# LANL-Bioinformatics/PCRamp

Measured on AMD Instinct MI355X. Metric: primer-pair x target amplification evals/sec, higher is better.
Workload: dtype u32

## Files before the change

### pcramp_amd/csrc/pcr_device.hip

```cpp
#include <hip/hip_runtime.h>
#include <cstring>
#include <rocprim/device/device_radix_sort.hpp>

#include <stdint.h>
#include <string.h>
#include <math.h>
#include <stdlib.h>
#include <string>
#include <vector>
#include <chrono>
#include <algorithm>
#include <unordered_map>
#include <type_traits>
#include <thread>
#include <mutex>
#include <condition_variable>
#include <functional>
#include <memory>
#include <atomic>
#include <cassert>
#include <sched.h>
#include <pthread.h>

#include "../../include/pcramp_hip.h"
#include "pcr_host.hpp"
#include "pcr_launch_queue.hpp"

using pcrhost::Planes;

namespace { thread_local std::string g_err; }
#include "pcr_owned.hpp"

namespace {

using pcrown::DevBuf; using pcrown::MappedBuf; using pcrown::Event; using pcrown::Stream;

#define HIP_TRY(expr) do{ hipError_t e_ = (expr); if(e_ != hipSuccess){ \
	g_err = std::string(#expr) + ": " + hipGetErrorString(e_); return PCR_ERR_DEVICE; } }while(0)

constexpr int TILE_POS = 1024;
constexpr int SCAN_THREADS = 256;
constexpr int SCAN_NPOS = TILE_POS/SCAN_THREADS;

constexpr int KEY_SEQ_SHIFT = 40;
constexpr int KEY_LOC_SHIFT = 8;
constexpr int LOC_BIAS = 64;

struct Hit { uint64_t key; uint32_t cand; uint32_t cnt; };

struct PassMail { volatile uint32_t counters[4]; volatile uint32_t seq; uint32_t pad[11]; };

constexpr uint32_t N_TOUCHED_UNKNOWN_DEV = 0xFFFFFFFFu;

struct IrrDev { Planes w; int32_t loc; uint32_t seq; uint32_t meta;  uint32_t local_id; };

struct DevEntry { Planes w; int32_t loc; uint32_t seq; uint32_t strand; uint32_t pad; };

struct OligoDev {
	Planes m;
	uint32_t floor2;
	float norm;
	int32_t start, stop;
	uint32_t p1, p2;
};

__constant__ float c_taq_mama[256];

const float h_taq_mama[256] = {
	1.000f, 0.968f, 0.947f, 1.034f, 0.547f, 0.253f, 0.230f, 0.359f, 0.606f, 0.282f, 0.372f, 0.347f, 0.957f, 0.382f, 0.399f, 0.687f,
	0.989f, 1.000f, 1.023f, 1.000f, 0.420f, 0.662f, 0.445f, 0.367f, 0.870f, 0.512f, 0.492f, 0.508f, 0.372f, 1.000f, 0.492f, 0.714f,
	1.011f, 1.000f, 1.000f, 1.000f, 0.459f, 0.277f, 0.570f, 0.343f, 0.927f, 0.362f, 0.590f, 0.542f, 0.439f, 0.488f, 0.978f, 0.662f,
	1.000f, 0.907f, 1.000f, 1.000f, 0.382f, 0.234f, 0.228f, 0.542f, 0.763f, 0.309f, 0.410f, 0.473f, 0.426f, 0.347f, 0.423f, 0.947f,
	0.590f, 0.334f, 0.445f, 0.323f, 1.000f, 0.978f, 0.927f, 0.989f, 0.907f, 0.645f, 0.525f, 0.455f, 0.927f, 0.408f, 0.408f, 0.707f,
	0.327f, 0.595f, 0.319f, 0.396f, 0.947f, 1.000f, 0.978f, 0.989f, 0.405f, 0.861f, 0.681f, 0.512f, 0.410f, 0.968f, 0.452f, 0.714f,
	0.410f, 0.420f, 0.590f, 0.311f, 1.023f, 1.000f, 1.000f, 1.000f, 0.488f, 0.898f, 0.907f, 0.566f, 0.442f, 0.449f, 0.989f, 0.707f,
	0.423f, 0.343f, 0.305f, 0.585f, 1.034f, 0.879f, 0.927f, 1.000f, 0.473f, 0.720f, 0.547f, 0.957f, 0.459f, 0.374f, 0.459f, 1.023f,
	1.023f, 0.429f, 0.473f, 0.477f, 1.023f, 0.466f, 0.420f, 0.477f, 1.000f, 0.978f, 0.907f, 0.978f, 0.907f, 0.380f, 0.525f, 0.669f,
	0.442f, 1.046f, 0.455f, 0.470f, 0.432f, 1.058f, 0.481f, 0.485f, 0.917f, 1.000f, 1.023f, 1.023f, 0.336f, 0.968f, 0.534f, 0.639f,
	0.617f, 0.452f, 1.011f, 0.439f, 0.492f, 0.504f, 0.978f, 0.462f, 0.989f, 0.947f, 1.000f, 0.978f, 0.405f, 0.405f, 0.888f, 0.606f,
	0.601f, 0.377f, 0.377f, 1.046f, 0.500f, 0.399f, 0.408f, 1.034f, 0.978f, 0.720f, 0.870f, 1.000f, 0.402f, 0.313f, 0.651f, 0.927f,
	0.978f, 0.462f, 0.466f, 0.488f, 0.420f, 0.239f, 0.225f, 0.336f, 0.504f, 0.269f, 0.319f, 0.656f, 1.000f, 0.835f, 0.907f, 1.034f,
	0.429f, 1.011f, 0.473f, 0.477f, 0.340f, 0.413f, 0.357f, 0.354f, 0.352f, 0.538f, 0.413f, 0.794f, 0.927f, 1.000f, 1.058f, 1.000f,
	0.595f, 0.492f, 0.968f, 0.485f, 0.367f, 0.282f, 0.388f, 0.439f, 0.413f, 0.309f, 0.566f, 0.917f, 0.957f, 0.957f, 1.000f, 0.989f,
	0.590f, 0.380f, 0.410f, 0.968f, 0.364f, 0.223f, 0.230f, 0.416f, 0.321f, 0.239f, 0.301f, 0.645f, 0.978f, 0.714f, 0.947f, 1.000f
};

__device__ __forceinline__ uint32_t funnel(uint32_t lo, uint32_t hi, uint32_t sh)
{
	return __builtin_amdgcn_alignbit(hi, lo, sh);
}

__device__ __forceinline__ uint32_t match_count(uint32_t wa, uint32_t wc, uint32_t wg, uint32_t wt, const uint4 m)
{
	return __popc((wa & m.x) | (wc & m.y) | (wg & m.z) | (wt & m.w));
}

__global__ void k_transpose(const uint8_t *__restrict__ packed, const uint64_t *__restrict__ byte_off,
	const uint64_t *__restrict__ len, const uint64_t *__restrict__ blk_off, const uint32_t *__restrict__ blk_seq,
	uint4 *__restrict__ planes, uint32_t *__restrict__ nib, uint32_t *__restrict__ tb, uint64_t total_blocks)
{
	const uint64_t gb = (uint64_t)blockIdx.x*blockDim.x + threadIdx.x;
	if(gb >= total_blocks) return;
	const uint32_t s = blk_seq[gb];
	const uint64_t b = gb - blk_off[s];
	const uint64_t L = len[s];
	const uint8_t *src = packed + byte_off[s];
	uint32_t a = 0, c = 0, g = 0, t = 0;
	uint32_t nw[4] = {0, 0, 0, 0};
	uint32_t tw[2] = {0, 0};
	for(int j = 0;j < 32;++j){
		const uint64_t pos = b*32 + j;
		if(pos >= L) break;
		const uint8_t v = src[pos >> 1];
		const uint32_t code = (pos & 1) ? (v & 0xF) : (v >> 4);
		a |= (code & 1u) << j;
		c |= ((code >> 1) & 1u) << j;
		g |= ((code >> 2) & 1u) << j;
		t |= ((code >> 3) & 1u) << j;
		nw[j >> 3] |= code << ((j & 7)*4);
		const uint32_t c2 = (code == 2) ? 1u : (code == 4) ? 2u : (code == 8) ? 3u : 0u;
		tw[j >> 4] |= c2 << ((j & 15)*2);
	}
	planes[gb] = make_uint4(a, c, g, t);
	((uint4 *)nib)[gb] = make_uint4(nw[0], nw[1], nw[2], nw[3]);
	((uint2 *)tb)[gb] = make_uint2(tw[0], tw[1]);
}

__global__ void k_valid(const uint4 *__restrict__ planes, const uint64_t *__restrict__ blk_off,
	const uint32_t *__restrict__ blk_seq, const uint64_t *__restrict__ nblk_real, uint32_t *__restrict__ valid,
	uint64_t total_blocks, uint32_t max_degen, uint64_t gc_ok, uint64_t first_block, uint64_t n_blocks)
{
	const uint64_t i = (uint64_t)blockIdx.x*blockDim.x + threadIdx.x;
	if(i >= n_blocks) return;
	const uint64_t gb = first_block + i;
	if(gb >= total_blocks) return;
	const uint32_t s = blk_seq[gb];
	const uint64_t b = gb - blk_off[s];
	if(b >= nblk_real[s]){ valid[gb] = 0; return; }
	const uint4 lo = planes[gb];
	const uint4 hi = planes[gb + 1];
	uint32_t nzl, d2l, d3l, d4l, cgl, nzh, d2h, d3h, d4h, cgh;
	{
		const uint32_t x = lo.x ^ lo.y, y = lo.x & lo.y, u = lo.z ^ lo.w, v = lo.z & lo.w;
		const uint32_t ones = x ^ u, c1 = x & u;
		const uint32_t twos = y ^ v ^ c1;
		const uint32_t fours = (y & v) | (c1 & (y ^ v));
		nzl = lo.x | lo.y | lo.z | lo.w;
		d2l = ~ones & twos & ~fours; d3l = ones & twos; d4l = fours;
		cgl = lo.y | lo.z;
	}
	{
		const uint32_t x = hi.x ^ hi.y, y = hi.x & hi.y, u = hi.z ^ hi.w, v = hi.z & hi.w;
		const uint32_t ones = x ^ u, c1 = x & u;
		const uint32_t twos = y ^ v ^ c1;
		const uint32_t fours = (y & v) | (c1 & (y ^ v));
		nzh = hi.x | hi.y | hi.z | hi.w;
		d2h = ~ones & twos & ~fours; d3h = ones & twos; d4h = fours;
		cgh = hi.y | hi.z;
	}
	uint32_t out = 0;
	for(uint32_t j = 0;j < 32;++j){
		if(funnel(nzl, nzh, j) != 0xFFFFFFFFu) continue;
		const uint32_t ngc = __popc(funnel(cgl, cgh, j));
		if(!((gc_ok >> ngc) & 1ull)) continue;
		const uint32_t n2 = __popc(funnel(d2l, d2h, j));
		const uint32_t n3 = __popc(funnel(d3l, d3h, j));
		const uint32_t n4 = __popc(funnel(d4l, d4h, j));
		const uint32_t e = n2 + 2*n4;
		bool exceeds;
		if(e >= 33){ exceeds = true; }
		else{
			uint64_t p3 = 1;
			for(uint32_t k = 0;k < n3;++k) p3 *= 3;
			exceeds = p3 > ((uint64_t)max_degen >> e);
		}
		if(!exceeds) out |= (1u << j);
	}
	valid[gb] = out;
}

struct HitSink { uint32_t *best; Hit *hits; uint32_t *seq_count; uint32_t *counters; uint32_t cap; uint32_t ncand; uint32_t epoch; };

__device__ __forceinline__ void record_hit_inline(const HitSink &k, uint32_t seq, uint32_t cand, uint64_t key, uint32_t cnt)
{
	const uint32_t tagged = (k.epoch << 8) | cnt;
	const uint32_t old = atomicMax(&k.best[(size_t)seq*k.ncand + cand], tagged);
	if(tagged >= old){
		const uint32_t slot = atomicAdd(&k.seq_count[seq], 1u);
		if(slot < k.cap){
			Hit h; h.key = key; h.cand = cand; h.cnt = cnt;
			k.hits[(size_t)seq*k.cap + slot] = h;
		}
		else{ atomicOr(&k.counters[0], 1u); atomicMax(&k.counters[2], slot + 1); }
	}
}

__device__ __noinline__ void record_hit(const HitSink k, uint32_t seq, uint32_t cand, uint64_t key, uint32_t cnt)
{
	record_hit_inline(k, seq, cand, key, cnt);
}

__device__ __forceinline__ uint64_t make_key(uint32_t seq, int32_t loc, uint32_t strand , uint32_t kind, uint32_t ord)
{
	return ((uint64_t)seq << KEY_SEQ_SHIFT) | ((uint64_t)(uint32_t)(loc + LOC_BIAS) << KEY_LOC_SHIFT) |
		((uint64_t)(strand - 1) << 7) | ((uint64_t)kind << 6) | ord;
}

__global__ void k_touched(const uint32_t *__restrict__ seq_count, uint32_t n, uint32_t *__restrict__ counters, uint32_t *__restrict__ touched)
{
	const uint32_t s = blockIdx.x*blockDim.x + threadIdx.x;
	const uint32_t fill = (s < n) ? seq_count[s] : 0u;
	const bool has = fill > 0;
	const uint64_t mask = __ballot(has);
	if(!mask) return;
	const uint32_t lane = threadIdx.x & 63u, leader = (uint32_t)__builtin_ctzll(mask);
	{
		uint32_t mx = fill;
		for(int d = 32;d > 0;d >>= 1) mx = max(mx, (uint32_t)__shfl_xor((int)mx, d));
		if(lane == leader) atomicMax(&counters[2], mx);
	}
	uint32_t base = 0;
	if(lane == leader) base = atomicAdd(&counters[3], (uint32_t)__builtin_popcountll(mask));
	base = __shfl(base, leader);
	if(has) touched[base + (uint32_t)__builtin_popcountll(mask & ((1ull << lane) - 1ull))] = s;
}

__global__ void k_touched_seg(const uint32_t *__restrict__ seg_hi, uint32_t n, uint32_t *__restrict__ counters, uint32_t *__restrict__ touched)
{
	const uint32_t s = blockIdx.x*blockDim.x + threadIdx.x;
	const bool has = s < n && seg_hi[s] != 0;
	const uint64_t mask = __ballot(has);
	if(!mask) return;
	const uint32_t lane = threadIdx.x & 63u, leader = (uint32_t)__builtin_ctzll(mask);
	uint32_t base = 0;
	if(lane == leader) base = atomicAdd(&counters[3], (uint32_t)__builtin_popcountll(mask));
	base = __shfl(base, leader);
	if(has) touched[base + (uint32_t)__builtin_popcountll(mask & ((1ull << lane) - 1ull))] = s;
}

__global__ __launch_bounds__(SCAN_THREADS) void k_scan(
	const uint4 *__restrict__ planes, const uint32_t *__restrict__ valid,
	const uint64_t *__restrict__ blk_off, const uint64_t *__restrict__ len, const uint8_t *__restrict__ active,
	const uint32_t *__restrict__ tile_seq, const uint32_t *__restrict__ tile_pos0,
	const uint4 *__restrict__ cand_fwd, const uint4 *__restrict__ cand_rc, const uint32_t *__restrict__ cand_floor,
	uint32_t ncand, HitSink sink)
{
	const uint32_t tile = blockIdx.x;
	const uint32_t seq = tile_seq[tile];
	if(!active[seq]) return;
	const uint64_t L = len[seq];
	const uint64_t base = blk_off[seq];
	const uint32_t p0 = tile_pos0[tile];

	uint32_t wa[SCAN_NPOS], wc[SCAN_NPOS], wg[SCAN_NPOS], wt[SCAN_NPOS], ok[SCAN_NPOS];
#pragma unroll
	for(int i = 0;i < SCAN_NPOS;++i){
		const uint32_t p = p0 + threadIdx.x + SCAN_THREADS*i;
		wa[i] = wc[i] = wg[i] = wt[i] = 0; ok[i] = 0;
		if((uint64_t)p + 32 <= L){
			const uint32_t b = p >> 5, sh = p & 31;
			const uint4 lo = planes[base + b];
			const uint4 hi = planes[base + b + 1];
			wa[i] = funnel(lo.x, hi.x, sh); wc[i] = funnel(lo.y, hi.y, sh);
			wg[i] = funnel(lo.z, hi.z, sh); wt[i] = funnel(lo.w, hi.w, sh);
			ok[i] = (valid[base + b] >> sh) & 1u;
		}
	}

	for(uint32_t c = 0;c < ncand;++c){
		const uint4 mf = cand_fwd[c];
		const uint4 mr = cand_rc[c];
		const uint32_t fl = cand_floor[c];
#pragma unroll
		for(int i = 0;i < SCAN_NPOS;++i){
			const uint32_t cf = match_count(wa[i], wc[i], wg[i], wt[i], mf);
			const uint32_t cr = match_count(wa[i], wc[i], wg[i], wt[i], mr);
			if((cf >= fl || cr >= fl) && ok[i]){
				const int32_t p = (int32_t)(p0 + threadIdx.x + SCAN_THREADS*i);
				if(cf >= fl) record_hit(sink, seq, c, make_key(seq, p, 1, 0, 0), cf);
				if(cr >= fl) record_hit(sink, seq, c, make_key(seq, p + 31, 2, 0, 0), cr);
			}
		}
	}
}

constexpr int IRR_THREADS = 256, IRR_PER_LANE = 2;
struct IrrArgs { const IrrDev *irr; const uint32_t *perm; uint32_t n_live; uint32_t off_mask;  };

__device__ __forceinline__ void scan_irr_block(uint32_t block, const IrrDev *__restrict__ irr, const uint32_t *__restrict__ perm, uint32_t n_live,
	const uint8_t *__restrict__ active, const uint4 *__restrict__ cand_fwd, const uint32_t *__restrict__ cand_floor, uint32_t ncand,
	const HitSink &sink)
{
	uint32_t wa[IRR_PER_LANE], wc[IRR_PER_LANE], wg[IRR_PER_LANE], wt[IRR_PER_LANE];
	const uint32_t i0 = block*(IRR_THREADS*IRR_PER_LANE) + threadIdx.x;
#pragma unroll
	for(int k = 0;k < IRR_PER_LANE;++k){
		const uint32_t i = i0 + k*IRR_THREADS;
		wa[k] = wc[k] = wg[k] = wt[k] = 0;
		if(i < n_live){
			const IrrDev e = irr[perm[i]];
			if(active[e.seq]){ wa[k] = e.w.a; wc[k] = e.w.c; wg[k] = e.w.g; wt[k] = e.w.t; }
		}
	}
#pragma unroll 8
	for(uint32_t c = 0;c < ncand;++c){
		const uint4 m = cand_fwd[c];
		const uint32_t fl = max(cand_floor[c], 1u);
		const bool zero_floor = cand_floor[c] == 0;
#pragma unroll
		for(int k = 0;k < IRR_PER_LANE;++k){
			const uint32_t cnt = match_count(wa[k], wc[k], wg[k], wt[k], m);
			if(cnt >= fl || (zero_floor && (wa[k] | wc[k] | wg[k] | wt[k]))){
				const IrrDev e = irr[perm[i0 + k*IRR_THREADS]];
				record_hit(sink, e.seq, c, make_key(e.seq, e.loc, e.meta & 0xFF, 1, (e.meta >> 16) & 0xFF), cnt);
			}
		}
	}
}

__global__ __launch_bounds__(IRR_THREADS) void k_scan_irr(const IrrDev *__restrict__ irr, const uint32_t *__restrict__ perm, uint32_t n_live,
	const uint8_t *__restrict__ active, const uint4 *__restrict__ cand_fwd, const uint32_t *__restrict__ cand_floor, uint32_t ncand,
	HitSink sink)
{
	scan_irr_block(blockIdx.x, irr, perm, n_live, active, cand_fwd, cand_floor, ncand, sink);
}

__device__ __forceinline__ void wave_sync() { __builtin_amdgcn_fence(__ATOMIC_ACQ_REL, "wavefront"); __builtin_amdgcn_wave_barrier(); }

#include "pcr_scan_bitsliced.inc"
#include "pcr_scan_seed.inc"
#include "pcr_scan_seed2.inc"
#include "pcr_scan_seed3.inc"

constexpr int FIN_WAVES = 8;
constexpr uint32_t MAX_BUCKET_CAP = 8192;


__device__ __forceinline__ void materialise_entry_at(uint64_t k, const uint4 *__restrict__ planes, uint64_t seq_base,
	const IrrDev *__restrict__ irr, const uint32_t *__restrict__ irr_off, DevEntry &e)
{
	const uint32_t seq = (uint32_t)(k >> KEY_SEQ_SHIFT);
	const int32_t loc = (int32_t)(uint32_t)((k >> KEY_LOC_SHIFT) & 0xFFFFFFFFull) - LOC_BIAS;
	const uint32_t strand = (uint32_t)((k >> 7) & 1) + 1;
	const uint32_t kind = (uint32_t)((k >> 6) & 1), ord = (uint32_t)(k & 63);
	e.loc = loc; e.seq = seq; e.strand = strand; e.pad = 0;
	if(kind == 0){
		const uint32_t p = (strand == 1) ? (uint32_t)loc : (uint32_t)(loc - 31);
		const uint32_t b = p >> 5, sh = p & 31;
		const uint4 lo = planes[seq_base + b];
		const uint4 hi = planes[seq_base + b + 1];
		const uint32_t a = funnel(lo.x, hi.x, sh), c = funnel(lo.y, hi.y, sh);
		const uint32_t g = funnel(lo.z, hi.z, sh), t = funnel(lo.w, hi.w, sh);
		if(strand == 1){ e.w.a = a; e.w.c = c; e.w.g = g; e.w.t = t; }
		else{ e.w.a = __brev(t); e.w.t = __brev(a); e.w.c = __brev(g); e.w.g = __brev(c); }
	}
	else{
		e.w.a = e.w.c = e.w.g = e.w.t = 0;
		for(uint32_t j = irr_off[seq];j < irr_off[seq + 1];++j){
			const IrrDev r = irr[j];
			if(r.loc == loc && (r.meta & 0xFF) == strand && ((r.meta >> 16) & 0xFF) == ord){ e.w = r.w; break; }
		}
	}
}

__device__ void materialise_entry(uint64_t k, const uint4 *__restrict__ planes, const uint64_t *__restrict__ blk_off,
	const IrrDev *__restrict__ irr, const uint32_t *__restrict__ irr_off, DevEntry &e)
{
	const uint32_t seq = (uint32_t)(k >> KEY_SEQ_SHIFT);
	const int32_t loc = (int32_t)(uint32_t)((k >> KEY_LOC_SHIFT) & 0xFFFFFFFFull) - LOC_BIAS;
	const uint32_t strand = (uint32_t)((k >> 7) & 1) + 1;
	const uint32_t kind = (uint32_t)((k >> 6) & 1), ord = (uint32_t)(k & 63);
	e.loc = loc; e.seq = seq; e.strand = strand; e.pad = 0;
	if(kind == 0){
		const uint32_t p = (strand == 1) ? (uint32_t)loc : (uint32_t)(loc - 31);
		const uint32_t b = p >> 5, sh = p & 31;
		const uint4 lo = planes[blk_off[seq] + b];
		const uint4 hi = planes[blk_off[seq] + b + 1];
		const uint32_t a = funnel(lo.x, hi.x, sh), c = funnel(lo.y, hi.y, sh);
		const uint32_t g = funnel(lo.z, hi.z, sh), t = funnel(lo.w, hi.w, sh);
		if(strand == 1){ e.w.a = a; e.w.c = c; e.w.g = g; e.w.t = t; }
		else{ e.w.a = __brev(t); e.w.t = __brev(a); e.w.c = __brev(g); e.w.g = __brev(c); }
	}
	else{
		e.w.a = e.w.c = e.w.g = e.w.t = 0;
		for(uint32_t j = irr_off[seq];j < irr_off[seq + 1];++j){
			const IrrDev r = irr[j];
			if(r.loc == loc && (r.meta & 0xFF) == strand && ((r.meta >> 16) & 0xFF) == ord){ e.w = r.w; break; }
		}
	}
}

template<int WAVES, bool ALL = false>
__global__ __launch_bounds__(64*WAVES) void k_finalize(const Hit *__restrict__ hits, const uint32_t *__restrict__ seq_count,
	uint32_t cap, const uint32_t *__restrict__ best, uint32_t ncand, const uint4 *__restrict__ planes,
	const uint64_t *__restrict__ blk_off, const IrrDev *__restrict__ irr, const uint32_t *__restrict__ irr_off,
	DevEntry *__restrict__ db, uint32_t *__restrict__ seg_hi, uint32_t *__restrict__ counters, uint32_t epoch,
	const uint32_t *__restrict__ touched)
{
	extern __shared__ __attribute__((aligned(16))) uint64_t fin_lds[];
	__shared__ uint32_t part_all[64*WAVES];
	const uint32_t wave = threadIdx.x >> 6, lane = threadIdx.x & 63;
	uint32_t np2cap = 1; while(np2cap < cap) np2cap <<= 1;
	for(uint32_t t_idx = blockIdx.x*WAVES + wave;t_idx < counters[3];t_idx += gridDim.x*WAVES){
	const uint32_t seq = touched[t_idx];
	uint64_t *fin_keys = fin_lds + (size_t)wave*np2cap;
	uint32_t *part = part_all + wave*64;
	const uint32_t n = min(seq_count[seq], cap);
	uint32_t np2 = 1; while(np2 < n) np2 <<= 1;
	for(uint32_t i = lane;i < np2;i += 64){
		uint64_t k = ~0ull;
		if(i < n){
			const Hit h = hits[(size_t)seq*cap + i];
			if constexpr (ALL) k = h.key;
			else if(((epoch << 8) | h.cnt) == best[(size_t)seq*ncand + h.cand]) k = h.key;
		}
		fin_keys[i] = k;
	}
	wave_sync();
	for(uint32_t k = 2;k <= np2;k <<= 1){
		for(uint32_t j = k >> 1;j > 0;j >>= 1){
			for(uint32_t i = lane;i < np2;i += 64){
				const uint32_t l = i ^ j;
				if(l > i){
					const uint64_t a = fin_keys[i], b = fin_keys[l];
					const bool up = ((i & k) == 0);
					if((a > b) == up){ fin_keys[i] = b; fin_keys[l] = a; }
				}
			}
			wave_sync();
		}
	}
	const uint32_t chunk = (np2 + 63)/64;
	const uint32_t lo = lane*chunk, hi = min(np2, lo + chunk);
	uint32_t cnt = 0;
	for(uint32_t i = lo;i < hi;++i){
		const uint64_t k = fin_keys[i];
		if(k != ~0ull && (i == 0 || fin_keys[i - 1] != k)) ++cnt;
	}
	part[lane] = cnt;
	wave_sync();
	if(lane == 0){
		uint32_t run = 0;
		for(int t = 0;t < 64;++t){ const uint32_t c = part[t]; part[t] = run; run += c; }
		seg_hi[seq] = seq*cap + run;
	}
	wave_sync();
	uint32_t rank = part[lane];
	for(uint32_t i = lo;i < hi;++i){
		const uint64_t k = fin_keys[i];
		if(k != ~0ull && (i == 0 || fin_keys[i - 1] != k)){
			DevEntry e;
			materialise_entry(k, planes, blk_off, irr, irr_off, e);
			db[(size_t)seq*cap + rank] = e;
			++rank;
		}
	}
	wave_sync();
	}
}

constexpr int FINBIG_THREADS = 256;
constexpr uint32_t MAX_BUCKET_CAP_GLOBAL = 65536;
template<bool ALL = false>
__global__ __launch_bounds__(FINBIG_THREADS) void k_finalize_big(const Hit *__restrict__ hits, const uint32_t *__restrict__ seq_count,
	uint32_t cap, const uint32_t *__restrict__ best, uint32_t ncand, const uint4 *__restrict__ planes,
	const uint64_t *__restrict__ blk_off, const IrrDev *__restrict__ irr, const uint32_t *__restrict__ irr_off,
	DevEntry *__restrict__ db, uint32_t *__restrict__ seg_hi, uint32_t *__restrict__ counters, uint32_t epoch,
	const uint32_t *__restrict__ touched, uint64_t *__restrict__ scratch)
{
	__shared__ uint32_t part[FINBIG_THREADS];
	if(blockIdx.x >= counters[3]) return;
	const uint32_t seq = touched[blockIdx.x], tid = threadIdx.x;
	uint32_t np2cap = 1; while(np2cap < cap) np2cap <<= 1;
	uint64_t *fin_keys = scratch + (size_t)blockIdx.x*np2cap;
	const uint32_t n = min(seq_count[seq], cap);
	uint32_t np2 = 1; while(np2 < n) np2 <<= 1;
	for(uint32_t i = tid;i < np2;i += FINBIG_THREADS){
		uint64_t k = ~0ull;
		if(i < n){
			const Hit h = hits[(size_t)seq*cap + i];
			if constexpr (ALL) k = h.key;
			else if(((epoch << 8) | h.cnt) == best[(size_t)seq*ncand + h.cand]) k = h.key;
		}
		fin_keys[i] = k;
	}
	__syncthreads();
	for(uint32_t k = 2;k <= np2;k <<= 1){
		for(uint32_t j = k >> 1;j > 0;j >>= 1){
			for(uint32_t i = tid;i < np2;i += FINBIG_THREADS){
				const uint32_t l = i ^ j;
				if(l > i){
					const uint64_t a = fin_keys[i], b = fin_keys[l];
					const bool up = ((i & k) == 0);
					if((a > b) == up){ fin_keys[i] = b; fin_keys[l] = a; }
				}
			}
			__syncthreads();
		}
	}
	const uint32_t chunk = (np2 + FINBIG_THREADS - 1)/FINBIG_THREADS;
	const uint32_t lo = min(np2, tid*chunk), hi = min(np2, lo + chunk);
	uint32_t cnt = 0;
	for(uint32_t i = lo;i < hi;++i){
		const uint64_t k = fin_keys[i];
		if(k != ~0ull && (i == 0 || fin_keys[i - 1] != k)) ++cnt;
	}
	part[tid] = cnt;
	__syncthreads();
	if(tid == 0){
		uint32_t run = 0;
		for(int t = 0;t < FINBIG_THREADS;++t){ const uint32_t c = part[t]; part[t] = run; run += c; }
		seg_hi[seq] = seq*cap + run;
	}
	__syncthreads();
	uint32_t rank = part[tid];
	for(uint32_t i = lo;i < hi;++i){
		const uint64_t k = fin_keys[i];
		if(k != ~0ull && (i == 0 || fin_keys[i - 1] != k)){
			DevEntry e;
			materialise_entry(k, planes, blk_off, irr, irr_off, e);
			db[(size_t)seq*cap + rank] = e;
			++rank;
		}
	}
}

#include "pcr_screen.inc"

#include "pcr_sw.inc"
#include "pcr_thermo.inc"

constexpr uint32_t N_TOUCHED_UNKNOWN = 0xFFFFFFFFu;
constexpr uint32_t EPOCH_LIMIT = (1u << 24) - 1;

struct SeqSet {
	uint32_t n = 0;
	std::vector<std::vector<uint8_t> > packed;
	std::vector<uint64_t> len, blk_off, nblk_real;
	std::vector<float> weight; DevBuf<float> d_weight; bool weight_dirty = true;
	std::vector<uint8_t> active;
	std::vector<std::vector<pcrhost::IrrEntry> > irr_host;
	uint64_t total_blocks = 0;
	uint32_t n_tiles = 0, n_irr = 0;
	bool ctrl_clean = false;
	bool touched_from_seg = false;
	uint32_t bucket_cap = 64;
	DevBuf<uint32_t> irr_perm; uint32_t irr_size_count[256];
	DevBuf<uint4> planes;
	DevBuf<uint32_t> valid, nib, tb, blk_seq, tile_seq, tile_pos0, irr_off, degen_tiles;
	uint32_t *valid_d() const { return valid.p + S2_VALID_FRONT; }
	uint32_t *tb_d() const { return tb.p + S2_TB_FRONT; }
	DevBuf<uint8_t> tile_degen; uint32_t n_degen_tiles = 0;
	DevBuf<TileDesc> tile_desc;
	DevBuf<uint64_t> d_len, d_blk_off, d_nblk_real;
	DevBuf<uint8_t> d_active;
	std::vector<uint8_t> has_eos; DevBuf<uint8_t> d_has_eos;
	DevBuf<IrrDev> irr;
	DevBuf<IrrScan> irr_scan;
	DevBuf<uint32_t> irx_first, irx_last, irx_words, irx_sums; bool irx_valid = false, irx_usable = false;
	uint32_t irr_n_multi = 0;
	DevBuf<uint32_t> pix_first, pix_last, pix_sums, blk_info, blk_local, blk_tile0; DevBuf<uint4> pix_ent; std::vector<uint32_t> pix_start_h; uint64_t pix_generation = 0; bool pix_valid = false, pix_usable = false;
	DevBuf<uint8_t> codes; DevBuf<uint64_t> d_code_off; bool have_codes = false;
	bool have_db = false;
	uint32_t n_entries = 0;
	uint32_t db_cap = 0;
	uint64_t n_slots = 0;
	DevBuf<DevEntry> db;
	DevBuf<uint32_t> touched;
	DevBuf<uint32_t> ctrl;
	uint32_t n_touched = 0;
	bool touched_built = false;
	uint32_t *d_seg_hi = nullptr;
};

}

struct HostPool {
	std::vector<std::thread> th;
	std::mutex m; std::condition_variable cv_go, cv_done;
	std::function<void(unsigned)> fn; unsigned n_parts = 0, next = 0, pending = 0; uint64_t gen = 0; bool stop = false;
	explicit HostPool(unsigned n_workers){ for(unsigned i = 0;i < n_workers;++i) th.emplace_back([this]{ work(); }); }
	~HostPool(){ { std::lock_guard<std::mutex> lk(m); stop = true; } cv_go.notify_all(); for(std::thread &t : th) t.join(); }
	unsigned size() const { return (unsigned)th.size(); }
	void work()
	{
		uint64_t seen = 0;
		std::unique_lock<std::mutex> lk(m);
		while(true){
			cv_go.wait(lk, [&]{ return stop || gen != seen; });
			if(stop) return;
			seen = gen;
			while(next < n_parts){ const unsigned p = next++; lk.unlock(); fn(p); lk.lock(); }
			if(--pending == 0) cv_done.notify_one();
		}
	}
	void run(unsigned parts, std::function<void(unsigned)> f)
	{
		std::unique_lock<std::mutex> lk(m);
		fn = std::move(f); n_parts = parts; next = 0; pending = (unsigned)th.size(); ++gen;
		cv_go.notify_all();
		while(next < n_parts){ const unsigned p = next++; lk.unlock(); fn(p); lk.lock(); }
		cv_done.wait(lk, [&]{ return pending == 0; });
	}
};

namespace { struct PassJob; struct Launcher; }

struct pcr_ctx {
	int device = 0;
	std::unique_ptr<HostPool> pool_;
	HostPool &host_pool()
	{
		if(!pool_){ const unsigned hw = std::max(1u, std::thread::hardware_concurrency()); pool_.reset(new HostPool(std::min(hw, 16u) - 1u)); }
		return *pool_;
	}
	Stream stream;
	Stream aux_stream;
	std::string design_text;
	DevBuf<uint64_t> split_where;
	pcr_params params;
	pcrhost::PackFilter filt;
	SeqSet sets[PCR_N_SETS];
	DevBuf<uint32_t> best, counters, mask, status;
	int scan_version = 3;
	bool force_seed1 = false;
	struct S2Key { uint32_t a, c, g, t, floor_; bool operator==(const S2Key &o) const { return a == o.a && c == o.c && g == o.g && t == o.t && floor_ == o.floor_; } };
	struct S2KeyHash { size_t operator()(const S2Key &k) const { uint64_t h = 0x9E3779B97F4A7C15ull; for(uint32_t v : {k.a, k.c, k.g, k.t, k.floor_}){ h ^= v; h *= 0x100000001B3ull; h ^= h >> 29; } return (size_t)h; } };
	struct S2Entry { std::vector<uint32_t> seeds;  uint32_t off_mask; bool seedable; uint4 mask;  };
	std::unordered_map<S2Key, S2Entry, S2KeyHash> s2_cache;
	std::vector<pcrhost::Seed> s2_tmp;
	static constexpr int S3_CHUNK_SETS = 4;
	struct S3Chunks { uint64_t gen = 0; uint32_t total = 0; std::vector<uint32_t> run; };
	struct S3Entry : S2Entry { std::vector<uint8_t> spans;  S3Chunks chunks[S3_CHUNK_SETS]; uint32_t next_slot = 0; };
	std::unordered_map<S2Key, S3Entry, S2KeyHash> s3_cache;
	std::vector<pcrhost::FoldSeed> s3_tmp;
	struct S3Launch { Seed3Slices W; uint32_t n_chunks, per_wg, slice_cap, n_irr_wg; };
	bool no_seed3 = false, s3_attr_set = false;
	bool s3_next = true;
	bool s2_attr_set = false; uint32_t s2_dbg = 0; bool no_irr_index = false;
	std::unordered_map<S2Key, S2Entry, S2KeyHash> s1_cache;
	DevBuf<uint32_t> s1_image, s1_heads, s1_multi, s1_part;
	bool host_seed_tables = false;
	DevBuf<Hit> hits;
	DevBuf<uint64_t> bits_fr, bits_rf;
	DevBuf<OligoDev> oligos;
	DevBuf<SwJob> sw_jobs; DevBuf<SwOut> sw_out; DevBuf<uint8_t> sw_q, sw_qlen, sw_t, entry_codes, entry_lens;
	DevBuf<AmpRec> amp_recs, amp_recs2; DevBuf<BgPairDev> bg_pairs;
	DevBuf<uint64_t> amp_keys; DevBuf<uint32_t> amp_pkeys, amp_pair_start; DevBuf<uint8_t> sort_tmp;
	DevBuf<thermo::Job> th_jobs; DevBuf<thermo::JobOut> th_out; DevBuf<int> th_dg; DevBuf<uint2> th_map; DevBuf<uint32_t> th_bad;
	float th_dg_salt = -1.0f;
	DevBuf<unsigned long long> th_dbg; bool th_attr_set = false;
	std::vector<thermo::Job> th_host_jobs; std::vector<thermo::JobOut> th_host_res;
	MappedBuf<uint8_t> sw_pin; Event sw_done[2];
	DevBuf<pcr_amplicon> mx_amp;
	DevBuf<OligoDev> opt_oligos; DevBuf<uint2> opt_jobs; DevBuf<float> opt_cov; DevBuf<uint32_t> opt_loc, opt_tasks;
	DevBuf<Planes> mx_keys; uint32_t mx_n_keys = 0; DevBuf<uint32_t> mx_count;
	DevBuf<uint8_t> pool_in, pool_tmp; DevBuf<uint32_t> pool_cnt, pool_ord; DevBuf<uint64_t> pool_eoff, pool_ioff, pool_keys; DevBuf<uint2> pool_items; DevBuf<pcr_product> pool_rec;
	DevBuf<uint8_t> site_in, site_tmp; DevBuf<uint32_t> site_cnt, site_ord, site_flag; DevBuf<uint64_t> site_eoff, site_joff, site_keys; DevBuf<uint2> site_items; DevBuf<float4> site_res; DevBuf<pcr_site> site_rec;
	bool site_attr_set = false;
	pcr_comm *shard_comm = nullptr; uint64_t shard_first = 0, shard_n_total = 0; int shard_mode = 0;
	DevBuf<uint64_t> sh_rec, sh_full; DevBuf<uint8_t> sh_stage;
	std::vector<uint64_t> shard_bounds; DevBuf<uint64_t> d_shard_bounds;
	bool design_ready = false; DevBuf<uint64_t> sh_bits;
	std::vector<std::vector<uint8_t> > samp_packed; std::vector<uint64_t> samp_len;
	void drop_shard(){ shard_comm = nullptr; shard_mode = 0; shard_bounds.clear(); design_ready = false; samp_packed.clear(); samp_len.clear(); }
	pcr_comm *trial_comm = nullptr;
	size_t amp_cap = size_t(1) << 20;
	uint32_t n_cu = 256;
	DevBuf<uint64_t> fin_scratch;
	std::vector<uint16_t> seed_count; std::vector<uint8_t> seed_fill, seed_own;
	uint32_t epoch = 0;
	uint32_t debug_epoch = 0;
	bool opt_pm_global = false;
	uint32_t opt_dbg_wg_tasks = 0, opt_dbg_task_cap = 0;
	uint64_t best_seen = 0;
	static constexpr int STAGE_RING = 4;
	struct StageSlot { MappedBuf<uint8_t> buf; Event done; bool busy = false;
	                   uint32_t guard_seq = 0;  };
	StageSlot stage[STAGE_RING]; int stage_next = 0;
	struct DirectSlot { DevBuf<uint8_t> buf{true}; uint32_t guard_seq = 0; };
	DirectSlot dstage[STAGE_RING]; int dstage_next = 0;
	bool direct_ok = false;
	typedef PassMail Mail;
	static constexpr uint32_t MAIL_RING = 8;
	MappedBuf<Mail> mail;
	uint32_t mail_seq = 0;
	MappedBuf<uint8_t> ret;
	MappedBuf<uint8_t> in;
	MappedBuf<uint32_t> ret_flag; uint32_t ret_seq = 0;
	struct Pending {
		uint32_t seq; int which; std::vector<pcr_pair> pairs; int opt5, opt3; float thr; uint32_t min_len;
		pcr_amplify_args args; uint64_t *d_fr, *d_rf;
	};
	std::vector<Pending> pending;
	bool launch_thread = true;
	Launcher *launcher = nullptr; pcrq::Client lq_client; uint64_t n_pipelined = 0;
	std::mutex job_m; std::vector<PassJob *> job_free, job_all;
	DevBuf<uint8_t> arena;
	const uint4 *d_cand_fwd = nullptr, *d_cand_rc = nullptr; const uint32_t *d_cand_floor = nullptr;
	const OligoDev *d_oligos = nullptr;
	bool debug_log = false;
	bool timing = false; double t_host[8] = {0, 0, 0, 0, 0, 0, 0, 0}; uint64_t n_timed = 0;
	bool prof = false; uint32_t prof_stride = 1, prof_pass = 0;
	std::vector<std::pair<Event, Event> > prof_events;
	double prof_ms = 0.0; uint64_t prof_launches = 0;
	std::vector<std::pair<Event, Event> > prof_events_k[PCR_PROF_KERNELS];
	double prof_ms_k[PCR_PROF_KERNELS] = {0.0, 0.0, 0.0}; uint64_t prof_launches_k[PCR_PROF_KERNELS] = {0, 0, 0};
};

namespace {

int drain(pcr_ctx *ctx);
int flush_launcher(pcr_ctx *ctx);
void detach_launcher(pcr_ctx *ctx);
void free_jobs(pcr_ctx *ctx);

struct ProfScope {
	pcr_ctx *ctx; int k; Event e0, e1;
	ProfScope(pcr_ctx *c, int kernel, bool on = true) : ctx(c), k(kernel)
	{
		if(!on || !ctx->prof || k < 0 || k >= PCR_PROF_KERNELS) return;
		if(e0.create() != hipSuccess || e1.create() != hipSuccess){ e0.release(); return; }
		(void)hipEventRecord(e0, ctx->stream);
	}
	void finish()
	{
		if(!e0) return;
		(void)hipEventRecord(e1, ctx->stream);
		((k == PCR_PROF_SCAN) ? ctx->prof_events : ctx->prof_events_k[k]).emplace_back(std::move(e0), std::move(e1));
	}
	~ProfScope() { finish(); }
};
constexpr int PCR_SET_SCRATCH = 3;
inline bool set_ok(pcr_set which) { return (unsigned)which <= (unsigned)PCR_SET_MULTIPLEX; }
#define CHECK_SET(which) do{ if(!set_ok(which)){ g_err = "unknown sequence set (PCR_SET_TARGET, PCR_SET_BACKGROUND or PCR_SET_MULTIPLEX)"; return PCR_ERR_ARG; } }while(0)
#define FLUSH(ctx) do{ if((ctx)->launcher){ const int frc_ = flush_launcher(ctx); if(frc_ != PCR_OK) return frc_; } }while(0)
#define DRAIN(ctx) do{ FLUSH(ctx); if(!(ctx)->pending.empty()){ const int drc_ = drain(ctx); if(drc_ != PCR_OK) return drc_; } }while(0)

struct HostTimer {
	pcr_ctx *ctx; int slot; std::chrono::steady_clock::time_point t0;
	HostTimer(pcr_ctx *c, int s) : ctx(c), slot(s) { if(ctx->timing) t0 = std::chrono::steady_clock::now(); }
	void next(int s)
	{
		if(!ctx->timing) return;
		const auto t1 = std::chrono::steady_clock::now();
		ctx->t_host[slot] += std::chrono::duration<double, std::micro>(t1 - t0).count();
		slot = s; t0 = t1;
	}
	~HostTimer() { next(slot); }
};

__global__ void k_apply_splits(const uint64_t *__restrict__ where, uint32_t n, uint32_t *__restrict__ planes , uint32_t *__restrict__ nib)
{
	const uint32_t i = blockIdx.x*blockDim.x + threadIdx.x;
	if(i >= n) return;
	const uint64_t gb = where[2*(size_t)i];
	const uint32_t bit = (uint32_t)where[2*(size_t)i + 1];
	const uint32_t m = ~(1u << bit);
	for(int k = 0;k < 4;++k) atomicAnd(&planes[gb*4 + k], m);
	atomicAnd(&nib[gb*4 + (bit >> 3)], ~(0xFu << ((bit & 7u)*4u)));
}

int upload_irregular(pcr_ctx *ctx, SeqSet &S)
{
	const auto tu0 = std::chrono::steady_clock::now();
	auto ms_since = [&](){ return std::chrono::duration<double, std::milli>(std::chrono::steady_clock::now() - tu0).count(); };
	double t_flat = 0, t_sort = 0, t_scan = 0, t_copy1 = 0;
	size_t total = 0;
	for(uint32_t s = 0;s < S.n;++s) total += S.irr_host[s].size();
	std::vector<IrrDev> flat(total);
	std::vector<uint32_t> off(S.n + 1, 0);
	for(int k = 0;k < 256;++k) S.irr_size_count[k] = 0;
	{
		size_t at = 0;
		for(uint32_t s = 0;s < S.n;++s){
			off[s] = (uint32_t)at;
			const std::vector<pcrhost::IrrEntry> &v = S.irr_host[s];
			for(size_t k = 0;k < v.size();++k){
				const pcrhost::IrrEntry &e = v[k];
				IrrDev &d = flat[at++];
				d.w = e.w; d.loc = e.loc; d.seq = s;
				d.meta = (uint32_t)e.strand | ((uint32_t)e.cws << 8) | ((uint32_t)e.ord << 16);
				d.local_id = (uint32_t)k;
				++S.irr_size_count[e.cws & 0xFF];
			}
		}
	}
	off[S.n] = (uint32_t)flat.size();
	S.n_irr = (uint32_t)flat.size();
	t_flat = ms_since();
	std::vector<uint32_t> perm(flat.size());
	t_sort = ms_since();
	int rc;
	{
		auto spread = [](uint64_t v) -> uint64_t {
			v = (v | (v << 16)) & 0x0000FFFF0000FFFFull; v = (v | (v << 8)) & 0x00FF00FF00FF00FFull; v = (v | (v << 4)) & 0x0F0F0F0F0F0F0F0Full;
			v = (v | (v << 2)) & 0x3333333333333333ull; v = (v | (v << 1)) & 0x5555555555555555ull; return v;
		};
		uint32_t start[256];
		uint32_t run = 0;
		for(int k = 255;k >= 0;--k){ start[k] = run; run += S.irr_size_count[k]; }
		std::vector<IrrScan> scan(perm.size());
		uint32_t n_multi = 0;
		for(size_t i = 0;i < flat.size();++i){
			const IrrDev &d = flat[i];
			const uint32_t at = start[(d.meta >> 8) & 0xFF]++;
			perm[at] = (uint32_t)i;
			const uint32_t multi = (d.w.a & d.w.c) | (d.w.a & d.w.g) | (d.w.a & d.w.t) | (d.w.c & d.w.g) | (d.w.c & d.w.t) | (d.w.g & d.w.t);
			if(multi) ++n_multi;
			const uint32_t lo = d.w.c | d.w.t, hi = d.w.g | d.w.t;
			const uint64_t code = spread(lo) | (spread(hi) << 1);
			IrrScan r; r.w0 = (uint32_t)code; r.w1 = (uint32_t)(code >> 32); r.idx_flags = (uint32_t)i | (multi ? 0x80000000u : 0u); r.seq = d.seq;
			scan[at] = r;
		}
		S.irr_n_multi = n_multi; S.irx_valid = false;
		t_scan = ms_since();
		if((rc = S.irr_scan.ensure_slack(scan.size() + 1)) != PCR_OK) return rc;
		if(!scan.empty()) HIP_TRY(hipMemcpy(S.irr_scan.p, scan.data(), scan.size()*sizeof(IrrScan), hipMemcpyHostToDevice));
	}
	t_copy1 = ms_since();
	if((rc = S.irr_perm.ensure_slack(perm.size() + 1)) != PCR_OK) return rc;
	if(!perm.empty()) HIP_TRY(hipMemcpyAsync(S.irr_perm.p, perm.data(), perm.size()*sizeof(uint32_t), hipMemcpyHostToDevice, ctx->stream));
	if((rc = S.irr.ensure_slack(flat.size())) != PCR_OK) return rc;
	if((rc = S.irr_off.ensure(off.size())) != PCR_OK) return rc;
	if(!flat.empty()) HIP_TRY(hipMemcpyAsync(S.irr.p, flat.data(), flat.size()*sizeof(IrrDev), hipMemcpyHostToDevice, ctx->stream));
	HIP_TRY(hipMemcpyAsync(S.irr_off.p, off.data(), off.size()*sizeof(uint32_t), hipMemcpyHostToDevice, ctx->stream));
	HIP_TRY(hipStreamSynchronize(ctx->stream));
	if(ctx->timing && flat.size() > 100000) fprintf(stderr, "[pcramp] irregular list of %zu words: flat %.1f  order %.1f  scan records %.1f  first copy %.1f  other copies %.1f ms\n", flat.size(), t_flat, t_sort - t_flat, t_scan - t_sort, t_copy1 - t_scan, ms_since() - t_copy1);
	return PCR_OK;
}

void launch_exclusive_scan(pcr_ctx *ctx, uint32_t *counts, uint32_t *starts, uint32_t n, uint32_t *sums)
{
	const uint32_t n_blocks = (n + 4095u)/4096u;
	hipLaunchKernelGGL(k_scan_blocks, dim3(n_blocks), dim3(1024), 0, ctx->stream, counts, starts, n, sums);
	hipLaunchKernelGGL(k_scan_sums, dim3(1), dim3(1024), 0, ctx->stream, sums, n_blocks);
	hipLaunchKernelGGL(k_scan_add, dim3(n_blocks), dim3(1024), 0, ctx->stream, starts, counts, n, sums);
}

constexpr uint32_t IRX_MAX_RUN = 1024;
int ensure_irr_index(pcr_ctx *ctx, SeqSet &S)
{
	if(S.irx_valid) return PCR_OK;
	int rc;
	if((rc = S.irx_first.ensure(IRX_KEYS + 4)) != PCR_OK) return rc;
	if((rc = S.irx_last.ensure(IRX_KEYS + 4)) != PCR_OK) return rc;
	if((rc = S.irx_words.ensure_slack((size_t)24*S.n_irr + 4)) != PCR_OK) return rc;
	const uint32_t n_blocks = (IRX_KEYS + 4095u)/4096u;
	if((rc = S.irx_sums.ensure(n_blocks + 4)) != PCR_OK) return rc;
	HIP_TRY(hipMemsetAsync(S.irx_last.p, 0, (size_t)IRX_KEYS*sizeof(uint32_t), ctx->stream));
	if(S.n_irr){
		hipLaunchKernelGGL(k_irx_count, dim3((S.n_irr + 255)/256), dim3(256), 0, ctx->stream, S.irr.p, S.n_irr, S.irx_last.p);
		HIP_TRY(hipGetLastError());
	}
	{
		uint32_t longest = 0;
		HIP_TRY(hipMemsetAsync(S.irx_sums.p + n_blocks, 0, sizeof(uint32_t), ctx->stream));
		hipLaunchKernelGGL(k_irx_max, dim3(256), dim3(256), 0, ctx->stream, S.irx_last.p, IRX_KEYS, S.irx_sums.p + n_blocks);
		HIP_TRY(hipMemcpyAsync(&longest, S.irx_sums.p + n_blocks, sizeof(uint32_t), hipMemcpyDeviceToHost, ctx->stream));
		HIP_TRY(hipStreamSynchronize(ctx->stream));
		S.irx_usable = longest <= IRX_MAX_RUN;
		if(!S.irx_usable){ S.irx_valid = true; return PCR_OK; }
	}
	launch_exclusive_scan(ctx, S.irx_last.p, S.irx_first.p, IRX_KEYS, S.irx_sums.p);
	HIP_TRY(hipGetLastError());
	if(S.n_irr){
		hipLaunchKernelGGL(k_irx_scatter, dim3((S.n_irr + 255)/256), dim3(256), 0, ctx->stream, S.irr.p, S.n_irr, S.irx_last.p, S.irx_words.p);
		HIP_TRY(hipGetLastError());
	}
	S.irx_valid = true;
	return PCR_OK;
}

int ensure_pos_index(pcr_ctx *ctx, SeqSet &S)
{
	if(S.pix_valid) return PCR_OK;
	S.pix_valid = true; S.pix_usable = false;
	if(S.total_blocks == 0 || S.total_blocks*32 >= (uint64_t(1) << 32) - 64) return PCR_OK;
	int rc;
	if((rc = S.pix_first.ensure(PIX_KEYS + 4)) != PCR_OK) return rc;
	if((rc = S.pix_last.ensure(PIX_KEYS + 4)) != PCR_OK) return rc;
	const uint32_t n_blocks = (PIX_KEYS + 4095u)/4096u;
	if((rc = S.pix_sums.ensure(n_blocks + 4)) != PCR_OK) return rc;
	if((rc = S.pix_ent.ensure(S.total_blocks*32 + 64)) != PCR_OK) return rc;
	{
		if(S.n >= (1u << 30)){ return PCR_OK; }
		if((rc = S.blk_info.ensure(S.total_blocks + 1)) != PCR_OK) return rc;
		if((rc = S.blk_local.ensure(S.total_blocks + 1)) != PCR_OK) return rc;
		std::vector<uint32_t> tile0((size_t)S.n + 1);
		uint64_t t0 = 0;
		for(uint32_t q = 0;q < S.n;++q){ tile0[q] = (uint32_t)t0; t0 += (S.len[q] >= 32) ? (S.len[q] - 7 + TILE_POS - 1)/TILE_POS : 0; }
		tile0[S.n] = (uint32_t)t0;
		if(t0 >= (uint64_t(1) << 32)) return PCR_OK;
		if((rc = S.blk_tile0.ensure((size_t)S.n + 1)) != PCR_OK) return rc;
		HIP_TRY(hipMemcpyAsync(S.blk_tile0.p, tile0.data(), ((size_t)S.n + 1)*sizeof(uint32_t), hipMemcpyHostToDevice, ctx->stream));
		hipLaunchKernelGGL(k_blk_info, dim3((unsigned)((S.total_blocks + 255)/256)), dim3(256), 0, ctx->stream, S.blk_seq.p, S.d_blk_off.p, S.d_len.p,
			S.blk_tile0.p, S.tile_degen.p, S.d_active.p, S.total_blocks, S.blk_info.p, S.blk_local.p);
		HIP_TRY(hipGetLastError());
		HIP_TRY(hipStreamSynchronize(ctx->stream));
	}
	HIP_TRY(hipMemsetAsync(S.pix_last.p, 0, (size_t)PIX_KEYS*sizeof(uint32_t), ctx->stream));
	const unsigned grid = (unsigned)((S.total_blocks + 255)/256);
	hipLaunchKernelGGL(k_pix_build<false>, dim3(grid), dim3(256), 0, ctx->stream, S.tb_d(), S.blk_seq.p, S.d_blk_off.p, S.d_len.p, S.total_blocks, S.pix_last.p, (uint4 *)nullptr);
	launch_exclusive_scan(ctx, S.pix_last.p, S.pix_first.p, PIX_KEYS, S.pix_sums.p);
	hipLaunchKernelGGL(k_pix_build<true>, dim3(grid), dim3(256), 0, ctx->stream, S.tb_d(), S.blk_seq.p, S.d_blk_off.p, S.d_len.p, S.total_blocks, S.pix_last.p, S.pix_ent.p);
	HIP_TRY(hipGetLastError());
	{
		S.pix_start_h.resize((size_t)PIX_KEYS + 1);
		HIP_TRY(hipMemcpyAsync(S.pix_start_h.data(), S.pix_first.p, (size_t)PIX_KEYS*sizeof(uint32_t), hipMemcpyDeviceToHost, ctx->stream));
		HIP_TRY(hipMemcpyAsync(S.pix_start_h.data() + PIX_KEYS, S.pix_last.p + (PIX_KEYS - 1), sizeof(uint32_t), hipMemcpyDeviceToHost, ctx->stream));
		HIP_TRY(hipStreamSynchronize(ctx->stream));
		static uint64_t generations = 0;
		S.pix_generation = ++generations;
	}
	S.pix_usable = true;
	return PCR_OK;
}

int run_valid(pcr_ctx *ctx, SeqSet &S, uint64_t first_block, uint64_t n_blocks)
{
	if(n_blocks == 0) return PCR_OK;
	const unsigned threads = 256;
	const unsigned grid = (unsigned)((n_blocks + threads - 1)/threads);
	hipLaunchKernelGGL(k_valid, dim3(grid), dim3(threads), 0, ctx->stream, S.planes.p, S.d_blk_off.p, S.blk_seq.p,
		S.d_nblk_real.p, S.valid_d(), S.total_blocks, ctx->filt.max_degen, ctx->filt.gc_ok, first_block, n_blocks);
	HIP_TRY(hipGetLastError());
	return PCR_OK;
}

int build_tile_desc(pcr_ctx *ctx, SeqSet &S)
{
	if(S.n_tiles == 0) return PCR_OK;
	int rc = S.tile_desc.ensure(S.n_tiles);
	if(rc != PCR_OK) return rc;
	hipLaunchKernelGGL(k_tile_desc, dim3((S.n_tiles + 255)/256), dim3(256), 0, ctx->stream, S.d_blk_off.p, S.d_len.p, S.d_active.p, S.tile_seq.p,
		S.tile_pos0.p, S.tile_degen.p, S.n_tiles, S.tile_desc.p);
	HIP_TRY(hipGetLastError());
	return PCR_OK;
}

void fill_oligo_planes(OligoDev &o, const Planes &m, float thr2)
{
	o.m = m;
	const unsigned size = (unsigned)pcrhost::planes_size(o.m);
	o.floor2 = (unsigned)((float)size*thr2);
	o.norm = (size > 0) ? (float)(1.0/size) : 0.0f;
	o.start = pcrhost::planes_start(o.m);
	o.stop = pcrhost::planes_stop(o.m);
	o.p1 = (o.stop >= 1) ? pcrhost::planes_nibble(o.m, o.stop - 1) : 0;
	o.p2 = (o.stop >= 0) ? pcrhost::planes_nibble(o.m, o.stop) : 0;
}

void fill_oligo(OligoDev &o, const uint64_t w[2], float thr2) { fill_oligo_planes(o, pcrhost::planes_of_word(w), thr2); }

__global__ void k_stage(const uint4 *__restrict__ src, uint4 *__restrict__ dst, uint32_t n16,
	uint4 *__restrict__ z0, uint32_t n0, uint4 *__restrict__ z1, uint32_t n1, uint4 *__restrict__ z2, uint32_t n2)
{
	const uint32_t i = blockIdx.x*blockDim.x + threadIdx.x, stride = gridDim.x*blockDim.x;
	for(uint32_t k = i;k < n16;k += stride) dst[k] = src[k];
	const uint4 zero = make_uint4(0, 0, 0, 0);
	for(uint32_t k = i;k < n0;k += stride) z0[k] = zero;
	for(uint32_t k = i;k < n1;k += stride) z1[k] = zero;
	for(uint32_t k = i;k < n2;k += stride) z2[k] = zero;
}

enum SpinEnd { SPIN_SEEN, SPIN_IDLE, SPIN_ERROR };
template<class Seen> inline SpinEnd spin_until(hipStream_t stream, Seen seen, hipError_t &err)
{
	for(uint64_t spins = 1;!seen();++spins){
		__builtin_ia32_pause();
		if((spins & 0x3FFF) == 0){
			err = hipStreamQuery(stream);
			if(err == hipSuccess) return SPIN_IDLE;
			if(err != hipErrorNotReady) return SPIN_ERROR;
		}
	}
	return SPIN_SEEN;
}

int wait_published(pcr_ctx *ctx, uint32_t seq)
{
	const PassMail *const slot = ctx->mail.host + (seq % pcr_ctx::MAIL_RING);
	hipError_t e = hipSuccess;
	const SpinEnd end = spin_until(ctx->stream, [&]{
		const uint32_t v = __atomic_load_n((const uint32_t *)&slot->seq, __ATOMIC_ACQUIRE);
		return v >= seq && (v - seq) % pcr_ctx::MAIL_RING == 0; }, e);
	if(end == SPIN_ERROR){ g_err = std::string("device pass failed: ") + hipGetErrorString(e); return PCR_ERR_DEVICE; }
	return PCR_OK;
}

struct Stager {
	pcr_ctx *ctx; size_t used = 0; bool direct = false;
	explicit Stager(pcr_ctx *c) : ctx(c) {}
	pcr_ctx::StageSlot *slot = nullptr; pcr_ctx::DirectSlot *dslot = nullptr;
	uint8_t *host = nullptr, *dev = nullptr;
	int begin_direct(size_t bytes)
	{
		direct = true;
		dslot = &ctx->dstage[ctx->dstage_next];
		ctx->dstage_next = (ctx->dstage_next + 1) % pcr_ctx::STAGE_RING;
		if(dslot->guard_seq){ const int grc = wait_published(ctx, dslot->guard_seq); if(grc != PCR_OK) return grc; dslot->guard_seq = 0; }
		if(bytes + 256 > dslot->buf.cap){
			if(dslot->buf.p) HIP_TRY(hipStreamSynchronize(ctx->stream));
			const int rc = dslot->buf.ensure(std::max<size_t>((bytes + 256)*2, 1 << 17));
			if(rc != PCR_OK) return rc;
		}
		host = dev = dslot->buf.p;
		used = 0;
		return PCR_OK;
	}
	void seal(uint32_t pass_seq)
	{
		__builtin_ia32_sfence();
		dslot->guard_seq = pass_seq + 1;
	}
	int begin(size_t bytes)
	{
		slot = &ctx->stage[ctx->stage_next];
		ctx->stage_next = (ctx->stage_next + 1) % pcr_ctx::STAGE_RING;
		if(slot->busy){ HIP_TRY(hipEventSynchronize(slot->done)); slot->busy = false; }
		if(slot->guard_seq){ const int grc = wait_published(ctx, slot->guard_seq); if(grc != PCR_OK) return grc; slot->guard_seq = 0; }
		int rc = slot->buf.ensure(bytes, std::max<size_t>(bytes*2, 1 << 16));
		if(rc != PCR_OK) return rc;
		host = slot->buf.host; dev = slot->buf.dev;
		if(!slot->done) HIP_TRY(slot->done.create(hipEventDisableTiming));
		rc = ctx->arena.ensure(bytes + 256);
		used = 0;
		return rc;
	}
	template<class T> T *put(const T *src, size_t n)
	{
		used = (used + 15) & ~size_t(15);
		memcpy(host + used, src, n*sizeof(T));
		T *at = (T *)((direct ? dev : ctx->arena.p) + used);
		used += n*sizeof(T);
		return at;
	}
	int ship(void *z0 = nullptr, size_t bytes0 = 0, void *z1 = nullptr, size_t bytes1 = 0, void *z2 = nullptr, size_t bytes2 = 0, uint32_t guard_seq = 0)
	{
		const uint32_t n16 = (uint32_t)((used + 15)/16), n0 = (uint32_t)((bytes0 + 15)/16), n1 = (uint32_t)((bytes1 + 15)/16), n2 = (uint32_t)((bytes2 + 15)/16);
		const uint32_t most = std::max(std::max(n16, n2), std::max(n0, n1));
		if(most){
			const unsigned grid = std::min<unsigned>((most + 255)/256, 512u);
			hipLaunchKernelGGL(k_stage, dim3(grid), dim3(256), 0, ctx->stream, (const uint4 *)dev, (uint4 *)ctx->arena.p, n16,
				(uint4 *)z0, n0, (uint4 *)z1, n1, (uint4 *)z2, n2);
			HIP_TRY(hipGetLastError());
		}
		if(guard_seq) slot->guard_seq = guard_seq;
		else{
			HIP_TRY(hipEventRecord(slot->done, ctx->stream));
			slot->busy = true;
		}
		return PCR_OK;
	}
};

__global__ void k_publish(const uint32_t *__restrict__ counters, pcr_ctx::Mail *mail, uint32_t seq)
{
	if(threadIdx.x < 4) mail->counters[threadIdx.x] = counters[threadIdx.x];
	__threadfence_system();
	__syncthreads();
	if(threadIdx.x == 0) __hip_atomic_store((uint32_t *)&mail->seq, seq, __ATOMIC_RELEASE, __HIP_MEMORY_SCOPE_SYSTEM);
}

int mail_wait(pcr_ctx *ctx, uint32_t seq, uint32_t out[4])
{
	pcr_ctx::Mail *const slot = ctx->mail.host + (seq % pcr_ctx::MAIL_RING);
	auto seen = [&]{ return __atomic_load_n((const uint32_t *)&slot->seq, __ATOMIC_ACQUIRE) == seq; };
	hipError_t e = hipSuccess;
	const SpinEnd end = spin_until(ctx->stream, seen, e);
	if(end == SPIN_ERROR){ g_err = std::string("device pass failed: ") + hipGetErrorString(e); return PCR_ERR_DEVICE; }
	if(end == SPIN_IDLE && !seen()){ g_err = "device pass finished without publishing its counters"; return PCR_ERR_DEVICE; }
	for(int i = 0;i < 4;++i) out[i] = slot->counters[i];
	return PCR_OK;
}

__global__ void k_return(const uint4 *__restrict__ s0, uint32_t n0, const uint4 *__restrict__ s1, uint32_t n1,
	const uint4 *__restrict__ s2, uint32_t n2, uint4 *__restrict__ dst)
{
	const uint32_t stride = gridDim.x*blockDim.x, t = blockIdx.x*blockDim.x + threadIdx.x;
	for(uint32_t i = t;i < n0;i += stride) dst[i] = s0[i];
	for(uint32_t i = t;i < n1;i += stride) dst[n0 + i] = s1[i];
	for(uint32_t i = t;i < n2;i += stride) dst[n0 + n1 + i] = s2[i];
}

__global__ void k_return_flag(uint32_t *flag, uint32_t seq)
{
	__threadfence_system();
	__hip_atomic_store(flag, seq, __ATOMIC_RELEASE, __HIP_MEMORY_SCOPE_SYSTEM);
}

int return_to_host(pcr_ctx *ctx, const void *s0, size_t b0, const void *s1, size_t b1, const void *s2, size_t b2, const uint8_t *out[3])
{
	const uint32_t n0 = (uint32_t)((b0 + 15)/16), n1 = (uint32_t)((b1 + 15)/16), n2 = (uint32_t)((b2 + 15)/16);
	const size_t need = ((size_t)n0 + n1 + n2)*16;
	int rc;
	if(!ctx->ret_flag.host){
		if((rc = ctx->ret_flag.ensure(64)) != PCR_OK) return rc;
		*ctx->ret_flag.host = 0;
	}
	if(need > ctx->ret.cap){
		HIP_TRY(hipStreamSynchronize(ctx->stream));
		if((rc = ctx->ret.ensure(need, std::max<size_t>(need*2, 1 << 20))) != PCR_OK) return rc;
	}
	const uint32_t most = std::max(n0, std::max(n1, n2));
	if(most){
		const unsigned grid = std::min<unsigned>((most + 255)/256, 1024u);
		hipLaunchKernelGGL(k_return, dim3(grid), dim3(256), 0, ctx->stream, (const uint4 *)s0, n0, (const uint4 *)s1, n1, (const uint4 *)s2, n2, (uint4 *)ctx->ret.dev);
		HIP_TRY(hipGetLastError());
	}
	const uint32_t seq = ++ctx->ret_seq;
	hipLaunchKernelGGL(k_return_flag, dim3(1), dim3(1), 0, ctx->stream, ctx->ret_flag.dev, seq);
	HIP_TRY(hipGetLastError());
	auto seen = [&]{ return __atomic_load_n((const uint32_t *)ctx->ret_flag.host, __ATOMIC_ACQUIRE) == seq; };
	hipError_t e = hipSuccess;
	const SpinEnd end = spin_until(ctx->stream, seen, e);
	if(end == SPIN_ERROR){ g_err = std::string("device work failed: ") + hipGetErrorString(e); return PCR_ERR_DEVICE; }
	if(end == SPIN_IDLE && !seen()){ g_err = "device work finished without raising the return flag"; return PCR_ERR_DEVICE; }
	out[0] = ctx->ret.host; out[1] = ctx->ret.host + (size_t)n0*16; out[2] = ctx->ret.host + ((size_t)n0 + n1)*16;
	return PCR_OK;
}

int mapped_input(pcr_ctx *ctx, const void *src, size_t bytes, const void **dev_out)
{
	if(bytes > ctx->in.cap){
		HIP_TRY(hipStreamSynchronize(ctx->stream));
		const int rc = ctx->in.ensure(bytes, std::max<size_t>(bytes*2, 1 << 18));
		if(rc != PCR_OK) return rc;
	}
	memcpy(ctx->in.host, src, bytes);
	*dev_out = ctx->in.dev;
	return PCR_OK;
}

struct FusedAmp {
	const pcr_pair *pairs; uint32_t n_pairs; const pcr_amplify_args *a; uint64_t *d_fr, *d_rf;
	bool staged = false; const OligoDev *d_oligos = nullptr; uint32_t pub_seq = 0; const uint32_t *pub_counters = nullptr;
	bool posted = false;
};

void build_oligos(const pcr_pair *pairs, uint32_t n_pairs, const pcr_amplify_args *a, std::vector<OligoDev> &ol)
{
	const float thr2 = a->collect_threshold*a->collect_threshold;
	ol.resize(2*(size_t)n_pairs);
	for(uint32_t i = 0;i < n_pairs;++i){
		fill_oligo(ol[2*i], pairs[i].f.w, thr2);
		fill_oligo(ol[2*i + 1], pairs[i].r.w, thr2);
	}
}

int ensure_touched(pcr_ctx *ctx, SeqSet &S)
{
	if(S.touched_built || !S.have_db || !S.ctrl.p) return PCR_OK;
	if(S.touched_from_seg) hipLaunchKernelGGL(k_touched_seg, dim3((S.n + 255)/256), dim3(256), 0, ctx->stream, S.d_seg_hi, S.n, S.ctrl.p, S.touched.p);
	else hipLaunchKernelGGL(k_touched, dim3((S.n + 255)/256), dim3(256), 0, ctx->stream, S.ctrl.p + 8, S.n, S.ctrl.p, S.touched.p);
	HIP_TRY(hipGetLastError());
	uint32_t n = 0;
	HIP_TRY(hipMemcpyAsync(&n, S.ctrl.p + 3, sizeof(uint32_t), hipMemcpyDeviceToHost, ctx->stream));
	HIP_TRY(hipStreamSynchronize(ctx->stream));
	S.n_touched = n; S.n_entries = n ? 1 : 0; S.touched_built = true;
	return PCR_OK;
}

int amplify_launch(pcr_ctx *ctx, SeqSet &S, const pcr_pair *pairs, uint32_t n_pairs, const pcr_amplify_args *a,
	uint64_t *d_fr, uint64_t *d_rf, const FusedAmp *fa = nullptr)
{
	{ const int erc = ensure_touched(ctx, S); if(erc != PCR_OK) return erc; }
	if(!S.have_db){ g_err = "pcr_amplify: no word DB (call pcr_select_words first)"; return PCR_ERR_STATE; }
	const uint64_t words = (S.n + 63)/64;
	const size_t bits_bytes = (size_t)n_pairs*words*sizeof(uint64_t);
	if(S.n_entries == 0 || n_pairs == 0){
		if(bits_bytes){
			HIP_TRY(hipMemsetAsync(d_fr, 0, bits_bytes, ctx->stream));
			HIP_TRY(hipMemsetAsync(d_rf, 0, bits_bytes, ctx->stream));
		}
		return PCR_OK;
	}
	HostTimer timer(ctx, 4);
	int rc;
	const bool prestaged = fa && fa->staged;
	if(prestaged) ctx->d_oligos = fa->d_oligos;
	else{
		std::vector<OligoDev> ol;
		build_oligos(pairs, n_pairs, a, ol);
		Stager st(ctx);
		if((rc = st.begin(ol.size()*sizeof(OligoDev) + 64)) != PCR_OK) return rc;
		ctx->d_oligos = st.put(ol.data(), ol.size());
		const bool vec_ok = ((uintptr_t)d_fr % 16 == 0) && ((uintptr_t)d_rf % 16 == 0) && (bits_bytes % 16 == 0);
		if(!vec_ok){
			HIP_TRY(hipMemsetAsync(d_fr, 0, bits_bytes, ctx->stream));
			HIP_TRY(hipMemsetAsync(d_rf, 0, bits_bytes, ctx->stream));
		}
		if((rc = vec_ok ? st.ship(d_fr, bits_bytes, d_rf, bits_bytes) : st.ship()) != PCR_OK) return rc;
	}
	timer.next(5);
	const uint32_t mask_words = (2*n_pairs + 31)/32;
	if((rc = ctx->mask.ensure((size_t)S.n_slots*mask_words)) != PCR_OK) return rc;
	if((rc = ctx->status.ensure(1)) != PCR_OK) return rc;
	const bool dev_n = S.n_touched == N_TOUCHED_UNKNOWN;
	const uint32_t *n_dev = dev_n ? S.ctrl.p + 3 : nullptr;
	const uint32_t n_t = dev_n ? 0u : S.n_touched, n_db = n_t*S.db_cap;
	const unsigned threads = dev_n ? 256 : 128;
	const unsigned grid = dev_n ? (unsigned)std::min<uint64_t>(((uint64_t)S.n*S.db_cap + threads - 1)/threads, 1024) : (n_db + threads - 1)/threads;
	const unsigned mgrid = dev_n ? std::min<unsigned>((S.n + MATCH_WAVES - 1)/MATCH_WAVES, 1024u) : (n_t + MATCH_WAVES - 1)/MATCH_WAVES;
	hipLaunchKernelGGL(k_match, dim3(std::max(mgrid, 1u)), dim3(64*MATCH_WAVES), 0, ctx->stream, S.db.p, n_t, n_dev, S.db_cap,
		S.touched.p, S.d_seg_hi, ctx->d_oligos, 2*n_pairs, mask_words, ctx->mask.p, ctx->status.p,
		prestaged ? fa->pub_counters : (const uint32_t *)nullptr, prestaged ? ctx->mail.dev + (fa->pub_seq % pcr_ctx::MAIL_RING) : (pcr_ctx::Mail *)nullptr,
		prestaged ? fa->pub_seq : 0u);
	HIP_TRY(hipGetLastError());
	hipLaunchKernelGGL(k_pair, dim3(grid), dim3(threads), 0, ctx->stream, S.db.p, n_db, n_dev, S.db_cap, S.touched.p, S.d_seg_hi, ctx->mask.p,
		mask_words, ctx->d_oligos, n_pairs, S.planes.p, S.d_blk_off.p, S.d_len.p, S.d_active.p, a->amp_min, a->amp_max,
		a->ident_threshold, a->use_taq_mama, d_fr, d_rf, words, ctx->status.p);
	HIP_TRY(hipGetLastError());
	return PCR_OK;
}

template<int NSLOT, int KLO>
int launch_scan2_nw(pcr_ctx *ctx, SeqSet &S, uint32_t nw, uint32_t group0, uint32_t n_groups, uint32_t gw, uint32_t ncand, const HitSink &sink,
	const uint32_t *d_tab, const uint32_t *d_bias, const uint32_t *tile_ids, uint32_t n_tiles, const uint32_t *orient_ids)
{
#define SCAN2_ARGS S.nib.p, S.planes.p, S.valid_d(), S.d_blk_off.p, S.d_len.p, S.d_active.p, S.tile_seq.p, S.tile_pos0.p, \
	d_tab, d_bias, group0, gw, tile_ids, orient_ids, ctx->d_cand_fwd, ctx->d_cand_rc, ctx->d_cand_floor, ncand, sink
	const dim3 grid(n_tiles, n_groups), block(SCAN2_THREADS);
	switch(nw){
		case 1: hipLaunchKernelGGL((k_scan2<1, NSLOT, KLO>), grid, block, 0, ctx->stream, SCAN2_ARGS); break;
		case 2: hipLaunchKernelGGL((k_scan2<2, NSLOT, KLO>), grid, block, 0, ctx->stream, SCAN2_ARGS); break;
		case 3: hipLaunchKernelGGL((k_scan2<3, NSLOT, KLO>), grid, block, 0, ctx->stream, SCAN2_ARGS); break;
		case 4: hipLaunchKernelGGL((k_scan2<4, NSLOT, KLO>), grid, block, 0, ctx->stream, SCAN2_ARGS); break;
		case 5: hipLaunchKernelGGL((k_scan2<5, NSLOT, KLO>), grid, block, 0, ctx->stream, SCAN2_ARGS); break;
		case 6: hipLaunchKernelGGL((k_scan2<6, NSLOT, KLO>), grid, block, 0, ctx->stream, SCAN2_ARGS); break;
		case 7: hipLaunchKernelGGL((k_scan2<7, NSLOT, KLO>), grid, block, 0, ctx->stream, SCAN2_ARGS); break;
		default: hipLaunchKernelGGL((k_scan2<8, NSLOT, KLO>), grid, block, 0, ctx->stream, SCAN2_ARGS); break;
	}
#undef SCAN2_ARGS
	HIP_TRY(hipGetLastError());
	return PCR_OK;
}

int launch_scan2(pcr_ctx *ctx, SeqSet &S, const Scan2Tables &T, uint32_t ncand, const HitSink &sink,
	const uint32_t *d_tab, const uint32_t *d_bias, const uint32_t *tile_ids, uint32_t n_tiles, const uint32_t *orient_ids)
{
	if(n_tiles == 0 || T.n_groups == 0) return PCR_OK;
	const uint32_t full = (T.last_words == T.gw) ? T.n_groups : T.n_groups - 1;
	int rc = PCR_OK;
	if(full){
		rc = (T.nslot == 26) ? launch_scan2_nw<26, 3>(ctx, S, T.gw, 0, full, T.gw, ncand, sink, d_tab, d_bias, tile_ids, n_tiles, orient_ids)
			: launch_scan2_nw<32, 0>(ctx, S, T.gw, 0, full, T.gw, ncand, sink, d_tab, d_bias, tile_ids, n_tiles, orient_ids);
		if(rc != PCR_OK) return rc;
	}
	if(full < T.n_groups){
		rc = (T.nslot == 26) ? launch_scan2_nw<26, 3>(ctx, S, T.last_words, full, 1, T.gw, ncand, sink, d_tab, d_bias, tile_ids, n_tiles, orient_ids)
			: launch_scan2_nw<32, 0>(ctx, S, T.last_words, full, 1, T.gw, ncand, sink, d_tab, d_bias, tile_ids, n_tiles, orient_ids);
	}
	return rc;
}

int count_entries(pcr_ctx *ctx, SeqSet &S)
{
	uint64_t total = 0;
	if(S.n_touched){
		std::vector<uint32_t> hi(S.n);
		HIP_TRY(hipMemcpyAsync(hi.data(), S.d_seg_hi, S.n*sizeof(uint32_t), hipMemcpyDeviceToHost, ctx->stream));
		HIP_TRY(hipStreamSynchronize(ctx->stream));
		for(uint32_t q = 0;q < S.n;++q){ if(hi[q]) total += hi[q] - (uint64_t)q*S.db_cap; }
	}
	S.n_entries = (uint32_t)total;
	return PCR_OK;
}

}

extern "C" {

const char *pcr_last_error(void) { return g_err.c_str(); }

pcr_ctx *pcr_create(int device, void *hip_stream, const pcr_params *params)
{
	int count = 0;
	if(hipGetDeviceCount(&count) != hipSuccess || count <= 0){
		g_err = "pcr_create: no HIP device available (this library has no CPU fallback)";
		return nullptr;
	}
	if(device < 0 || device >= count){ g_err = "pcr_create: bad device index"; return nullptr; }
	if(hipSetDevice(device) != hipSuccess){ g_err = "pcr_create: hipSetDevice failed"; return nullptr; }
	hipDeviceProp_t prop;
	if(hipGetDeviceProperties(&prop, device) != hipSuccess){ g_err = "pcr_create: hipGetDeviceProperties failed"; return nullptr; }
	if(std::string(prop.gcnArchName).find("gfx950") == std::string::npos){
		g_err = std::string("pcr_create: device is ") + prop.gcnArchName + ", this build targets gfx950 only";
		return nullptr;
	}
	pcr_ctx *ctx = new pcr_ctx();
	ctx->device = device;
	if(hip_stream) ctx->stream.borrow((hipStream_t)hip_stream);
	else if(ctx->stream.create() != hipSuccess){ g_err = "pcr_create: hipStreamCreate failed"; delete ctx; return nullptr; }
	if(params){ ctx->params = *params; }
	else{ ctx->params.pack_max_degen = 256; ctx->params.pack_min_gc = 0.0f; ctx->params.pack_max_gc = 1.0f; }
	{ hipDeviceProp_t prop; if(hipGetDeviceProperties(&prop, device) == hipSuccess && prop.multiProcessorCount > 0) ctx->n_cu = (uint32_t)prop.multiProcessorCount; }
	if(const char *v = getenv("PCRAMP_TIMING")) ctx->timing = v[0] == '1';
	ctx->debug_log = getenv("PCRAMP_DEBUG") != nullptr;
	if(const char *v = getenv("PCRAMP_DEBUG_EPOCH")) ctx->debug_epoch = (uint32_t)strtoul(v, nullptr, 0);
	if(const char *v = getenv("PCRAMP_OPT_PM")) ctx->opt_pm_global = v[0] == 'g';
	if(const char *v = getenv("PCRAMP_DEBUG_OPT_TASKS")){ unsigned a = 0, b = 0; if(sscanf(v, "%u,%u", &a, &b) >= 1){ ctx->opt_dbg_wg_tasks = a; ctx->opt_dbg_task_cap = b; } }
	if(const char *v = getenv("PCRAMP_SEED")) ctx->force_seed1 = v[0] == '1';
	if(const char *v = getenv("PCRAMP_SEED_TABLES")) ctx->host_seed_tables = v[0] == 'h';
	if(const char *v = getenv("PCRAMP_S2DBG")) ctx->s2_dbg = (uint32_t)atoi(v);
	if(const char *v = getenv("PCRAMP_IRR_INDEX")) ctx->no_irr_index = v[0] == '0';
	if(const char *v = getenv("PCRAMP_SEED3")) ctx->no_seed3 = v[0] == '0';
	if(const char *v = getenv("PCRAMP_S3_NEXT")) ctx->s3_next = v[0] != '0';
	if(const char *v = getenv("PCRAMP_LAUNCH_THREAD")) ctx->launch_thread = v[0] != '0';
	if(const char *v = getenv("PCRAMP_SCAN")){ if(v[0] == '1') ctx->scan_version = 1; else if(v[0] == '2') ctx->scan_version = 2; }
	{
		const char *v = getenv("PCRAMP_STAGE");
		if(!(v && v[0] == 'k') && prop.isLargeBar){
			DevBuf<uint32_t> probe(true); MappedBuf<uint32_t> back; const std::string err_before = g_err;
			constexpr uint32_t PROBE_WORDS = 1024;
			if(probe.ensure(PROBE_WORDS) == PCR_OK && back.ensure(PROBE_WORDS*sizeof(uint32_t)) == PCR_OK){
				hipPointerAttribute_t at;
				bool ok = hipPointerGetAttributes(&at, probe.p) == hipSuccess;
				for(int round = 0;ok && round < 2;++round){
					volatile uint32_t *w = (volatile uint32_t *)probe.p;
					for(uint32_t i = 0;i < PROBE_WORDS;++i){ w[i] = 0x9E3779B9u*(i + 1) + (uint32_t)round; back.host[i] = 0; }
					__builtin_ia32_sfence();
					hipLaunchKernelGGL(k_stage, dim3(1), dim3(256), 0, ctx->stream, (const uint4 *)probe.p, (uint4 *)back.dev, PROBE_WORDS/4,
						(uint4 *)nullptr, 0u, (uint4 *)nullptr, 0u, (uint4 *)nullptr, 0u);
					ok = hipGetLastError() == hipSuccess && hipStreamSynchronize(ctx->stream) == hipSuccess;
					for(uint32_t i = 0;ok && i < PROBE_WORDS;++i) ok = back.host[i] == 0x9E3779B9u*(i + 1) + (uint32_t)round;
				}
				ctx->direct_ok = ok;
			}
			else{ (void)hipGetLastError(); g_err = err_before; }
		}
	}
	ctx->filt.max_degen = ctx->params.pack_max_degen;
	ctx->filt.set_gc(ctx->params.pack_min_gc, ctx->params.pack_max_gc);
	if(hipMemcpyToSymbol(HIP_SYMBOL(c_taq_mama), h_taq_mama, sizeof(h_taq_mama)) != hipSuccess ||
	   hipMemcpyToSymbol(HIP_SYMBOL(thermo::c_H), PCR_NN_H, sizeof(PCR_NN_H)) != hipSuccess ||
	   hipMemcpyToSymbol(HIP_SYMBOL(thermo::c_S), PCR_NN_S, sizeof(PCR_NN_S)) != hipSuccess ||
	   hipMemcpyToSymbol(HIP_SYMBOL(thermo::c_loop_S), PCR_LOOP_S, sizeof(PCR_LOOP_S)) != hipSuccess ||
	   hipMemcpyToSymbol(HIP_SYMBOL(thermo::c_bulge_S), PCR_BULGE_S, sizeof(PCR_BULGE_S)) != hipSuccess ||
	   hipMemcpyToSymbol(HIP_SYMBOL(thermo::c_hairpin_S), PCR_HAIRPIN_S, sizeof(PCR_HAIRPIN_S)) != hipSuccess ||
	   hipMemcpyToSymbol(HIP_SYMBOL(thermo::c_special_H), PCR_SPECIAL_H, sizeof(PCR_SPECIAL_H)) != hipSuccess ||
	   hipMemcpyToSymbol(HIP_SYMBOL(thermo::c_special_S), PCR_SPECIAL_S, sizeof(PCR_SPECIAL_S)) != hipSuccess ||
	   hipMemcpyToSymbol(HIP_SYMBOL(thermo::c_special_key), PCR_SPECIAL_KEY, sizeof(PCR_SPECIAL_KEY)) != hipSuccess ||
	   hipMemcpyToSymbol(HIP_SYMBOL(thermo::c_wc), PCR_WC, sizeof(PCR_WC)) != hipSuccess){
		g_err = "pcr_create: hipMemcpyToSymbol failed"; delete ctx; return nullptr;
	}
	if(ctx->mail.ensure(sizeof(pcr_ctx::Mail)*pcr_ctx::MAIL_RING) != PCR_OK){ g_err = "pcr_create: mapped host allocation failed"; delete ctx; return nullptr; }
	memset((void *)ctx->mail.host, 0, sizeof(pcr_ctx::Mail)*pcr_ctx::MAIL_RING);
	return ctx;
}

void pcr_destroy(pcr_ctx *ctx)
{
	if(!ctx) return;
	(void)hipSetDevice(ctx->device);
	(void)flush_launcher(ctx);
	detach_launcher(ctx);
	(void)hipStreamSynchronize(ctx->stream);
	if(ctx->aux_stream) (void)hipStreamSynchronize(ctx->aux_stream);
	ctx->pending.clear();
	free_jobs(ctx);
	if(ctx->timing && ctx->n_timed){
		const double n = (double)ctx->n_timed;
		fprintf(stderr, "[pcramp] host us/pass by stage: A (plan, caller's thread) %.1f  B (stage + launch, %s) %.1f  (%llu of %llu passes pipelined, queue depth <= %u)\n",
			ctx->t_host[0]/n, ctx->n_pipelined ? "launcher thread" : "caller's thread", (ctx->t_host[1] + ctx->t_host[2])/n,
			(unsigned long long)ctx->n_pipelined, (unsigned long long)ctx->n_timed, ctx->lq_client.max_depth);
		fprintf(stderr, "[pcramp] host us/pass: plan %.1f  stage %.1f  launch %.1f  wait %.1f | amplify prep %.1f  launch %.1f  (%llu passes)\n",
			ctx->t_host[0]/n, ctx->t_host[1]/n, ctx->t_host[2]/n, ctx->t_host[3]/n, ctx->t_host[4]/n, ctx->t_host[5]/n, (unsigned long long)ctx->n_timed);
	}
	delete ctx;
}

uint32_t pcr_num_sequences(pcr_ctx *ctx, pcr_set which) { return (ctx && set_ok(which)) ? ctx->sets[which].n : 0; }
uint64_t pcr_bitset_words(pcr_ctx *ctx, pcr_set which) { return (ctx && set_ok(which)) ? (ctx->sets[which].n + 63)/64 : 0; }

int pcr_staging_mode(pcr_ctx *ctx) { return (ctx && ctx->direct_ok) ? 1 : 0; }

int pcr_launcher_stats(pcr_ctx *ctx, uint64_t *passes_pipelined, uint32_t *max_queue_depth)
{
	if(!ctx){ g_err = "null ctx"; return PCR_ERR_ARG; }
	if(passes_pipelined) *passes_pipelined = ctx->n_pipelined;
	if(max_queue_depth) *max_queue_depth = ctx->lq_client.max_depth;
	return PCR_OK;
}

int pcr_live_resources(uint64_t out[4])
{
	if(!out){ g_err = "pcr_live_resources: bad argument"; return PCR_ERR_ARG; }
	for(int k = 0;k < 4;++k) out[k] = pcrown::g_live[k].load();
	return PCR_OK;
}

int pcr_synchronize(pcr_ctx *ctx)
{
	if(!ctx){ g_err = "null ctx"; return PCR_ERR_ARG; }
	HIP_TRY(hipSetDevice(ctx->device));
	DRAIN(ctx);
	HIP_TRY(hipStreamSynchronize(ctx->stream));
	return PCR_OK;
}

static int load_sequences_impl(pcr_ctx *ctx, int which, const uint8_t *packed4, const uint64_t *byte_offsets,
	const uint64_t *lengths, const float *weights, uint32_t n);

int pcr_load_sequences(pcr_ctx *ctx, pcr_set which, const uint8_t *packed4, const uint64_t *byte_offsets,
	const uint64_t *lengths, const float *weights, uint32_t n)
{
	if(!set_ok(which)){ g_err = "pcr_load_sequences: unknown sequence set"; return PCR_ERR_ARG; }
	return load_sequences_impl(ctx, (int)which, packed4, byte_offsets, lengths, weights, n);
}

static int load_sequences_impl(pcr_ctx *ctx, int which, const uint8_t *packed4, const uint64_t *byte_offsets,
	const uint64_t *lengths, const float *weights, uint32_t n)
{
	if(!ctx || which < 0 || which >= PCR_N_SETS || (n && (!packed4 || !byte_offsets || !lengths))){
		g_err = "pcr_load_sequences: bad argument"; return PCR_ERR_ARG;
	}
	DRAIN(ctx);
	if(n >= (1u << 24)){ g_err = "pcr_load_sequences: at most 2^24-1 sequences per GPU shard"; return PCR_ERR_CAPACITY; }
	HIP_TRY(hipSetDevice(ctx->device));
	HIP_TRY(hipStreamSynchronize(ctx->stream));
	SeqSet &S = ctx->sets[which];
	S.have_db = false; S.n_entries = 0; S.have_codes = false;
	S.n = n;
	S.packed.assign(n, std::vector<uint8_t>());
	S.len.assign(lengths, lengths + n);
	if(which == PCR_SET_TARGET) ctx->drop_shard();
	if(which == PCR_SET_TARGET || which == PCR_SET_BACKGROUND) ctx->trial_comm = nullptr;
	S.weight.assign(n, 1.0f);
	if(weights) S.weight.assign(weights, weights + n);
	S.weight_dirty = true;
	S.ctrl_clean = false; S.touched_from_seg = false;
	S.active.assign(n, 1);
	S.has_eos.assign(n, 0);
	S.blk_off.assign(n + 1, 0);
	S.nblk_real.assign(n, 0);
	S.irr_host.assign(n, std::vector<pcrhost::IrrEntry>());
	uint64_t total_bytes = 0, total_blocks = 0, n_tiles = 0;
	std::vector<uint64_t> dev_byte_off(n);
	for(uint32_t s = 0;s < n;++s){
		if(lengths[s] >= (uint64_t(1) << 31)){ g_err = "pcr_load_sequences: sequence longer than 2^31-1 bases"; return PCR_ERR_CAPACITY; }
		const uint64_t nb = (lengths[s] + 1)/2;
		S.packed[s].assign(packed4 + byte_offsets[s], packed4 + byte_offsets[s] + nb);
		if((lengths[s] & 1) && nb) S.packed[s][nb - 1] &= 0xF0;
		{
			const std::vector<uint8_t> &b = S.packed[s];
			bool eos = false;
			const uint64_t full = lengths[s]/2;
			for(uint64_t k = 0;k < full && !eos;++k) eos = ((b[k] & 0xF0) == 0) || ((b[k] & 0x0F) == 0);
			if(!eos && (lengths[s] & 1)) eos = ((b[full] & 0xF0) == 0);
			S.has_eos[s] = eos ? 1 : 0;
		}
		dev_byte_off[s] = total_bytes;
		total_bytes += nb;
		S.blk_off[s] = total_blocks;
		S.nblk_real[s] = (lengths[s] + 31)/32;
		total_blocks += S.nblk_real[s] + 2;
		if(lengths[s] >= 32) n_tiles += (lengths[s] - 7 + TILE_POS - 1)/TILE_POS;
	}
	S.blk_off[n] = total_blocks;
	S.total_blocks = total_blocks;
	if(n_tiles >= (uint64_t(1) << 31)){ g_err = "pcr_load_sequences: too many tiles"; return PCR_ERR_CAPACITY; }
	S.n_tiles = (uint32_t)n_tiles;

	std::vector<uint32_t> blk_seq(total_blocks), tile_seq(n_tiles), tile_pos0(n_tiles);
	uint64_t t = 0;
	S.pix_valid = false; S.pix_usable = false;
	for(uint32_t s = 0;s < n;++s){
		for(uint64_t b = S.blk_off[s];b < S.blk_off[s + 1];++b) blk_seq[b] = s;
		if(lengths[s] >= 32){
			const uint64_t nt = (lengths[s] - 7 + TILE_POS - 1)/TILE_POS;
			for(uint64_t k = 0;k < nt;++k, ++t){ tile_seq[t] = s; tile_pos0[t] = (uint32_t)(k*TILE_POS); }
		}
		pcrhost::PackedSeq q; q.buf = S.packed[s].data(); q.len = lengths[s];
		if(!pcrhost::irregular_words(q, ctx->filt, S.irr_host[s])){
			g_err = "pcr_load_sequences: more than 64 irregular words share one (loc, strand)"; return PCR_ERR_CAPACITY;
		}
	}

	int rc;
	DevBuf<uint8_t> d_packed; DevBuf<uint64_t> d_byte_off;
	if((rc = d_packed.ensure(total_bytes)) != PCR_OK) return rc;
	if((rc = d_byte_off.ensure(n)) != PCR_OK) return rc;
	if((rc = S.planes.ensure(total_blocks)) != PCR_OK) return rc;
	if((rc = S.valid.ensure(S2_VALID_FRONT + total_blocks + S2_TAIL_BLOCKS)) != PCR_OK) return rc;
	if((rc = S.nib.ensure(total_blocks*4 + 8)) != PCR_OK) return rc;
	if((rc = S.tb.ensure(S2_TB_FRONT + (total_blocks + S2_TAIL_BLOCKS)*2 + 8)) != PCR_OK) return rc;
	if((rc = S.tile_degen.ensure(n_tiles + 1)) != PCR_OK) return rc;
	if((rc = S.degen_tiles.ensure(n_tiles + 1)) != PCR_OK) return rc;
	if((rc = S.blk_seq.ensure(total_blocks)) != PCR_OK) return rc;
	if((rc = S.tile_seq.ensure(n_tiles)) != PCR_OK) return rc;
	if((rc = S.tile_pos0.ensure(n_tiles)) != PCR_OK) return rc;
	if((rc = S.d_len.ensure(n)) != PCR_OK) return rc;
	if((rc = S.d_blk_off.ensure(n + 1)) != PCR_OK) return rc;
	if((rc = S.d_nblk_real.ensure(n)) != PCR_OK) return rc;
	if((rc = S.d_active.ensure(n)) != PCR_OK) return rc;
	if((rc = S.d_has_eos.ensure(n)) != PCR_OK) return rc;
#define H2D(dst, src, bytes) do{ if((bytes) > 0){ hipError_t e_ = hipMemcpy(dst, src, bytes, hipMemcpyHostToDevice); \
	if(e_ != hipSuccess){ g_err = std::string("hipMemcpy: ") + hipGetErrorString(e_); return PCR_ERR_DEVICE; } } }while(0)
	{
		std::vector<uint8_t> flat(total_bytes);
		for(uint32_t s = 0;s < n;++s){ if(!S.packed[s].empty()) memcpy(flat.data() + dev_byte_off[s], S.packed[s].data(), S.packed[s].size()); }
		H2D(d_packed.p, flat.data(), flat.size());
	}
	H2D(d_byte_off.p, dev_byte_off.data(), n*sizeof(uint64_t));
	H2D(S.blk_seq.p, blk_seq.data(), total_blocks*sizeof(uint32_t));
	H2D(S.tile_seq.p, tile_seq.data(), n_tiles*sizeof(uint32_t));
	H2D(S.tile_pos0.p, tile_pos0.data(), n_tiles*sizeof(uint32_t));
	H2D(S.d_len.p, S.len.data(), n*sizeof(uint64_t));
	H2D(S.d_blk_off.p, S.blk_off.data(), (n + 1)*sizeof(uint64_t));
	H2D(S.d_nblk_real.p, S.nblk_real.data(), n*sizeof(uint64_t));
	H2D(S.d_active.p, S.active.data(), n);
	H2D(S.d_has_eos.p, S.has_eos.data(), n);
#undef H2D
	{
		hipError_t e_ = hipMemsetAsync(S.valid.p, 0, S2_VALID_FRONT*sizeof(uint32_t), ctx->stream);
		if(e_ == hipSuccess) e_ = hipMemsetAsync(S.valid_d() + total_blocks, 0, S2_TAIL_BLOCKS*sizeof(uint32_t), ctx->stream);
		if(e_ == hipSuccess) e_ = hipMemsetAsync(S.tb.p, 0, S2_TB_FRONT*sizeof(uint32_t), ctx->stream);
		if(e_ == hipSuccess) e_ = hipMemsetAsync(S.tb_d() + total_blocks*2, 0, (S2_TAIL_BLOCKS*2 + 8)*sizeof(uint32_t), ctx->stream);
		if(e_ != hipSuccess){ g_err = std::string("load: padding memset: ") + hipGetErrorString(e_); return PCR_ERR_DEVICE; }
	}
	if(total_blocks){
		const unsigned threads = 256;
		const unsigned grid = (unsigned)((total_blocks + threads - 1)/threads);
		hipLaunchKernelGGL(k_transpose, dim3(grid), dim3(threads), 0, ctx->stream, d_packed.p, d_byte_off.p, S.d_len.p,
			S.d_blk_off.p, S.blk_seq.p, S.planes.p, S.nib.p, S.tb_d(), total_blocks);
		if(hipGetLastError() != hipSuccess){ g_err = "k_transpose launch failed"; return PCR_ERR_DEVICE; }
		if((rc = run_valid(ctx, S, 0, total_blocks)) != PCR_OK) return rc;
	}
	S.bucket_cap = 64;
	S.n_degen_tiles = 0;
	if(n_tiles){
		hipLaunchKernelGGL(k_tile_degen, dim3((unsigned)((n_tiles + 255)/256)), dim3(256), 0, ctx->stream, S.planes.p, S.d_blk_off.p,
			S.d_nblk_real.p, S.tile_seq.p, S.tile_pos0.p, (uint32_t)n_tiles, S.tile_degen.p);
		if(hipGetLastError() != hipSuccess){ g_err = "k_tile_degen launch failed"; return PCR_ERR_DEVICE; }
	}
	if(total_blocks >= (uint64_t(1) << 40)){ g_err = "pcr_load_sequences: more than 2^40 blocks"; return PCR_ERR_CAPACITY; }
	if((rc = build_tile_desc(ctx, S)) != PCR_OK) return rc;
	if(hipStreamSynchronize(ctx->stream) != hipSuccess){ g_err = "load: stream sync failed"; return PCR_ERR_DEVICE; }
	if(n_tiles){
		std::vector<uint8_t> flags(n_tiles);
		std::vector<uint32_t> list;
		if(hipMemcpy(flags.data(), S.tile_degen.p, n_tiles, hipMemcpyDeviceToHost) != hipSuccess){ g_err = "load: flag download failed"; return PCR_ERR_DEVICE; }
		for(uint64_t t2 = 0;t2 < n_tiles;++t2){ if(flags[t2]) list.push_back((uint32_t)t2); }
		S.n_degen_tiles = (uint32_t)list.size();
		if(!list.empty() && hipMemcpy(S.degen_tiles.p, list.data(), list.size()*sizeof(uint32_t), hipMemcpyHostToDevice) != hipSuccess){
			g_err = "load: tile list upload failed"; return PCR_ERR_DEVICE;
		}
	}
	d_packed.release(); d_byte_off.release();
	return upload_irregular(ctx, S);
}

int pcr_set_active(pcr_ctx *ctx, pcr_set which, const uint8_t *active)
{
	if(!set_ok(which)){ g_err = "pcr_set_active: unknown sequence set"; return PCR_ERR_ARG; }
	if(!ctx || !active){ g_err = "pcr_set_active: bad argument"; return PCR_ERR_ARG; }
	DRAIN(ctx);
	HIP_TRY(hipSetDevice(ctx->device));
	SeqSet &S = ctx->sets[which];
	for(uint32_t i = 0;i < S.n;++i) S.active[i] = active[i] ? 1 : 0;
	if(S.n){
		HIP_TRY(hipMemcpyAsync(S.d_active.p, S.active.data(), S.n, hipMemcpyHostToDevice, ctx->stream));
		{ const int rc = build_tile_desc(ctx, S); if(rc != PCR_OK) return rc; }
		if(S.pix_valid && S.pix_usable && S.total_blocks){
			hipLaunchKernelGGL(k_blk_active, dim3((unsigned)((S.total_blocks + 255)/256)), dim3(256), 0, ctx->stream, S.blk_info.p, S.blk_seq.p, S.d_active.p, S.total_blocks);
			HIP_TRY(hipGetLastError());
		}
		HIP_TRY(hipStreamSynchronize(ctx->stream));
	}
	return PCR_OK;
}

int pcr_split_many(pcr_ctx *ctx, pcr_set which, const uint32_t *seq, const uint64_t *pos, uint32_t n)
{
	if(!set_ok(which)){ g_err = "pcr_split: unknown sequence set"; return PCR_ERR_ARG; }
	if(!ctx || (n && (!seq || !pos))){ g_err = "pcr_split: bad argument"; return PCR_ERR_ARG; }
	if(n == 0) return PCR_OK;
	DRAIN(ctx);
	HIP_TRY(hipSetDevice(ctx->device));
	SeqSet &S = ctx->sets[which];
	for(uint32_t i = 0;i < n;++i){ if(seq[i] >= S.n || pos[i] >= S.len[seq[i]]){ g_err = "pcr_split: out of range"; return PCR_ERR_ARG; } }
	std::vector<uint64_t> where(2*(size_t)n);
	std::vector<uint32_t> touched_seq;
	bool eos_changed = false;
	for(uint32_t i = 0;i < n;++i){
		uint8_t &v = S.packed[seq[i]][pos[i] >> 1];
		v = (pos[i] & 1) ? (v & 0xF0) : (v & 0x0F);
		if(!S.has_eos[seq[i]]){ S.has_eos[seq[i]] = 1; eos_changed = true; }
		where[2*(size_t)i] = S.blk_off[seq[i]] + (pos[i] >> 5); where[2*(size_t)i + 1] = pos[i] & 31u;
		touched_seq.push_back(seq[i]);
	}
	std::sort(touched_seq.begin(), touched_seq.end());
	touched_seq.erase(std::unique(touched_seq.begin(), touched_seq.end()), touched_seq.end());
	int rc;
	if(eos_changed) HIP_TRY(hipMemcpyAsync(S.d_has_eos.p, S.has_eos.data(), S.n, hipMemcpyHostToDevice, ctx->stream));
	if((rc = ctx->split_where.ensure(where.size())) != PCR_OK) return rc;
	HIP_TRY(hipMemcpyAsync(ctx->split_where.p, where.data(), where.size()*sizeof(uint64_t), hipMemcpyHostToDevice, ctx->stream));
	hipLaunchKernelGGL(k_apply_splits, dim3((n + 255)/256), dim3(256), 0, ctx->stream, ctx->split_where.p, n, (uint32_t *)S.planes.p, S.nib.p);
	HIP_TRY(hipGetLastError());
	HIP_TRY(hipStreamSynchronize(ctx->stream));
	for(uint32_t i = 0;i < n;++i){
		const uint64_t gb = where[2*(size_t)i];
		const uint64_t first = (gb > S.blk_off[seq[i]]) ? gb - 1 : gb;
		if((rc = run_valid(ctx, S, first, gb - first + 1)) != PCR_OK) return rc;
	}
	const auto t0 = std::chrono::steady_clock::now();
	for(uint32_t sq : touched_seq){
		S.irr_host[sq].clear();
		pcrhost::PackedSeq q; q.buf = S.packed[sq].data(); q.len = S.len[sq];
		if(!pcrhost::irregular_words(q, ctx->filt, S.irr_host[sq])){ g_err = "pcr_split: irregular word overflow"; return PCR_ERR_CAPACITY; }
	}
	S.have_db = false; S.have_codes = false;
	const auto t1 = std::chrono::steady_clock::now();
	rc = upload_irregular(ctx, S);
	if(ctx->timing) fprintf(stderr, "[pcramp] split_many: %u splits in %zu sequences; irregular words %.1f ms, list upload %.1f ms\n", n, touched_seq.size(),
		std::chrono::duration<double, std::milli>(t1 - t0).count(), std::chrono::duration<double, std::milli>(std::chrono::steady_clock::now() - t1).count());
	return rc;
}

int pcr_split(pcr_ctx *ctx, pcr_set which, uint32_t seq, uint64_t pos)
{
	return pcr_split_many(ctx, which, &seq, &pos, 1);
}

}

#include "pcr_select.inc"
#include "pcr_select_sites.inc"

extern "C" {

int pcr_select_words(pcr_ctx *ctx, pcr_set which, const pcr_pair *pairs, uint32_t n_pairs, int optimize_5, int optimize_3,
	float threshold, uint32_t min_oligo_length, uint64_t *n_entries_out)
{
	if(!set_ok(which)){ g_err = "pcr_select_words: unknown sequence set"; return PCR_ERR_ARG; }
	if(!ctx || (n_pairs && !pairs)){ g_err = "pcr_select_words: bad argument"; return PCR_ERR_ARG; }
	DRAIN(ctx);
	return select_impl(ctx, which, pairs, n_pairs, optimize_5, optimize_3, threshold, min_oligo_length, n_entries_out, false);
}

int pcr_screen_device(pcr_ctx *ctx, pcr_set which, const pcr_pair *pairs, uint32_t n_pairs, int optimize_5, int optimize_3,
	float select_threshold, uint32_t min_oligo_length, const pcr_amplify_args *args, uint64_t *d_bits_fr, uint64_t *d_bits_rf)
{
	if(!set_ok(which)){ g_err = "pcr_screen_device: unknown sequence set"; return PCR_ERR_ARG; }
	if(!ctx || !args || (n_pairs && (!pairs || !d_bits_fr || !d_bits_rf))){ g_err = "pcr_screen_device: bad argument"; return PCR_ERR_ARG; }
	if(ctx->pending.size() + 2 >= pcr_ctx::MAIL_RING) DRAIN(ctx);
	return screen_pass(ctx, which, pairs, n_pairs, optimize_5, optimize_3, select_threshold, min_oligo_length, args, d_bits_fr, d_bits_rf);
}

int64_t pcr_get_entries(pcr_ctx *ctx, pcr_set which, pcr_entry *out, uint64_t cap)
{
	if(!set_ok(which)){ g_err = "pcr_get_entries: unknown sequence set"; return PCR_ERR_ARG; }
	if(!ctx){ g_err = "null ctx"; return PCR_ERR_ARG; }
	DRAIN(ctx);
	SeqSet &S = ctx->sets[which];
	if(!S.have_db){ g_err = "pcr_get_entries: no word DB"; return PCR_ERR_STATE; }
	{ const int rc = count_entries(ctx, S); if(rc != PCR_OK) return rc; }
	if(cap && out && S.n_entries){
		std::vector<DevEntry> h(S.n_slots);
		std::vector<uint32_t> hi(S.n);
		hipError_t e = hipStreamSynchronize(ctx->stream);
		if(e == hipSuccess) e = hipMemcpy(h.data(), S.db.p, S.n_slots*sizeof(DevEntry), hipMemcpyDeviceToHost);
		if(e == hipSuccess) e = hipMemcpy(hi.data(), S.d_seg_hi, S.n*sizeof(uint32_t), hipMemcpyDeviceToHost);
		if(e != hipSuccess){ g_err = std::string("pcr_get_entries: ") + hipGetErrorString(e); return PCR_ERR_DEVICE; }
		uint64_t k = 0;
		for(uint32_t q = 0;q < S.n && k < cap;++q){
			for(uint32_t i = q*S.db_cap;i < hi[q] && k < cap;++i, ++k){
				pcrhost::word_of_planes(h[i].w, out[k].word.w);
				out[k].loc = h[i].loc; out[k].index = h[i].seq; out[k].strand = h[i].strand; out[k].pad = 0;
			}
// ... 284 lines not shown
```

### pcramp_amd/csrc/pcr_select.inc

```
namespace {

struct PlanLists {
	std::vector<uint32_t> s2_seeds; std::vector<uint4> s2_masks; std::vector<uint8_t> s2_floors;
	std::vector<uint32_t> s2_group_end, s2_group_offmask, s2_group_or, s2_group_nor;
	std::vector<pcr_ctx::S3Launch> s3_launch;
	std::vector<uint32_t> s3_prefix;
	std::vector<uint8_t> s3_spans;
	std::vector<uint32_t> s1_seeds;
	void clear()
	{
		s2_seeds.clear(); s2_masks.clear(); s2_floors.clear(); s2_group_end.clear(); s2_group_offmask.clear(); s2_group_or.clear(); s2_group_nor.clear();
		s3_launch.clear(); s3_prefix.clear(); s3_spans.clear(); s1_seeds.clear();
	}
};

inline uint32_t spread16(uint32_t v)
{
	v &= 0xFFFFu;
	v = (v | (v << 8)) & 0x00FF00FFu; v = (v | (v << 4)) & 0x0F0F0F0Fu;
	v = (v | (v << 2)) & 0x33333333u; return (v | (v << 1)) & 0x55555555u;
}

constexpr uint32_t S2_MAX_GROUPS = 4096;
bool plan_seed2(pcr_ctx *ctx, PlanLists &L, const std::vector<pcrhost::Candidate> &cand, std::vector<uint32_t> &or_seed, std::vector<uint32_t> &or_plain, uint32_t &irr_off_mask,
	const SeqSet *S3 = nullptr)
{
	std::vector<uint32_t> &pf = L.s3_prefix;
	pf.clear();
	uint32_t pf_run = 0;
	const uint32_t n_or = 2*(uint32_t)cand.size();
	std::vector<uint32_t> &out = L.s2_seeds;
	out.clear(); L.s2_group_end.clear(); L.s2_group_offmask.clear(); L.s2_group_or.clear(); L.s2_group_nor.clear();
	irr_off_mask = 0;
	L.s2_masks.resize(n_or);
	if(ctx->s2_cache.size() > 16384) ctx->s2_cache.clear();
	size_t group_begin = 0; uint32_t group_mask = 0, group_or0 = 0, group_last = 0;
	auto fits = [&](size_t n, uint32_t g_or){
		if(S3) return g_or <= S3_MAX_OR && n <= S3_MAX_SEEDS;
		return g_or <= S2_MAX_OR && n <= S2_MAX_SEEDS && sizeof(S2Shared) + 17*(size_t)g_or + 8*n + 1024 <= 160*1024;
	};
	auto mask_of = [](const Planes &m){
		return make_uint4(spread16(m.a) | (spread16(m.a >> 16) << 1), spread16(m.c) | (spread16(m.c >> 16) << 1),
		                  spread16(m.g) | (spread16(m.g >> 16) << 1), spread16(m.t) | (spread16(m.t >> 16) << 1));
	};
	std::vector<uint8_t> &spans = L.s3_spans;
	spans.clear();
	if(ctx->s3_cache.size() > 16384) ctx->s3_cache.clear();
	for(uint32_t o = 0;o < n_or;++o){
		const pcrhost::Candidate &c = cand[o >> 1];
		const Planes &m = (o & 1u) ? c.rc : c.fwd;
		const pcr_ctx::S2Key key = {m.a, m.c, m.g, m.t, c.floor_};
		pcr_ctx::S3Entry *e3 = nullptr; const pcr_ctx::S2Entry *e2 = nullptr;
		if(S3){
			auto it = ctx->s3_cache.find(key);
			if(it == ctx->s3_cache.end()){
				pcr_ctx::S3Entry e; e.off_mask = 0;
				ctx->s3_tmp.clear(); ctx->s2_tmp.clear();
				e.seedable = pcrhost::orientation_index_seeds(m, c.floor_, ctx->s3_next, ctx->s3_tmp, ctx->s2_tmp);
				e.mask = mask_of(m);
				e.seeds.reserve(ctx->s3_tmp.size()); e.spans.reserve(ctx->s3_tmp.size());
				for(const pcrhost::FoldSeed &sd : ctx->s3_tmp){
					e.seeds.push_back((sd.code << 14) | ((uint32_t)sd.off << 9)); e.spans.push_back((uint8_t)(sd.lo | (sd.hi << 2))); e.off_mask |= 1u << sd.off;
				}
				it = ctx->s3_cache.emplace(key, std::move(e)).first;
			}
			e3 = &it->second; e2 = e3;
		}
		else{
			auto it = ctx->s2_cache.find(key);
			if(it == ctx->s2_cache.end()){
				pcr_ctx::S2Entry e; e.off_mask = 0;
				ctx->s2_tmp.clear();
				e.seedable = pcrhost::orientation_seeds(m, c.floor_, 0, ctx->s2_tmp, nullptr, S2_Q);
				e.mask = mask_of(m);
				e.seeds.reserve(ctx->s2_tmp.size());
				for(const pcrhost::Seed &sd : ctx->s2_tmp){ e.seeds.push_back((sd.code << 14) | ((uint32_t)sd.off << 9)); e.off_mask |= 1u << sd.off; }
				it = ctx->s2_cache.emplace(key, std::move(e)).first;
			}
			e2 = &it->second;
		}
		const pcr_ctx::S2Entry &e = *e2;
		L.s2_masks[o] = e.mask;
		if(!e.seedable){ or_plain.push_back(o); continue; }
		or_seed.push_back(o);
		if(!fits(out.size() - group_begin + e.seeds.size(), o - group_or0 + 1)){
			if(!fits(e.seeds.size(), 1) || L.s2_group_end.size() + 1 >= S2_MAX_GROUPS) return false;
			L.s2_group_end.push_back((uint32_t)out.size()); L.s2_group_offmask.push_back(group_mask); L.s2_group_or.push_back(group_or0); L.s2_group_nor.push_back(group_last - group_or0 + 1);
			group_begin = out.size(); group_mask = 0; group_or0 = o;
			if(S3){ pf.push_back(pf_run); pf_run = 0; }
		}
		group_last = o;
		const size_t at = out.size();
		out.resize(at + e.seeds.size());
		for(size_t k = 0;k < e.seeds.size();++k) out[at + k] = e.seeds[k] | (o - group_or0);
		if(S3){
			spans.insert(spans.end(), e3->spans.begin(), e3->spans.end());
			pcr_ctx::S3Chunks *ch = nullptr;
			for(pcr_ctx::S3Chunks &x : e3->chunks){ if(x.gen == S3->pix_generation){ ch = &x; break; } }
			if(!ch){
				ch = &e3->chunks[e3->next_slot]; e3->next_slot = (e3->next_slot + 1u) % pcr_ctx::S3_CHUNK_SETS;
				ch->run.resize(e.seeds.size());
				const uint32_t *const start = S3->pix_start_h.data();
				uint32_t run = 0;
				for(size_t k = 0;k < e.seeds.size();++k){
					const uint32_t key4 = (e.seeds[k] >> 14) << 2, sp = e3->spans[k];
					ch->run[k] = run; run += (start[key4 + (sp >> 2) + 1u] - start[key4 + (sp & 3u)] + 63u) >> 6;
				}
				ch->total = run; ch->gen = S3->pix_generation;
			}
			const size_t pa = pf.size();
			pf.resize(pa + ch->run.size());
			for(size_t k = 0;k < ch->run.size();++k) pf[pa + k] = pf_run + ch->run[k];
			pf_run += ch->total;
		}
		if(!(o & 1u)){ irr_off_mask |= e.off_mask; group_mask |= e.off_mask; }
	}
	L.s2_group_end.push_back((uint32_t)out.size()); L.s2_group_offmask.push_back(group_mask); L.s2_group_or.push_back(group_or0);
	L.s2_group_nor.push_back(or_seed.empty() ? 0u : group_last - group_or0 + 1);
	if(S3) pf.push_back(pf_run);
	return true;
}

constexpr size_t S3_LDS_BUDGET = 120*1024;
constexpr uint32_t S3_WG_THREADS = 1024;
uint32_t seed3_grid(const pcr_ctx *ctx) { return std::min<uint32_t>(2*ctx->n_cu, S3_MAX_WG); }
bool plan_seed3_slices(pcr_ctx *ctx, PlanLists &PL, bool with_irr)
{
	const uint32_t G_all = seed3_grid(ctx), seeds_per_turn = 16u*(S3_WG_THREADS/64);
	PL.s3_launch.resize(PL.s2_group_end.size());
	size_t g_begin = 0, g_prefix = 0;
	for(size_t g = 0;g < PL.s2_group_end.size();++g){
		const uint32_t ns = PL.s2_group_end[g] - (uint32_t)g_begin;
		g_begin = PL.s2_group_end[g];
		const uint32_t *P = PL.s3_prefix.data() + g_prefix;
		g_prefix += (size_t)ns + 1;
		pcr_ctx::S3Launch &L = PL.s3_launch[g];
		L.n_irr_wg = with_irr ? std::min<uint32_t>((ns + seeds_per_turn - 1u)/seeds_per_turn, G_all/4u) : 0u;
		const uint32_t G = G_all - L.n_irr_wg;
		L.n_chunks = P[ns]; L.per_wg = std::max<uint32_t>(1u, (L.n_chunks + G - 1u)/G); L.slice_cap = 2;
		if(ns == 0) continue;
		uint32_t at = 0;
		for(uint32_t w = 0;w <= G;++w){
			const uint64_t target = (uint64_t)w*L.per_wg;
			while(at + 1u < ns && P[at + 1u] <= target) ++at;
			L.W.start[w] = at;
		}
		for(uint32_t w = G + 1;w <= S3_MAX_WG;++w) L.W.start[w] = at;
		for(uint32_t w = 0;w < G;++w) L.slice_cap = std::max(L.slice_cap, std::min(L.W.start[w + 1] + 2u, ns + 1u) - L.W.start[w]);
		if(17*(size_t)PL.s2_group_nor[g] + 9*(size_t)L.slice_cap + 64 > S3_LDS_BUDGET) return false;
	}
	return true;
}

void plan_seed1(pcr_ctx *ctx, PlanLists &L, const std::vector<pcrhost::Candidate> &cand, std::vector<uint32_t> &or_seed, std::vector<uint32_t> &or_plain, uint32_t &irr_off_mask)
{
	const uint32_t n_or = 2*(uint32_t)cand.size();
	std::vector<uint32_t> &out = L.s1_seeds;
	out.clear();
	irr_off_mask = 0;
	if(ctx->s1_cache.size() > 16384) ctx->s1_cache.clear();
	std::vector<const pcr_ctx::S2Entry *> ent(n_or);
	size_t total = 0;
	for(uint32_t o = 0;o < n_or;++o){
		const pcrhost::Candidate &c = cand[o >> 1];
		const Planes &m = (o & 1u) ? c.rc : c.fwd;
		const pcr_ctx::S2Key key = {m.a, m.c, m.g, m.t, c.floor_};
		auto it = ctx->s1_cache.find(key);
		if(it == ctx->s1_cache.end()){
			pcr_ctx::S2Entry e; e.off_mask = 0;
			ctx->s2_tmp.clear();
			e.seedable = pcrhost::orientation_seeds(m, c.floor_, 0, ctx->s2_tmp);
			e.seeds.reserve(ctx->s2_tmp.size());
			for(const pcrhost::Seed &sd : ctx->s2_tmp){ e.seeds.push_back(sd.code | ((uint32_t)sd.off << 16)); e.off_mask |= 1u << sd.off; }
			it = ctx->s1_cache.emplace(key, std::move(e)).first;
		}
		ent[o] = &it->second;
		if(ent[o]->seedable) total += ent[o]->seeds.size();
	}
	std::vector<uint8_t> drop(n_or, 0);
	if(total > S1_MAX_SEEDS){
		std::vector<uint32_t> by_len;
		for(uint32_t o = 0;o < n_or;++o){ if(ent[o]->seedable) by_len.push_back(o); }
		std::stable_sort(by_len.begin(), by_len.end(), [&](uint32_t x, uint32_t y){ return ent[x]->seeds.size() > ent[y]->seeds.size(); });
		for(size_t i = 0;i < by_len.size() && total > S1_MAX_SEEDS;++i){ drop[by_len[i]] = 1; total -= ent[by_len[i]]->seeds.size(); }
	}
	out.resize(total);
	size_t at = 0;
	for(uint32_t o = 0;o < n_or;++o){
		const pcr_ctx::S2Entry &e = *ent[o];
		if(!e.seedable || drop[o]){ or_plain.push_back(o); continue; }
		or_seed.push_back(o);
		const uint32_t tag = o << 21;
		for(size_t k = 0;k < e.seeds.size();++k) out[at + k] = e.seeds[k] | tag;
		at += e.seeds.size();
		if(!(o & 1u)) irr_off_mask |= e.off_mask;
	}
}

struct HostSeedPlan {
	std::vector<pcrhost::Seed> seeds;
	std::vector<std::vector<std::pair<uint16_t, int8_t> > > inheritors;
	size_t n_inherited = 0;
	std::vector<uint32_t> image, heads, multi;
};

int plan_seed_host(pcr_ctx *ctx, const std::vector<pcrhost::Candidate> &cand, HostSeedPlan &H, std::vector<uint32_t> &or_seed, std::vector<uint32_t> &or_plain,
	uint32_t &irr_off_mask)
{
	const uint32_t n_or = 2*(uint32_t)cand.size();
	struct OrientInfo { uint32_t begin, end; int max_exact_pos; bool seeded; };
	std::vector<OrientInfo> info;
	std::vector<pcrhost::Seed> &seeds = H.seeds;
	std::vector<std::vector<std::pair<uint16_t, int8_t> > > &inheritors = H.inheritors;
	size_t &n_inherited = H.n_inherited;
	std::vector<uint32_t> &image = H.image, &heads = H.heads, &multi = H.multi;
	info.assign(n_or, OrientInfo());
	inheritors.assign(n_or, std::vector<std::pair<uint16_t, int8_t> >());
	seeds.reserve((size_t)n_or*32);
	for(uint32_t o = 0;o < n_or;++o){
		const pcrhost::Candidate &c = cand[o >> 1];
		OrientInfo &me = info[o];
		me.begin = (uint32_t)seeds.size(); me.max_exact_pos = -1;
		const uint32_t bo = 2*c.base + (o & 1u);
		const int32_t sh = (o & 1u) ? -c.shift : c.shift;
		if(c.base != (o >> 1) && info[bo].seeded && info[bo].max_exact_pos <= 24 && info[bo].max_exact_pos + sh <= 24){
			inheritors[bo].push_back(std::make_pair((uint16_t)o, (int8_t)sh));
			n_inherited += info[bo].end - info[bo].begin;
			me.seeded = true; me.max_exact_pos = (info[bo].max_exact_pos < 0) ? -1 : info[bo].max_exact_pos + sh;
		}
		else me.seeded = pcrhost::orientation_seeds((o & 1) ? c.rc : c.fwd, c.floor_, o, seeds, &me.max_exact_pos);
		me.end = (uint32_t)seeds.size();
		if(me.seeded) or_seed.push_back(o); else or_plain.push_back(o);
	}
	if(or_seed.empty()) return PCR_OK;
	if(ctx->seed_count.size() != 65536){ ctx->seed_count.assign(65536, 0); ctx->seed_own.assign(65536, 0); }
	std::vector<uint16_t> &count = ctx->seed_count;
	bool overflow = false;
	uint32_t distinct = 0;
	std::vector<uint8_t> &own = ctx->seed_own;
	for(;;){
		image.assign(SEED_IMAGE_WORDS, 0u);
		overflow = false; distinct = 0;
		for(const pcrhost::Seed &sd : seeds){
			uint16_t &c = count[sd.code];
			if(c == 0){ image[sd.code >> 5] |= 1u << (sd.code & 31); ++distinct; }
			c = (uint16_t)(c + 1 + (inheritors.empty() ? 0 : inheritors[sd.orient].size()));
			if(c > 255){ overflow = true; break; }
			++own[sd.code];
		}
		if(distinct > SEED_MAX_DISTINCT) overflow = true;
		if(!overflow || n_inherited || or_seed.size() < 2) break;
		for(const pcrhost::Seed &sd : seeds){ count[sd.code] = 0; own[sd.code] = 0; }
		std::vector<uint32_t> by_len(or_seed);
		std::stable_sort(by_len.begin(), by_len.end(), [&](uint32_t x, uint32_t y){ return info[x].end - info[x].begin > info[y].end - info[y].begin; });
		const size_t n_drop = (by_len.size() + 3)/4;
		std::vector<uint8_t> drop(n_or, 0);
		for(size_t i = 0;i < n_drop;++i) drop[by_len[i]] = 1;
		std::vector<pcrhost::Seed> kept; kept.reserve(seeds.size());
		for(uint32_t o = 0;o < n_or;++o){
			const uint32_t b = info[o].begin, e = info[o].end;
			info[o].begin = (uint32_t)kept.size();
			if(!drop[o]) kept.insert(kept.end(), seeds.begin() + b, seeds.begin() + e);
			info[o].end = (uint32_t)kept.size();
			if(drop[o]) info[o].seeded = false;
		}
		seeds.swap(kept);
		or_seed.clear(); or_plain.clear();
		for(uint32_t o = 0;o < n_or;++o){ if(info[o].seeded) or_seed.push_back(o); else or_plain.push_back(o); }
	}
	for(const pcrhost::Seed &sd : seeds){
		if(sd.orient & 1u) continue;
		irr_off_mask |= 1u << sd.off;
		if(!inheritors.empty()){ for(const std::pair<uint16_t, int8_t> &in : inheritors[sd.orient]) irr_off_mask |= 1u << (sd.off + in.second); }
	}
	if(overflow){
		or_plain.clear(); or_seed.clear(); image.clear();
		for(uint32_t o = 0;o < n_or;++o) or_plain.push_back(o);
	}
	else{
		uint16_t *rank16 = (uint16_t *)(image.data() + SEED_BITMAP_WORDS);
		uint32_t run = 0;
		for(uint32_t w = 0;w < SEED_BITMAP_WORDS;++w){ rank16[w] = (uint16_t)run; run += (uint32_t)__builtin_popcount(image[w]); }
		heads.assign(distinct, 0u);
		uint32_t n_multi = 0;
		for(const pcrhost::Seed &sd : seeds){
			const uint32_t h = rank16[sd.code >> 5] + (uint32_t)__builtin_popcount(image[sd.code >> 5] & ((1u << (sd.code & 31)) - 1u));
			if(count[sd.code] == 1){ heads[h] = SEED_SINGLE | ((uint32_t)sd.orient << 8) | sd.off; continue; }
			if(heads[h] == 0){ heads[h] = 0x40000000u | n_multi; n_multi += own[sd.code]; }
		}
		std::vector<uint32_t> raw(n_multi, 0u);
		std::vector<uint8_t> &fill = ctx->seed_fill; fill.assign(distinct, 0);
		for(const pcrhost::Seed &sd : seeds){
			if(count[sd.code] == 1) continue;
			const uint32_t h = rank16[sd.code >> 5] + (uint32_t)__builtin_popcount(image[sd.code >> 5] & ((1u << (sd.code & 31)) - 1u));
			const uint32_t start = heads[h] & 0x3FFFFFFFu;
			raw[start + fill[h]++] = (uint32_t)sd.orient | ((uint32_t)sd.off << 24);
		}
		multi.clear(); multi.reserve(n_multi + n_multi/2 + 16);
		for(uint32_t h = 0;h < distinct;++h){
			if(heads[h] & SEED_SINGLE) continue;
			const uint32_t start = heads[h] & 0x3FFFFFFFu, n = fill[h];
			const uint32_t out0 = (uint32_t)multi.size();
			uint32_t header_at = 0, members = 0, cur_base = 0xFFFFFFFFu; int32_t cur_boff = -1;
			for(uint32_t e = 0;e < n;++e){
				const uint32_t sd = raw[start + e], orient = sd & 0xFFFFu, off = sd >> 24;
				const pcrhost::Candidate &c = cand[orient >> 1];
				const int32_t sh = (orient & 1u) ? -c.shift : c.shift;
				int32_t boff = (int32_t)off - sh;
				uint32_t base_orient = 2*c.base + (orient & 1u);
				if(boff < 0 || boff > 24){ boff = (int32_t)off; base_orient = orient; }
				if(members && base_orient == cur_base && boff == cur_boff && members < 256){
					multi.push_back(sd); ++members;
					multi[header_at] = SEED_GROUP | cur_base | ((uint32_t)cur_boff << 16) | ((members - 1) << 21);
				}
				else{
					header_at = (uint32_t)multi.size(); members = 1; cur_base = base_orient; cur_boff = boff;
					multi.push_back(SEED_GROUP | cur_base | ((uint32_t)cur_boff << 16));
					multi.push_back(sd);
				}
				if(!inheritors.empty()){
					for(const std::pair<uint16_t, int8_t> &in : inheritors[orient]){
						if(members == 256){
							header_at = (uint32_t)multi.size(); members = 0;
							multi.push_back(SEED_GROUP | cur_base | ((uint32_t)cur_boff << 16));
						}
						multi.push_back((uint32_t)in.first | ((uint32_t)((int32_t)off + in.second) << 24)); ++members;
						multi[header_at] = SEED_GROUP | cur_base | ((uint32_t)cur_boff << 16) | ((members - 1) << 21);
					}
				}
			}
			heads[h] = (out0 << 9) | ((uint32_t)multi.size() - out0);
		}
		n_multi = (uint32_t)multi.size();
		if(n_multi >= (1u << 22)){ ctx->seed_count.clear(); g_err = "pcr_select_words: seed table too large"; return PCR_ERR_CAPACITY; }
	}
	return PCR_OK;
}


enum class ScanForm { Popcount, BitSliced, Seed1Host, Seed1Dev, Seed2, Seed3 };
inline const char *form_name(ScanForm f)
{
	static const char *const names[] = { "popcount", "bitsliced", "seed1-host", "seed1-dev", "seed2", "seed3" };
	return names[(int)f];
}
inline bool is_seed1(ScanForm f) { return f == ScanForm::Seed1Host || f == ScanForm::Seed1Dev; }
inline bool is_seed2(ScanForm f) { return f == ScanForm::Seed2 || f == ScanForm::Seed3; }

struct ScanPlan {
	ScanForm form = ScanForm::BitSliced;
	std::vector<uint32_t> or_seed, or_plain;
	uint32_t irr_off_mask = 0;
	HostSeedPlan H;
	bool s3_with_irr = false;
	bool need_plain = false, need_seedset = false;
	size_t n_seeds = 0;
	uint32_t n_live = 0, min_len = 0;
	void reset()
	{
		form = ScanForm::BitSliced; or_seed.clear(); or_plain.clear(); irr_off_mask = 0;
		H.seeds.clear(); H.inheritors.clear(); H.n_inherited = 0; H.image.clear(); H.heads.clear(); H.multi.clear();
		s3_with_irr = need_plain = need_seedset = false; n_seeds = 0; n_live = min_len = 0;
	}
};

inline uint32_t live_irregular(const SeqSet &S, uint32_t min_oligo_length)
{
	uint32_t n_live = 0;
	for(uint32_t k = std::min<uint32_t>(min_oligo_length, 256);k < 256;++k) n_live += S.irr_size_count[k];
	return n_live;
}

int irr_index_usable(pcr_ctx *ctx, SeqSet &S, bool &usable)
{
	usable = false;
	if(S.irr_n_multi != 0 || (uint64_t)24*S.n_irr >= (uint64_t(1) << 32)) return PCR_OK;
	const int rc = ensure_irr_index(ctx, S);
	usable = rc == PCR_OK && S.irx_usable;
	return rc;
}

int choose_scan_form(pcr_ctx *ctx, SeqSet &S, const std::vector<pcrhost::Candidate> &cand, int optimize_5, int optimize_3, uint32_t min_oligo_length, ScanPlan &P, PlanLists &L)
{
	const uint32_t n_or = 2*(uint32_t)cand.size();
	std::vector<uint32_t> &or_seed = P.or_seed, &or_plain = P.or_plain;
	P.min_len = min_oligo_length; P.n_live = live_irregular(S, min_oligo_length);
	int rc;
	const bool no_shifts = ctx->scan_version == 3 && !optimize_5 && !optimize_3;
	const bool seed2_ok = no_shifts && !ctx->force_seed1 && n_or <= 65535;
	bool want_seed3 = false;
	if(seed2_ok && !ctx->no_seed3 && !ctx->no_irr_index && ctx->s2_dbg == 0){
		bool worth = true;
		if(!S.pix_valid){
			std::vector<uint32_t> os, op; uint32_t om = 0;
			worth = plan_seed2(ctx, L, cand, os, op, om, nullptr) && op.empty() && !os.empty();
		}
		if(worth){
			if((rc = ensure_pos_index(ctx, S)) != PCR_OK) return rc;
			bool irr_ok = P.n_live == 0;
			if(S.pix_usable && !irr_ok && (rc = irr_index_usable(ctx, S, irr_ok)) != PCR_OK) return rc;
			want_seed3 = S.pix_usable && irr_ok; P.s3_with_irr = P.n_live > 0;
		}
	}
	bool use_seed2 = false;
	if(seed2_ok){
		use_seed2 = plan_seed2(ctx, L, cand, or_seed, or_plain, P.irr_off_mask, want_seed3 ? &S : nullptr);
		if(want_seed3 && !(use_seed2 && or_plain.empty() && !or_seed.empty() && plan_seed3_slices(ctx, L, P.s3_with_irr))){
			or_seed.clear(); or_plain.clear();
			use_seed2 = plan_seed2(ctx, L, cand, or_seed, or_plain, P.irr_off_mask, nullptr);
		}
		if(use_seed2 && !or_plain.empty() && (n_or <= S1_MAX_OR || or_seed.empty())) use_seed2 = false;
		if(!use_seed2){ or_seed.clear(); or_plain.clear(); P.irr_off_mask = 0; }
	}
	const bool use_seed3 = use_seed2 && want_seed3 && or_plain.empty() && !or_seed.empty()
		&& L.s3_prefix.size() == L.s2_seeds.size() + L.s2_group_end.size() && L.s3_spans.size() == L.s2_seeds.size();
	if(use_seed2){ P.form = use_seed3 ? ScanForm::Seed3 : ScanForm::Seed2; P.n_seeds = L.s2_seeds.size(); }
	else if(no_shifts && !ctx->host_seed_tables && n_or <= S1_MAX_OR){
		plan_seed1(ctx, L, cand, or_seed, or_plain, P.irr_off_mask);
		P.form = ScanForm::Seed1Dev; P.n_seeds = L.s1_seeds.size();
	}
	else if(ctx->scan_version == 3 && n_or <= 65535){
		const int prc = plan_seed_host(ctx, cand, P.H, or_seed, or_plain, P.irr_off_mask);
		if(ctx->seed_count.size() == 65536){ for(const pcrhost::Seed &sd : P.H.seeds){ ctx->seed_count[sd.code] = 0; ctx->seed_own[sd.code] = 0; } }
		if(prc != PCR_OK) return prc;
		P.form = ScanForm::Seed1Host; P.n_seeds = P.H.seeds.size() + P.H.n_inherited;
	}
	else{
		for(uint32_t o = 0;o < n_or;++o) or_plain.push_back(o);
		P.form = (ctx->scan_version == 1) ? ScanForm::Popcount : ScanForm::BitSliced;
	}
	if(or_seed.empty() && P.form != ScanForm::Popcount) P.form = ScanForm::BitSliced;
	P.need_plain = (ctx->scan_version != 1) && !or_plain.empty();
	P.need_seedset = !or_seed.empty() && S.n_degen_tiles > 0;
	return PCR_OK;
}

struct PassJob {
	pcr_ctx *ctx = nullptr; int which = 0, opt5 = 0, opt3 = 0; float thr = 0.0f; uint32_t min_len = 0; bool async = false;
	pcr_amplify_args args = {}; FusedAmp fa = {}; bool has_fa = false;
	uint32_t seq = 0;
	bool begun = false, ctrl_was_clean = false;
	std::vector<pcrhost::Candidate> cand; ScanPlan P; PlanLists L;
	std::vector<uint4> hf, hr; std::vector<uint32_t> hfl;
	std::vector<OligoDev> ol;
	bool fuse = false; size_t bits_bytes = 0;
	void reset()
	{
		seq = 0; begun = ctrl_was_clean = false; has_fa = false; fa = FusedAmp(); async = false;
		cand.clear(); P.reset(); L.clear(); hf.clear(); hr.clear(); hfl.clear(); ol.clear(); fuse = false; bits_bytes = 0;
	}
};

struct Scan2Staged { Scan2Tables T; const uint32_t *d_tab = nullptr, *d_bias = nullptr, *d_map = nullptr; };
struct StagedTables {
	SeedTables ST = {};
	Seed2Tables ST2 = {};
	const uint32_t *d_s3_prefix = nullptr; const uint8_t *d_s3_spans = nullptr;
	Scan2Staged plain, seedset;
	bool lean = false, fuse = false;
	size_t bits_bytes = 0;
};

void stage_scan2(Stager &st, const std::vector<uint32_t> &orients, Scan2Staged &B)
{
	B.d_tab = st.put(B.T.tab.data(), B.T.tab.size());
	B.d_bias = st.put(B.T.bias.data(), B.T.bias.size());
	std::vector<uint32_t> m(orients);
	m.resize((m.size() + 255) & ~size_t(255), 0xFFFFFFFFu);
	B.d_map = st.put(m.data(), m.size());
}

void prepare_tables(const SeqSet &S, PassJob &J, FusedAmp *fa)
{
	const std::vector<pcrhost::Candidate> &cand = J.cand;
	const uint32_t ncand = (uint32_t)cand.size(), n_or = 2*ncand;
	J.hf.resize(ncand); J.hr.resize(ncand); J.hfl.resize(ncand);
	for(uint32_t c = 0;c < ncand;++c){
		J.hf[c] = make_uint4(cand[c].fwd.a, cand[c].fwd.c, cand[c].fwd.g, cand[c].fwd.t);
		J.hr[c] = make_uint4(cand[c].rc.a, cand[c].rc.c, cand[c].rc.g, cand[c].rc.t);
		J.hfl[c] = cand[c].floor_;
	}
	if(is_seed2(J.P.form)){
		std::vector<uint8_t> &floors2 = J.L.s2_floors;
		floors2.assign(((size_t)n_or + 15) & ~size_t(15), 0);
		for(uint32_t o = 0;o < n_or;++o) floors2[o] = (uint8_t)std::min<uint32_t>(cand[o >> 1].floor_, 255u);
	}
	J.fuse = false; J.bits_bytes = 0; J.ol.clear();
	if(fa && fa->n_pairs){
		J.bits_bytes = (size_t)fa->n_pairs*((S.n + 63)/64)*sizeof(uint64_t);
		J.fuse = ((uintptr_t)fa->d_fr % 16 == 0) && ((uintptr_t)fa->d_rf % 16 == 0) && (J.bits_bytes % 16 == 0);
		if(J.fuse) build_oligos(fa->pairs, fa->n_pairs, fa->a, J.ol);
	}
}

int stage_tables(pcr_ctx *ctx, SeqSet &S, const PassJob &J, FusedAmp *fa, bool async, bool ctrl_was_clean, StagedTables &T)
{
	const std::vector<pcrhost::Candidate> &cand = J.cand;
	const ScanPlan &P = J.P; const PlanLists &L = J.L;
	const uint32_t ncand = (uint32_t)cand.size(), n_or = 2*ncand;
	const bool seed2 = is_seed2(P.form), seed3 = P.form == ScanForm::Seed3;
	const bool build_tables = P.form == ScanForm::Seed1Dev;
	const HostSeedPlan &H = P.H;
	int rc;
	if(P.need_plain) build_scan2_tables(cand, P.or_plain, T.plain.T);
	if(P.need_seedset) build_scan2_tables(cand, P.or_seed, T.seedset.T);
	size_t bytes = ncand*(2*sizeof(uint4) + sizeof(uint32_t)) + 1024;
	bytes += (T.plain.T.tab.size() + T.plain.T.bias.size() + P.or_plain.size() + 256)*sizeof(uint32_t);
	bytes += (T.seedset.T.tab.size() + T.seedset.T.bias.size() + P.or_seed.size() + 256)*sizeof(uint32_t);
	bytes += (H.image.size() + H.heads.size() + H.multi.size() + 64)*sizeof(uint32_t);
	if(seed2){
		bytes += L.s2_masks.size()*sizeof(uint4) + L.s2_floors.size() + L.s2_seeds.size()*sizeof(uint32_t) + 512;
		if(seed3) bytes += L.s3_prefix.size()*sizeof(uint32_t) + L.s3_spans.size() + 128;
	}
	if(build_tables) bytes += L.s1_seeds.size()*sizeof(uint32_t) + 256;
	T.bits_bytes = J.bits_bytes; T.fuse = J.fuse;
	if(T.fuse) bytes += J.ol.size()*sizeof(OligoDev) + 64;
	const uint32_t guard_seq = J.seq ? J.seq : ctx->mail_seq + 1;
	const uint64_t gen = S.ctrl.generation;
	if((rc = S.ctrl.ensure(8 + 2*(size_t)S.n + 4)) != PCR_OK) return rc;
	T.lean = ctx->direct_ok && async && T.fuse && seed2 && !P.or_seed.empty() && ctrl_was_clean && gen == S.ctrl.generation
		&& S.bucket_cap == POST_CAP && 2*fa->n_pairs <= 32*POST_MASK_WORDS;
	if(ctx->debug_log) fprintf(stderr, "[pcramp] staging: %s\n", T.lean ? "lean (tables written into device memory, no staging launch)" : "k_stage");
	Stager st(ctx);
	if((rc = T.lean ? st.begin_direct(bytes) : st.begin(bytes)) != PCR_OK) return rc;
	ctx->d_cand_fwd = st.put(J.hf.data(), ncand);
	ctx->d_cand_rc = st.put(J.hr.data(), ncand);
	ctx->d_cand_floor = st.put(J.hfl.data(), ncand);
	if(P.need_plain) stage_scan2(st, P.or_plain, T.plain);
	if(P.need_seedset) stage_scan2(st, P.or_seed, T.seedset);
	if(!H.image.empty()){
		T.ST.image = st.put(H.image.data(), H.image.size());
		T.ST.heads = st.put(H.heads.data(), H.heads.size());
		T.ST.multi = H.multi.empty() ? T.ST.heads : st.put(H.multi.data(), H.multi.size());
	}
	const uint32_t *d_s1_seeds = nullptr;
	if(build_tables){
		d_s1_seeds = st.put(L.s1_seeds.data(), L.s1_seeds.size());
		if((rc = ctx->s1_image.ensure(SEED_IMAGE_WORDS)) != PCR_OK) return rc;
		if((rc = ctx->s1_heads.ensure(2*(size_t)S1_MAX_SEEDS)) != PCR_OK) return rc;
		if((rc = ctx->s1_multi.ensure(S1_MAX_SEEDS)) != PCR_OK) return rc;
		T.ST.image = ctx->s1_image.p; T.ST.heads = ctx->s1_heads.p; T.ST.multi = ctx->s1_multi.p; T.ST.flat = 1;
	}
	if(seed2){
		T.ST2.seeds = st.put(L.s2_seeds.data(), L.s2_seeds.size());
		T.ST2.masks = st.put(L.s2_masks.data(), L.s2_masks.size());
		T.ST2.floors = st.put(L.s2_floors.data(), L.s2_floors.size());
		T.ST2.n_seeds = (uint32_t)L.s2_seeds.size(); T.ST2.n_or = n_or;
		if(seed3){ T.d_s3_prefix = st.put(L.s3_prefix.data(), L.s3_prefix.size()); T.d_s3_spans = st.put(L.s3_spans.data(), L.s3_spans.size()); }
	}
	const size_t ctrl_bytes = (8 + 2*(size_t)S.n)*sizeof(uint32_t);
	if(T.fuse){
		fa->d_oligos = st.put(J.ol.data(), J.ol.size());
		fa->staged = true;
		if(T.lean) st.seal(guard_seq);
		else if((rc = st.ship(S.ctrl.p, ctrl_bytes, fa->d_fr, T.bits_bytes, fa->d_rf, T.bits_bytes, guard_seq)) != PCR_OK) return rc;
	}
	else if((rc = st.ship(S.ctrl.p, ctrl_bytes, nullptr, 0, nullptr, 0, guard_seq)) != PCR_OK) return rc;
	if(build_tables){
		if((rc = ctx->s1_part.ensure(2*S1_GROUPS)) != PCR_OK) return rc;
		hipLaunchKernelGGL(k_seed_tables<false>, dim3(S1_GROUPS), dim3(S1_BUILD_THREADS), 0, ctx->stream, d_s1_seeds, (uint32_t)L.s1_seeds.size(),
			ctx->s1_part.p, ctx->s1_image.p, ctx->s1_heads.p, ctx->s1_multi.p);
		hipLaunchKernelGGL(k_seed_tables<true>, dim3(S1_GROUPS), dim3(S1_BUILD_THREADS), 0, ctx->stream, d_s1_seeds, (uint32_t)L.s1_seeds.size(),
			ctx->s1_part.p, ctx->s1_image.p, ctx->s1_heads.p, ctx->s1_multi.p);
		HIP_TRY(hipGetLastError());
	}
	return PCR_OK;
}


int launch_popcount(pcr_ctx *ctx, SeqSet &S, const HitSink &sink)
{
	hipLaunchKernelGGL(k_scan, dim3(S.n_tiles), dim3(SCAN_THREADS), 0, ctx->stream, S.planes.p, S.valid_d(),
		S.d_blk_off.p, S.d_len.p, S.d_active.p, S.tile_seq.p, S.tile_pos0.p, ctx->d_cand_fwd, ctx->d_cand_rc,
		ctx->d_cand_floor, sink.ncand, sink);
	HIP_TRY(hipGetLastError());
	return PCR_OK;
}

int launch_seed1(pcr_ctx *ctx, SeqSet &S, const ScanPlan &P, const StagedTables &T, const HitSink &sink)
{
	const uint32_t ncand = sink.ncand;
	const bool cand_lds = ncand <= SEED_CAND_LDS;
	const auto kernel = cand_lds ? k_seed<true> : k_seed<false>;
	const size_t dyn = cand_lds ? (size_t)ncand*(2*sizeof(uint4) + sizeof(uint32_t)) : 0;
	int per_cu = 0;
	const hipError_t oe = hipOccupancyMaxActiveBlocksPerMultiprocessor(&per_cu, kernel, SEED_THREADS, dyn);
	const size_t lds_wg = ((sizeof(SeedShared) + dyn + 4095)/4096)*4096;
	per_cu = std::max(1, std::min<int>(per_cu, (int)((160*1024)/lds_wg)));
	const uint32_t resident = (oe == hipSuccess) ? (uint32_t)per_cu*ctx->n_cu : SEED_MAX_GRID;
	const uint32_t tiles_per_wg = SEED_WAVES*SEED_TILES_PER_WAVE;
	const dim3 sgrid(std::min<uint32_t>((S.n_tiles + tiles_per_wg - 1)/tiles_per_wg, resident)), sblock(SEED_THREADS);
	IrrArgs IA; IA.irr = S.irr.p; IA.perm = S.irr_perm.p; IA.n_live = P.n_live; IA.off_mask = P.or_plain.empty() ? P.irr_off_mask : 0u;
	const uint32_t irr_wgs = (P.n_live + IRR_THREADS*IRR_PER_LANE - 1)/(IRR_THREADS*IRR_PER_LANE);
	const dim3 fgrid(sgrid.x + irr_wgs);
	if(ctx->debug_log) fprintf(stderr, "[pcramp] k_seed: %d workgroups per CU x %u CUs\n", per_cu, ctx->n_cu);
	hipLaunchKernelGGL(kernel, fgrid, sblock, dyn, ctx->stream, S.tb_d(), S.planes.p, S.valid_d(), S.d_blk_off.p, S.d_nblk_real.p, S.d_len.p, S.d_active.p,
		S.tile_seq.p, S.tile_pos0.p, S.tile_degen.p, S.n_tiles, T.ST, ctx->d_cand_fwd, ctx->d_cand_rc, ctx->d_cand_floor, ncand, IA, sgrid.x, sink);
	HIP_TRY(hipGetLastError());
	return PCR_OK;
}

int launch_seed3_group(pcr_ctx *ctx, SeqSet &S, const Seed2Tables &Tg, const uint32_t *d_chunk_prefix, const uint8_t *d_spans, const pcr_ctx::S3Launch &L3, const IrrArgs2 &IA,
	const HitSink &sink, const S2Clear &Z)
{
	Seed3Tables T3; T3.seeds = Tg.seeds; T3.spans = d_spans; T3.chunk_prefix = d_chunk_prefix; T3.masks = Tg.masks; T3.floors = Tg.floors;
	T3.n_seeds = Tg.n_seeds; T3.n_or = Tg.n_or; T3.or_base = Tg.or_base;
	T3.pix_first = S.pix_first.p; T3.pix_last = S.pix_last.p; T3.pix_ent = S.pix_ent.p;
	Seed3Set Q3 = { S.valid_d(), S.blk_info.p, S.blk_local.p, S.d_active.p };
	T3.n_chunks = L3.n_chunks; T3.per_wg = L3.per_wg; T3.slice_cap = L3.slice_cap;
	T3.n_irr_wg = IA.ix_first ? L3.n_irr_wg : 0u;
	const size_t dyn3 = (size_t)Tg.n_or*sizeof(uint4) + 2*(size_t)T3.slice_cap*sizeof(uint32_t) + (((size_t)Tg.n_or + 15) & ~size_t(15)) + (((size_t)T3.slice_cap + 15) & ~size_t(15)) + 16;
	if(!ctx->s3_attr_set){
		HIP_TRY(hipFuncSetAttribute((const void *)k_seed3<S3_WG_THREADS>, hipFuncAttributeMaxDynamicSharedMemorySize, 128*1024));
		ctx->s3_attr_set = true;
	}
	hipLaunchKernelGGL(k_seed3<S3_WG_THREADS>, dim3(seed3_grid(ctx)), dim3(S3_WG_THREADS), dyn3, ctx->stream, T3, Q3, IA, ctx->d_cand_fwd, ctx->d_cand_floor, sink, Z, L3.W);
	return PCR_OK;
}

int launch_seed_groups(pcr_ctx *ctx, SeqSet &S, const ScanPlan &P, const PlanLists &L, const StagedTables &T, const FusedAmp *fa, const HitSink &sink)
{
	const bool seed3 = P.form == ScanForm::Seed3;
	const uint32_t tiles_per_wg = S2_WAVES*2;
	const dim3 sgrid(std::max<uint32_t>(1u, std::min<uint32_t>((S.n_tiles + tiles_per_wg - 1)/tiles_per_wg, ctx->n_cu))), sblock(S2_THREADS);
	int rc;
	if(!ctx->s2_attr_set){
		HIP_TRY(hipFuncSetAttribute((const void *)k_seed2<false>, hipFuncAttributeMaxDynamicSharedMemorySize, (int)(160*1024 - sizeof(S2Shared))));
		HIP_TRY(hipFuncSetAttribute((const void *)k_seed2<true>, hipFuncAttributeMaxDynamicSharedMemorySize, (int)(160*1024 - sizeof(S2Shared))));
		ctx->s2_attr_set = true;
	}
	const auto k_seed2_of_ctx = ctx->s2_dbg ? k_seed2<true> : k_seed2<false>;
	bool irr_by_index = P.s3_with_irr;
	if(!seed3){
		irr_by_index = P.or_plain.empty() && P.n_live > 0 && !ctx->no_irr_index;
		for(size_t g = 0, b = 0;g < L.s2_group_end.size();++g){ if((size_t)L.s2_group_end[g] - b > (size_t)sgrid.x*S2_THREADS) irr_by_index = false; b = L.s2_group_end[g]; }
		if(irr_by_index && (rc = irr_index_usable(ctx, S, irr_by_index)) != PCR_OK) return rc;
	}
	uint32_t g_begin = 0, g_prefix = 0;
	bool first_launch = true;
	for(size_t g = 0;g < L.s2_group_end.size();++g){
		Seed2Tables Tg = T.ST2;
		const uint32_t or0 = L.s2_group_or[g], g_or = L.s2_group_nor[g];
		const uint8_t *const d_spans = seed3 ? T.d_s3_spans + g_begin : nullptr;
		Tg.seeds = T.ST2.seeds + g_begin; Tg.n_seeds = L.s2_group_end[g] - g_begin;
		Tg.masks = T.ST2.masks + (size_t)or0; Tg.floors = T.ST2.floors + or0; Tg.n_or = g_or; Tg.or_base = or0;
		g_begin = L.s2_group_end[g];
		if(Tg.n_seeds == 0){ g_prefix += 1u; continue; }
		const size_t dyn = (size_t)g_or*sizeof(uint4) + (((size_t)g_or + 15) & ~size_t(15)) + 8*((size_t)Tg.n_seeds + 64) + 16;
		IrrArgs2 IA; IA.scan = S.irr_scan.p; IA.irr = S.irr.p; IA.n_live = P.n_live;
		IA.off_mask = L.s2_group_offmask[g];
		IA.exhaustive = first_launch ? 1u : 0u;
		IA.ix_first = IA.ix_last = IA.ix_words = nullptr; IA.min_cws = std::min<uint32_t>(P.min_len, 255u);
		if(!P.or_plain.empty()){
			IA.off_mask = 0;
			if(!first_launch) IA.n_live = 0;
		}
		else if(irr_by_index){
			IA.ix_first = S.irx_first.p; IA.ix_last = S.irx_last.p; IA.ix_words = S.irx_words.p; IA.n_live = 0;
		}
		if(ctx->debug_log) fprintf(stderr, "[pcramp] k_seed2: %u workgroups, %u seeds of orientations %u..%u (group %zu of %zu), %zu + %zu B of LDS\n", sgrid.x, Tg.n_seeds,
			or0, or0 + g_or - 1, g + 1, L.s2_group_end.size(), sizeof(S2Shared), dyn);
		S2Clear Z = { nullptr, 0u, nullptr, 0u, nullptr };
		if(T.lean && first_launch){
			Z.z0 = (uint4 *)fa->d_fr; Z.z1 = (uint4 *)fa->d_rf; Z.n0 = Z.n1 = (uint32_t)(T.bits_bytes/16); Z.ctrl = sink.counters;
		}
		if(seed3){
			if((rc = launch_seed3_group(ctx, S, Tg, T.d_s3_prefix + g_prefix, d_spans, L.s3_launch[g], IA, sink, Z)) != PCR_OK) return rc;
			g_prefix += Tg.n_seeds + 1u;
		}
		else hipLaunchKernelGGL(k_seed2_of_ctx, sgrid, sblock, dyn, ctx->stream, S.tb_d(), S.valid_d(), S.tile_desc.p, S.n_tiles, Tg, S.d_active.p, ctx->d_cand_fwd, ctx->d_cand_floor,
			sink.ncand, IA, sink, ctx->s2_dbg, Z);
		HIP_TRY(hipGetLastError());
		first_launch = false;
	}
	return PCR_OK;
}

int launch_irregular(pcr_ctx *ctx, SeqSet &S, const ScanPlan &P, const HitSink &sink)
{
	const unsigned irr_grid = (P.n_live + IRR_THREADS*IRR_PER_LANE - 1)/(IRR_THREADS*IRR_PER_LANE);
	hipLaunchKernelGGL(k_scan_irr, dim3(irr_grid), dim3(IRR_THREADS), 0, ctx->stream, S.irr.p, S.irr_perm.p, P.n_live,
		S.d_active.p, ctx->d_cand_fwd, ctx->d_cand_floor, sink.ncand, sink);
	HIP_TRY(hipGetLastError());
	return PCR_OK;
}

int launch_scans(pcr_ctx *ctx, SeqSet &S, const ScanPlan &P, const PlanLists &L, const StagedTables &T, const FusedAmp *fa, const HitSink &sink)
{
	int rc = PCR_OK;
	const uint32_t ncand = sink.ncand;
	if(S.n_tiles){
		ProfScope scan_prof(ctx, PCR_PROF_SCAN, ctx->prof && (ctx->prof_pass++ % ctx->prof_stride) == 0);
		if(P.need_plain && (rc = launch_scan2(ctx, S, T.plain.T, ncand, sink, T.plain.d_tab, T.plain.d_bias, nullptr, S.n_tiles, T.plain.d_map)) != PCR_OK) return rc;
		if(P.form == ScanForm::Popcount) rc = launch_popcount(ctx, S, sink);
		else if(is_seed1(P.form)) rc = launch_seed1(ctx, S, P, T, sink);
		else if(is_seed2(P.form)) rc = launch_seed_groups(ctx, S, P, L, T, fa, sink);
		if(rc != PCR_OK) return rc;
		if(P.need_seedset && (rc = launch_scan2(ctx, S, T.seedset.T, ncand, sink, T.seedset.d_tab, T.seedset.d_bias, S.degen_tiles.p, S.n_degen_tiles,
			T.seedset.d_map)) != PCR_OK) return rc;
		scan_prof.finish();
	}
	const bool irr_taken = S.n_tiles && (is_seed1(P.form) || is_seed2(P.form));
	if(P.n_live && !irr_taken) rc = launch_irregular(ctx, S, P, sink);
	return rc;
}


template<class K>
void launch_post(K kernel, uint32_t waves, pcr_ctx *ctx, SeqSet &S, const HitSink &sink, const FusedAmp *fa, uint32_t seq)
{
	hipLaunchKernelGGL(kernel, dim3((S.n + waves - 1)/waves), dim3(64*waves), 0, ctx->stream, sink.hits, sink.seq_count, sink.best, sink.ncand, S.planes.p,
		S.d_blk_off.p, S.irr.p, S.irr_off.p, S.db.p, S.d_seg_hi, sink.counters, sink.epoch, S.n,
		fa->d_oligos, fa->n_pairs, (2*fa->n_pairs + 31)/32, S.d_len.p, S.d_active.p, fa->a->amp_min, fa->a->amp_max,
		fa->a->ident_threshold, fa->a->use_taq_mama, fa->d_fr, fa->d_rf, (uint64_t)((S.n + 63)/64), ctx->mail.dev + (seq % pcr_ctx::MAIL_RING), seq);
}
int fused_tail(pcr_ctx *ctx, SeqSet &S, const HitSink &sink, FusedAmp *fa, uint32_t reserved_seq)
{
	const uint32_t seq = reserved_seq ? reserved_seq : ++ctx->mail_seq;
	if(sink.cap == POST_CAP){
		launch_post(k_post<8>, 8, ctx, S, sink, fa, seq);
		S.ctrl_clean = true; S.touched_from_seg = true;
	}
	else if(sink.cap == 128) launch_post(k_post_big<128, 4>, 4, ctx, S, sink, fa, seq);
	else launch_post(k_post_big<256, 4>, 4, ctx, S, sink, fa, seq);
	HIP_TRY(hipGetLastError());
	fa->posted = true;
	S.touched_built = false;
	return PCR_OK;
}

template<class K, class... Extra>
void launch_finalize(K kernel, dim3 grid, dim3 block, size_t lds, pcr_ctx *ctx, SeqSet &S, const HitSink &sink, Extra... extra)
{
	hipLaunchKernelGGL(kernel, grid, block, lds, ctx->stream, sink.hits, sink.seq_count, sink.cap, sink.best, sink.ncand, S.planes.p, S.d_blk_off.p, S.irr.p,
		S.irr_off.p, S.db.p, S.d_seg_hi, sink.counters, sink.epoch, S.touched.p, extra...);
}
template<bool ALL = false>
int plain_tail(pcr_ctx *ctx, SeqSet &S, const HitSink &sink, bool async, FusedAmp *fa)
{
	int rc;
	hipLaunchKernelGGL(k_touched, dim3((S.n + 255)/256), dim3(256), 0, ctx->stream, sink.seq_count, S.n, sink.counters, S.touched.p);
	HIP_TRY(hipGetLastError());
	S.touched_built = true;
	uint32_t np2 = 1; while(np2 < sink.cap) np2 <<= 1;
	if(np2 <= 1024) launch_finalize(k_finalize<FIN_WAVES, ALL>, dim3((S.n + FIN_WAVES - 1)/FIN_WAVES), dim3(64*FIN_WAVES), (size_t)FIN_WAVES*np2*sizeof(uint64_t), ctx, S, sink);
	else if(np2 <= MAX_BUCKET_CAP) launch_finalize(k_finalize<1, ALL>, dim3(S.n), dim3(64), (size_t)np2*sizeof(uint64_t), ctx, S, sink);
	else{
		if((rc = ctx->fin_scratch.ensure((size_t)S.n*np2)) != PCR_OK) return rc;
		launch_finalize(k_finalize_big<ALL>, dim3(S.n), dim3(FINBIG_THREADS), 0, ctx, S, sink, ctx->fin_scratch.p);
	}
	HIP_TRY(hipGetLastError());
	++ctx->mail_seq;
	if(async && fa && fa->staged){ fa->pub_seq = ctx->mail_seq; fa->pub_counters = sink.counters; }
	else{
		hipLaunchKernelGGL(k_publish, dim3(1), dim3(64), 0, ctx->stream, sink.counters, ctx->mail.dev + (ctx->mail_seq % pcr_ctx::MAIL_RING), ctx->mail_seq);
		HIP_TRY(hipGetLastError());
	}
	return PCR_OK;
}

uint32_t resized_buckets(bool overflowed, uint32_t cap, uint32_t largest_fill, int attempt)
{
	if(overflowed){
		uint32_t want = cap*2;
		while(want < largest_fill && want < MAX_BUCKET_CAP_GLOBAL) want *= 2;
		return want;
	}
	if(cap <= 64 || attempt >= 12) return 0;
	uint32_t want = 64;
	while(want < largest_fill + largest_fill/16) want *= 2;
	return (want*4 <= cap) ? want : 0;
}

inline bool fused_tail_fits(uint32_t cap, uint32_t n_pairs) { return (cap == POST_CAP || cap == 128 || cap == 256) && 2*n_pairs <= 32*POST_MASK_WORDS; }
inline bool buckets_fit(uint64_t n_slots) { return n_slots < (uint64_t(1) << 32) && n_slots*(sizeof(Hit) + sizeof(DevEntry)) <= (uint64_t(96) << 30); }

inline bool begin_pass(SeqSet &S)
{
	S.have_db = false; S.n_entries = 0;
	const bool ctrl_was_clean = S.ctrl_clean;
	S.ctrl_clean = false; S.touched_from_seg = false;
	return ctrl_was_clean;
}

int plan_pass(pcr_ctx *ctx, PassJob &J, const pcr_pair *pairs, uint32_t n_pairs)
{
	SeqSet &S = ctx->sets[J.which];
	HostTimer timer(ctx, 0);
	if(ctx->timing) ++ctx->n_timed;
	pcrhost::build_candidates((const uint64_t *)pairs, n_pairs, J.opt5 != 0, J.opt3 != 0, J.thr, J.cand);
	const uint32_t ncand = (uint32_t)J.cand.size();
	if(S.n == 0 || ncand == 0) return PCR_OK;
	int rc;
	if((rc = choose_scan_form(ctx, S, J.cand, J.opt5, J.opt3, J.min_len, J.P, J.L)) != PCR_OK) return rc;
	if(ctx->debug_log) fprintf(stderr, "[pcramp] scan plan: form=%s, %u candidates, %zu seeded orientations (%zu seeds), %zu plain, %u/%u IUPAC tiles, %u-slot buckets\n",
		form_name(J.P.form), ncand, J.P.or_seed.size(), J.P.n_seeds, J.P.or_plain.size(), S.n_degen_tiles, S.n_tiles, S.bucket_cap);
	prepare_tables(S, J, J.has_fa ? &J.fa : nullptr);
	return PCR_OK;
}

bool plans_without_device_work(const pcr_ctx *ctx, const SeqSet &S, int opt5, int opt3, uint32_t min_len)
{
	if(ctx->scan_version != 3 || opt5 || opt3 || ctx->force_seed1) return false;
	const bool may_want_seed3 = !ctx->no_seed3 && !ctx->no_irr_index && ctx->s2_dbg == 0;
	if(may_want_seed3 && !S.pix_valid) return false;
	if(live_irregular(S, min_len) == 0 || ctx->no_irr_index) return true;
	return S.irr_n_multi != 0 || (uint64_t)24*S.n_irr >= (uint64_t(1) << 32) || S.irx_valid;
}

bool pass_is_pipelinable(const pcr_ctx *ctx, const PassJob &J)
{
	const SeqSet &S = ctx->sets[J.which];
	return J.async && J.has_fa && J.fuse && S.n != 0 && !J.cand.empty() && is_seed2(J.P.form)
		&& fused_tail_fits(S.bucket_cap, J.fa.n_pairs) && buckets_fit((uint64_t)S.n*S.bucket_cap);
}

int run_pass(pcr_ctx *ctx, PassJob &J, uint64_t *n_entries_out)
{
	SeqSet &S = ctx->sets[J.which];
	FusedAmp *const fa = J.has_fa ? &J.fa : nullptr;
	const bool async = J.async;
	const bool ctrl_was_clean = J.begun ? J.ctrl_was_clean : begin_pass(S);
	const ScanPlan &P = J.P;
	const uint32_t ncand = (uint32_t)J.cand.size();
	if(S.n == 0 || ncand == 0){ S.have_db = true; S.n_touched = 0; return PCR_OK; }
	HostTimer timer(ctx, 1);
	int rc;
	if((rc = ctx->best.ensure((size_t)S.n*ncand)) != PCR_OK) return rc;
	if(ctx->best.generation != ctx->best_seen){
		HIP_TRY(hipMemsetAsync(ctx->best.p, 0, ctx->best.cap*sizeof(uint32_t), ctx->stream));
		ctx->best_seen = ctx->best.generation; ctx->epoch = std::min(ctx->debug_epoch, EPOCH_LIMIT);
	}
	StagedTables T;
	if((rc = stage_tables(ctx, S, J, fa, async, ctrl_was_clean, T)) != PCR_OK) return rc;

	timer.next(2);
	uint32_t h_counters[4];
	if((rc = S.touched.ensure(S.n)) != PCR_OK) return rc;
	S.d_seg_hi = S.ctrl.p + 8 + S.n;
	for(int attempt = 0;;++attempt){
		const uint32_t cap = S.bucket_cap;
		const uint64_t n_slots = (uint64_t)S.n*cap;
		if(!buckets_fit(n_slots)){
			assert(J.seq == 0);
			S.bucket_cap = 64;
			g_err = "pcr_select_words: the per-sequence hit buckets would not fit (too many tied sites per sequence)"; return PCR_ERR_CAPACITY;
		}
		if((rc = ctx->hits.ensure(n_slots)) != PCR_OK) return rc;
		if((rc = S.db.ensure(n_slots)) != PCR_OK) return rc;
		if(attempt > 0) HIP_TRY(hipMemsetAsync(S.ctrl.p, 0, (8 + 2*(size_t)S.n)*sizeof(uint32_t), ctx->stream));
		if(ctx->epoch >= EPOCH_LIMIT){
			HIP_TRY(hipMemsetAsync(ctx->best.p, 0, ctx->best.cap*sizeof(uint32_t), ctx->stream));
			ctx->epoch = 0;
		}
		++ctx->epoch;
		HitSink sink; sink.best = ctx->best.p; sink.hits = ctx->hits.p; sink.seq_count = S.ctrl.p + 8;
		sink.counters = S.ctrl.p; sink.cap = cap; sink.ncand = ncand; sink.epoch = ctx->epoch;
		const bool fused = async && fa && fa->staged && fused_tail_fits(cap, fa->n_pairs);
		if(J.seq && !fused){ g_err = "pcr_screen_device: a pipelined pass lost its fused tail"; return PCR_ERR_STATE; }
		if((rc = launch_scans(ctx, S, P, J.L, T, fa, sink)) != PCR_OK) return rc;
		if((rc = fused ? fused_tail(ctx, S, sink, fa, J.seq) : plain_tail(ctx, S, sink, async, fa)) != PCR_OK) return rc;
		if(async){
			S.db_cap = cap; S.n_slots = n_slots;
			S.n_touched = N_TOUCHED_UNKNOWN; S.n_entries = 1; S.have_db = true;
			return PCR_OK;
		}
		timer.next(3);
		if((rc = mail_wait(ctx, ctx->mail_seq, h_counters)) != PCR_OK) return rc;
		timer.next(2);
		S.db_cap = cap; S.n_slots = n_slots;
		const bool overflowed = (h_counters[0] & 1u) != 0;
		if(overflowed && (attempt >= 12 || cap >= MAX_BUCKET_CAP_GLOBAL)){ g_err = "pcr_select_words: more than 65536 candidate sites in one sequence (per-sequence bucket limit)"; return PCR_ERR_CAPACITY; }
		const uint32_t want = resized_buckets(overflowed, cap, h_counters[2], attempt);
		if(!want) break;
		S.bucket_cap = want;
	}
	if(ctx->debug_log) fprintf(stderr, "[pcramp] pass done: %u-slot buckets, largest fill %u, %u sequences with entries\n", S.db_cap, h_counters[2], h_counters[3]);
	S.n_touched = h_counters[3];
	S.n_entries = S.n_touched ? 1 : 0;
	S.have_db = true;
	if(n_entries_out){
		if((rc = count_entries(ctx, S)) != PCR_OK) return rc;
		*n_entries_out = S.n_entries;
	}
	return PCR_OK;
}

void fill_job(pcr_ctx *ctx, PassJob &J, pcr_set which, int optimize_5, int optimize_3, float threshold, uint32_t min_oligo_length, bool async, const FusedAmp *fa)
{
	J.ctx = ctx; J.which = (int)which; J.opt5 = optimize_5; J.opt3 = optimize_3; J.thr = threshold; J.min_len = min_oligo_length; J.async = async;
	J.has_fa = fa != nullptr;
	if(fa){ J.fa = *fa; J.args = *fa->a; J.fa.a = &J.args; }
}

int select_impl(pcr_ctx *ctx, pcr_set which, const pcr_pair *pairs, uint32_t n_pairs, int optimize_5, int optimize_3,
	float threshold, uint32_t min_oligo_length, uint64_t *n_entries_out, bool async, FusedAmp *fa = nullptr)
{
	if(!ctx || (n_pairs && !pairs)){ g_err = "pcr_select_words: bad argument"; return PCR_ERR_ARG; }
	if(min_oligo_length < 1 || min_oligo_length > 32){ g_err = "pcr_select_words: min_oligo_length must be in [1,32]"; return PCR_ERR_ARG; }
	HIP_TRY(hipSetDevice(ctx->device));
	if(n_entries_out) *n_entries_out = 0;
	assert(ctx->lq_client.queued.load() == 0);
	PassJob J;
	fill_job(ctx, J, which, optimize_5, optimize_3, threshold, min_oligo_length, async, fa);
	J.ctrl_was_clean = begin_pass(ctx->sets[which]); J.begun = true;
	int rc = plan_pass(ctx, J, pairs, n_pairs);
	if(rc == PCR_OK) rc = run_pass(ctx, J, n_entries_out);
	if(fa){ const pcr_amplify_args *a = fa->a; *fa = J.fa; fa->a = a; }
	return rc;
}


struct Launcher {
	int device; hipStream_t stream; unsigned refs = 0;
	cpu_set_t near; bool have_near = false;
	pcrq::LaunchQueue q;
	Launcher(int dev, hipStream_t st, unsigned spin_us);
};
std::mutex g_launchers_m;
std::vector<Launcher *> g_launchers;

PassJob *acquire_job(pcr_ctx *ctx)
{
	PassJob *J = nullptr;
	{
		std::lock_guard<std::mutex> lk(ctx->job_m);
		if(!ctx->job_free.empty()){ J = ctx->job_free.back(); ctx->job_free.pop_back(); }
	}
	if(!J){ J = new PassJob(); ctx->job_all.push_back(J); }
	return J;
}
void release_job(pcr_ctx *ctx, PassJob *J)
{
	J->reset();
	std::lock_guard<std::mutex> lk(ctx->job_m);
	ctx->job_free.push_back(J);
}
void free_jobs(pcr_ctx *ctx)
{
	for(PassJob *J : ctx->job_all) delete J;
	ctx->job_all.clear(); ctx->job_free.clear();
}

constexpr unsigned LAUNCH_SPIN_US = 200;

bool read_cpu_list(const std::string &path, cpu_set_t &set)
{
	CPU_ZERO(&set);
	FILE *f = fopen(path.c_str(), "r");
	if(!f) return false;
	char buf[4096]; const bool got = fgets(buf, sizeof(buf), f) != nullptr;
	fclose(f);
	if(!got) return false;
	for(const char *p = buf;*p && *p != '\n';){
		char *e; const long a = strtol(p, &e, 10);
		if(e == p) return false;
		long b = a;
		if(*e == '-'){ p = e + 1; b = strtol(p, &e, 10); if(e == p) return false; }
		for(long c = a;c <= b && c < CPU_SETSIZE;++c) CPU_SET((int)c, &set);
		p = (*e == ',') ? e + 1 : e;
	}
	return true;
}
bool near_cpus(cpu_set_t &out)
{
	const int cpu = sched_getcpu();
	if(cpu < 0) return false;
	const std::string base = "/sys/devices/system/cpu/cpu" + std::to_string(cpu);
	cpu_set_t llc, core, allowed;
	if(!read_cpu_list(base + "/cache/index3/shared_cpu_list", llc)) return false;
	if(!read_cpu_list(base + "/topology/thread_siblings_list", core)) CPU_ZERO(&core);
	CPU_SET(cpu, &core);
	if(sched_getaffinity(0, sizeof(allowed), &allowed) != 0) return false;
	CPU_ZERO(&out);
	for(int c = 0;c < CPU_SETSIZE;++c){ if(CPU_ISSET(c, &llc) && CPU_ISSET(c, &allowed) && !CPU_ISSET(c, &core)) CPU_SET(c, &out); }
	return CPU_COUNT(&out) > 0;
}

Launcher::Launcher(int dev, hipStream_t st, unsigned spin_us) : device(dev), stream(st),
	q([](void *job, std::string &err) -> int {
		PassJob &J = *(PassJob *)job;
		assert(J.seq != 0 && J.ctx->launcher);
		const int rc = run_pass(J.ctx, J, nullptr);
		if(rc != PCR_OK) err = g_err;
		return rc;
	},
	[](void *job){ PassJob *J = (PassJob *)job; release_job(J->ctx, J); },
	[this]{
		if(have_near) (void)pthread_setaffinity_np(pthread_self(), sizeof(near), &near);
		(void)hipSetDevice(device);
	},
	spin_us)
{
	const char *v = getenv("PCRAMP_LAUNCH_PIN");
	have_near = !(v && v[0] == '0') && near_cpus(near);
}

Launcher *attach_launcher(pcr_ctx *ctx)
{
	if(ctx->launcher) return ctx->launcher;
	std::lock_guard<std::mutex> lk(g_launchers_m);
	for(Launcher *L : g_launchers){ if(L->device == ctx->device && L->stream == ctx->stream){ ++L->refs; return ctx->launcher = L; } }
	unsigned spin = LAUNCH_SPIN_US;
	if(const char *v = getenv("PCRAMP_LAUNCH_SPIN_US")) spin = (unsigned)std::min<unsigned long>(strtoul(v, nullptr, 0), 10000ul);
	Launcher *L = new Launcher(ctx->device, ctx->stream, spin);
	if(ctx->debug_log || ctx->timing) fprintf(stderr, "[pcramp] launcher thread for stream %p: caller on cpu %d, launcher %s (%d cpus), spin %u us\n", (void *)ctx->stream,
		sched_getcpu(), L->have_near ? "pinned beside it" : "not pinned", L->have_near ? CPU_COUNT(&L->near) : 0, spin);
	L->refs = 1;
	g_launchers.push_back(L);
	return ctx->launcher = L;
}
void detach_launcher(pcr_ctx *ctx)
{
	Launcher *L = ctx->launcher;
	if(!L) return;
	ctx->launcher = nullptr;
	{
		std::lock_guard<std::mutex> lk(g_launchers_m);
		if(--L->refs) return;
		g_launchers.erase(std::find(g_launchers.begin(), g_launchers.end(), L));
	}
	L->q.stop();
	delete L;
}

int flush_launcher(pcr_ctx *ctx)
{
	if(!ctx->launcher) return PCR_OK;
	ctx->launcher->q.flush(&ctx->lq_client);
	int code; std::string msg; uint32_t seq;
	if(!ctx->lq_client.take_error(code, msg, seq)) return PCR_OK;
	std::vector<pcr_ctx::Pending> &pd = ctx->pending;
	pd.erase(std::remove_if(pd.begin(), pd.end(), [&](const pcr_ctx::Pending &q){ return (int32_t)(q.seq - seq) >= 0; }), pd.end());
	g_err = msg;
	return code;
}

int screen_pass(pcr_ctx *ctx, pcr_set which, const pcr_pair *pairs, uint32_t n_pairs, int optimize_5, int optimize_3,
	float select_threshold, uint32_t min_oligo_length, const pcr_amplify_args *args, uint64_t *d_bits_fr, uint64_t *d_bits_rf)
{
	if(min_oligo_length < 1 || min_oligo_length > 32){ g_err = "pcr_select_words: min_oligo_length must be in [1,32]"; return PCR_ERR_ARG; }
	int rc;
	if(ctx->lq_client.poisoned.load(std::memory_order_acquire) && (rc = flush_launcher(ctx)) != PCR_OK) return rc;
	HIP_TRY(hipSetDevice(ctx->device));
	SeqSet &S = ctx->sets[which];
	FusedAmp fa; fa.pairs = pairs; fa.n_pairs = n_pairs; fa.a = args; fa.d_fr = d_bits_fr; fa.d_rf = d_bits_rf;
	PassJob *J = acquire_job(ctx);
	fill_job(ctx, *J, which, optimize_5, optimize_3, select_threshold, min_oligo_length, true, &fa);
	bool inline_pass = !ctx->launch_thread || !plans_without_device_work(ctx, S, optimize_5, optimize_3, min_oligo_length);
	if(inline_pass){
		if((rc = flush_launcher(ctx)) != PCR_OK){ release_job(ctx, J); return rc; }
		J->ctrl_was_clean = begin_pass(S); J->begun = true;
	}
	rc = plan_pass(ctx, *J, pairs, n_pairs);
	if(rc == PCR_OK && !inline_pass && !pass_is_pipelinable(ctx, *J)){
		inline_pass = true;
		rc = flush_launcher(ctx);
	}
	if(rc != PCR_OK){
		if(!J->begun){ (void)flush_launcher(ctx); (void)begin_pass(S); }
		release_job(ctx, J);
		return rc;
	}
	pcr_ctx::Pending p;
	p.which = (int)which; p.pairs.assign(pairs, pairs + n_pairs); p.opt5 = optimize_5; p.opt3 = optimize_3;
	p.thr = select_threshold; p.min_len = min_oligo_length; p.args = *args; p.d_fr = d_bits_fr; p.d_rf = d_bits_rf;
	if(!inline_pass){
		Launcher *L = attach_launcher(ctx);
		p.seq = J->seq = ++ctx->mail_seq;
		J->fa.pairs = nullptr;
		ctx->pending.push_back(std::move(p));
		++ctx->n_pipelined;
		L->q.push(&ctx->lq_client, J, J->seq);
		return PCR_OK;
	}
	assert(ctx->lq_client.queued.load() == 0);
	const uint32_t seq0 = ctx->mail_seq;
	rc = run_pass(ctx, *J, nullptr);
	if(rc == PCR_OK && !J->fa.posted) rc = amplify_launch(ctx, S, pairs, n_pairs, args, d_bits_fr, d_bits_rf, &J->fa);
	release_job(ctx, J);
	if(rc != PCR_OK) return rc;
	if(ctx->mail_seq != seq0){
		p.seq = ctx->mail_seq;
		ctx->pending.push_back(std::move(p));
	}
	return PCR_OK;
}

int drain(pcr_ctx *ctx)
{
	{ const int frc = flush_launcher(ctx); if(frc != PCR_OK) return frc; }
	if(ctx->pending.empty()) return PCR_OK;
	std::vector<pcr_ctx::Pending> pend;
	pend.swap(ctx->pending);
	int rc;
	for(size_t i = 0;i < pend.size();++i){
		uint32_t c[4];
		if((rc = mail_wait(ctx, pend[i].seq, c)) != PCR_OK) return rc;
		SeqSet &S = ctx->sets[pend[i].which];
		if(!(c[0] & 1u)){
			if(c[3] == N_TOUCHED_UNKNOWN_DEV){ S.n_touched = N_TOUCHED_UNKNOWN; S.n_entries = 1; }
			else{ S.n_touched = c[3]; S.n_entries = c[3] ? 1 : 0; }
			continue;
		}
		uint32_t want = S.bucket_cap*2;
		while(want < c[2] && want < MAX_BUCKET_CAP_GLOBAL) want *= 2;
		S.bucket_cap = std::min(want, MAX_BUCKET_CAP_GLOBAL);
		for(size_t j = i;j < pend.size();++j){
			const pcr_ctx::Pending &q = pend[j];
			if((rc = select_impl(ctx, (pcr_set)q.which, q.pairs.data(), (uint32_t)q.pairs.size(), q.opt5, q.opt3, q.thr, q.min_len, nullptr, false)) != PCR_OK) return rc;
			if((rc = amplify_launch(ctx, ctx->sets[q.which], q.pairs.data(), (uint32_t)q.pairs.size(), &q.args, q.d_fr, q.d_rf)) != PCR_OK) return rc;
		}
		break;
	}
	return PCR_OK;
}

}
```

Baseline: 23.91 billion.

## Restructure seed3 host planning around cached per-orientation blocks and deferred expansion

Replaces the per-pass seed3 list building with a BlockCache that keeps each orientation's seeds, spans and per-generation chunk prefix runs in one aligned block. The pass plan now holds lightweight records, and the seed, span and prefix arrays are expanded straight into the staging buffer instead of being built in intermediate vectors and then copied. The aim is to cut host planning time and memcpy traffic on the pipelined pass path. It also adds per-stage plan timers and env switches, and it carries the risk of subtle mismatches in slice or group bookkeeping.

Measured after the change: 23.09 billion. -3.4%, worse.

```diff
diff --git a/pcramp_amd/csrc/pcr_device.hip b/pcramp_amd/csrc/pcr_device.hip
--- a/pcramp_amd/csrc/pcr_device.hip
+++ b/pcramp_amd/csrc/pcr_device.hip
@@ -25,6 +25,7 @@
 #include "../../include/pcramp_hip.h"
 #include "pcr_host.hpp"
 #include "pcr_launch_queue.hpp"
+#include "pcr_plan.hpp"
 
 using pcrhost::Planes;
 
@@ -629,14 +630,10 @@
 	struct S2Entry { std::vector<uint32_t> seeds;  uint32_t off_mask; bool seedable; uint4 mask;  };
 	std::unordered_map<S2Key, S2Entry, S2KeyHash> s2_cache;
 	std::vector<pcrhost::Seed> s2_tmp;
-	static constexpr int S3_CHUNK_SETS = 4;
-	struct S3Chunks { uint64_t gen = 0; uint32_t total = 0; std::vector<uint32_t> run; };
-	struct S3Entry : S2Entry { std::vector<uint8_t> spans;  S3Chunks chunks[S3_CHUNK_SETS]; uint32_t next_slot = 0; };
-	std::unordered_map<S2Key, S3Entry, S2KeyHash> s3_cache;
-	std::vector<pcrhost::FoldSeed> s3_tmp;
+	pcrplan::BlockCache s3_blocks;
+	bool s3_lists_caller = false;
 	struct S3Launch { Seed3Slices W; uint32_t n_chunks, per_wg, slice_cap, n_irr_wg; };
 	bool no_seed3 = false, s3_attr_set = false;
-	bool s3_next = true;
 	bool s2_attr_set = false; uint32_t s2_dbg = 0; bool no_irr_index = false;
 	std::unordered_map<S2Key, S2Entry, S2KeyHash> s1_cache;
 	DevBuf<uint32_t> s1_image, s1_heads, s1_multi, s1_part;
@@ -701,6 +698,7 @@
 	const OligoDev *d_oligos = nullptr;
 	bool debug_log = false;
 	bool timing = false; double t_host[8] = {0, 0, 0, 0, 0, 0, 0, 0}; uint64_t n_timed = 0;
+	double t_plan[5] = {0, 0, 0, 0, 0};
 	bool prof = false; uint32_t prof_stride = 1, prof_pass = 0;
 	std::vector<std::pair<Event, Event> > prof_events;
 	double prof_ms = 0.0; uint64_t prof_launches = 0;
@@ -1028,6 +1026,14 @@
 		used = 0;
 		return rc;
 	}
+	template<class T> T *reserve(size_t n, T *&host_at)
+	{
+		used = (used + 15) & ~size_t(15);
+		host_at = (T *)(host + used);
+		T *at = (T *)((direct ? dev : ctx->arena.p) + used);
+		used += n*sizeof(T);
+		return at;
+	}
 	template<class T> T *put(const T *src, size_t n)
 	{
 		used = (used + 15) & ~size_t(15);
@@ -1306,7 +1312,9 @@
 	if(const char *v = getenv("PCRAMP_S2DBG")) ctx->s2_dbg = (uint32_t)atoi(v);
 	if(const char *v = getenv("PCRAMP_IRR_INDEX")) ctx->no_irr_index = v[0] == '0';
 	if(const char *v = getenv("PCRAMP_SEED3")) ctx->no_seed3 = v[0] == '0';
-	if(const char *v = getenv("PCRAMP_S3_NEXT")) ctx->s3_next = v[0] != '0';
+	if(const char *v = getenv("PCRAMP_S3_NEXT")) ctx->s3_blocks.fold = v[0] != '0';
+	if(const char *v = getenv("PCRAMP_S3_LISTS")) ctx->s3_lists_caller = v[0] == 'c';
+	if(const char *v = getenv("PCRAMP_DEBUG_S3_BLOCKS")) ctx->s3_blocks.entry_limit = (size_t)strtoul(v, nullptr, 0);
 	if(const char *v = getenv("PCRAMP_LAUNCH_THREAD")) ctx->launch_thread = v[0] != '0';
 	if(const char *v = getenv("PCRAMP_SCAN")){ if(v[0] == '1') ctx->scan_version = 1; else if(v[0] == '2') ctx->scan_version = 2; }
 	{
@@ -1367,6 +1375,8 @@
 			(unsigned long long)ctx->n_pipelined, (unsigned long long)ctx->n_timed, ctx->lq_client.max_depth);
 		fprintf(stderr, "[pcramp] host us/pass: plan %.1f  stage %.1f  launch %.1f  wait %.1f | amplify prep %.1f  launch %.1f  (%llu passes)\n",
 			ctx->t_host[0]/n, ctx->t_host[1]/n, ctx->t_host[2]/n, ctx->t_host[3]/n, ctx->t_host[4]/n, ctx->t_host[5]/n, (unsigned long long)ctx->n_timed);
+		fprintf(stderr, "[pcramp] host us/pass, stage A in parts: candidates %.1f  blocks + records %.1f  slices %.1f  tables %.1f  enqueue %.1f\n",
+			ctx->t_plan[0]/n, ctx->t_plan[1]/n, ctx->t_plan[2]/n, ctx->t_plan[3]/n, ctx->t_plan[4]/n);
 	}
 	delete ctx;
 }
diff --git a/pcramp_amd/csrc/pcr_plan.hpp b/pcramp_amd/csrc/pcr_plan.hpp
--- /dev/null
+++ b/pcramp_amd/csrc/pcr_plan.hpp
@@ -0,0 +1,250 @@
+#ifndef PCR_PLAN_HPP
+#define PCR_PLAN_HPP
+
+#include <stdint.h>
+#include <stdlib.h>
+#include <string.h>
+#include <algorithm>
+#include <unordered_map>
+#include <vector>
+
+#include "pcr_host.hpp"
+
+namespace pcrplan {
+
+constexpr uint32_t MAX_OR = 448, MAX_SEEDS = 1u << 16, MAX_GROUPS = 4096, MAX_WG = 512;
+constexpr size_t LDS_BUDGET = 120*1024;
+constexpr uint32_t WG_THREADS = 1024;
+constexpr int CHUNK_SETS = 4;
+constexpr uint32_t U32_UNIT = 8, SPAN_UNIT = 32;
+constexpr size_t LIST_SLACK = 32;
+
+struct Mask16 { uint32_t x, y, z, w; };
+
+inline uint32_t spread16(uint32_t v)
+{
+	v &= 0xFFFFu;
+	v = (v | (v << 8)) & 0x00FF00FFu; v = (v | (v << 4)) & 0x0F0F0F0Fu;
+	v = (v | (v << 2)) & 0x33333333u; return (v | (v << 1)) & 0x55555555u;
+}
+inline Mask16 mask_of(const pcrhost::Planes &m)
+{
+	const Mask16 r = { spread16(m.a) | (spread16(m.a >> 16) << 1), spread16(m.c) | (spread16(m.c >> 16) << 1),
+	                   spread16(m.g) | (spread16(m.g >> 16) << 1), spread16(m.t) | (spread16(m.t >> 16) << 1) };
+	return r;
+}
+
+struct Key { uint32_t a, c, g, t, floor_; bool operator==(const Key &o) const { return a == o.a && c == o.c && g == o.g && t == o.t && floor_ == o.floor_; } };
+struct KeyHash { size_t operator()(const Key &k) const { uint64_t h = 0x9E3779B97F4A7C15ull; for(uint32_t v : {k.a, k.c, k.g, k.t, k.floor_}){ h ^= v; h *= 0x100000001B3ull; h ^= h >> 29; } return (size_t)h; } };
+
+struct alignas(32) Block {
+	uint32_t ns, ns8, sp32, off_mask;
+	Mask16 mask;
+	bool seedable;
+	uint32_t next_slot;
+	uint64_t gen[CHUNK_SETS];
+	uint32_t total[CHUNK_SETS];
+	const uint32_t *seeds() const { return (const uint32_t *)(this + 1); }
+	uint32_t *seeds() { return (uint32_t *)(this + 1); }
+	uint32_t *run(int slot) { return seeds() + (size_t)(1 + slot)*ns8; }
+	uint8_t *spans() { return (uint8_t *)(seeds() + (size_t)(1 + CHUNK_SETS)*ns8); }
+};
+inline uint32_t round_up(uint32_t n, uint32_t unit) { return (n + unit - 1u)/unit*unit; }
+
+struct SetIndex { const uint32_t *start; uint64_t generation; };
+
+struct Rec { const uint32_t *seeds, *run; const uint8_t *spans; uint32_t ns, local, seed_base, chunk_base; };
+
+struct PassPlan {
+	std::vector<Rec> recs;
+	std::vector<uint32_t> group_rec_end;
+	std::vector<uint32_t> group_end, group_offmask, group_or, group_nor, group_chunks;
+	std::vector<Mask16> masks;
+	uint32_t n_seeds = 0;
+	void clear()
+	{
+		recs.clear(); group_rec_end.clear(); group_end.clear(); group_offmask.clear(); group_or.clear(); group_nor.clear(); group_chunks.clear();
+		masks.clear(); n_seeds = 0;
+	}
+	size_t n_groups() const { return group_end.size(); }
+	uint32_t group_seeds(size_t g) const { return group_end[g] - (g ? group_end[g - 1] : 0u); }
+	size_t prefix_size() const { return (size_t)n_seeds + group_end.size(); }
+};
+
+class BlockCache {
+public:
+	size_t entry_limit = 16384;
+	bool fold = true;
+	BlockCache() {}
+	~BlockCache() { clear(); }
+	BlockCache(const BlockCache &) = delete;
+	BlockCache &operator=(const BlockCache &) = delete;
+	size_t size() const { return map_.size(); }
+	void clear()
+	{
+		for(auto &kv : map_) free(kv.second);
+		map_.clear();
+	}
+	Block *get(const pcrhost::Planes &m, uint32_t floor_)
+	{
+		const Key key = {m.a, m.c, m.g, m.t, floor_};
+		auto it = map_.find(key);
+		if(it != map_.end()) return it->second;
+		tmp3_.clear(); tmp2_.clear();
+		const bool seedable = pcrhost::orientation_index_seeds(m, floor_, fold, tmp3_, tmp2_);
+		const uint32_t ns = (uint32_t)tmp3_.size(), ns8 = round_up(ns, U32_UNIT), sp32 = round_up(ns, SPAN_UNIT);
+		const size_t bytes = sizeof(Block) + (size_t)(1 + CHUNK_SETS)*ns8*sizeof(uint32_t) + sp32;
+		Block *b = (Block *)aligned_alloc(alignof(Block), (bytes + alignof(Block) - 1)/alignof(Block)*alignof(Block));
+		if(!b) abort();
+		memset(b, 0, bytes);
+		b->ns = ns; b->ns8 = ns8; b->sp32 = sp32; b->seedable = seedable; b->mask = mask_of(m);
+		uint32_t *sd = b->seeds(); uint8_t *sp = b->spans();
+		for(uint32_t k = 0;k < ns;++k){
+			const pcrhost::FoldSeed &f = tmp3_[k];
+			sd[k] = (f.code << 14) | ((uint32_t)f.off << 9); sp[k] = (uint8_t)(f.lo | (f.hi << 2)); b->off_mask |= 1u << f.off;
+		}
+		map_.emplace(key, b);
+		return b;
+	}
+private:
+	std::unordered_map<Key, Block *, KeyHash> map_;
+	std::vector<pcrhost::FoldSeed> tmp3_; std::vector<pcrhost::Seed> tmp2_;
+};
+
+template<class Flush>
+inline int block_chunks(Block *b, const SetIndex &X, Flush &flush, bool &flushed, int &slot_out)
+{
+	for(int s = 0;s < CHUNK_SETS;++s){ if(b->gen[s] == X.generation){ slot_out = s; return 0; } }
+	const int slot = (int)b->next_slot;
+	if(b->gen[slot] != 0 && !flushed){
+		const int rc = flush();
+		if(rc != 0) return rc;
+		flushed = true;
+	}
+	b->next_slot = (b->next_slot + 1u) % CHUNK_SETS;
+	const uint32_t *const sd = b->seeds(); const uint8_t *const sp = b->spans();
+	uint32_t *const run = b->run(slot);
+	uint32_t acc = 0;
+	for(uint32_t k = 0;k < b->ns;++k){
+		const uint32_t key4 = (sd[k] >> 14) << 2, s = sp[k];
+		run[k] = acc; acc += (X.start[key4 + (s >> 2) + 1u] - X.start[key4 + (s & 3u)] + 63u) >> 6;
+	}
+	b->total[slot] = acc; b->gen[slot] = X.generation;
+	slot_out = slot;
+	return 0;
+}
+
+template<class Flush>
+inline int plan_lists(BlockCache &C, PassPlan &P, const std::vector<pcrhost::Candidate> &cand, const SetIndex &X, std::vector<uint32_t> &or_seed,
+	std::vector<uint32_t> &or_plain, uint32_t &irr_off_mask, Flush flush, bool &fits)
+{
+	const uint32_t n_or = 2*(uint32_t)cand.size();
+	P.clear();
+	P.masks.resize(n_or);
+	irr_off_mask = 0; fits = true;
+	bool flushed = false;
+	int rc;
+	if(C.size() > C.entry_limit){
+		if((rc = flush()) != 0) return rc;
+		flushed = true;
+		C.clear();
+	}
+	auto fit = [](size_t n, uint32_t g_or){ return g_or <= MAX_OR && n <= MAX_SEEDS; };
+	uint32_t n_out = 0, group_begin = 0, group_mask = 0, group_or0 = 0, group_last = 0, pf_run = 0;
+	for(uint32_t o = 0;o < n_or;++o){
+		const pcrhost::Candidate &c = cand[o >> 1];
+		Block *const b = C.get((o & 1u) ? c.rc : c.fwd, c.floor_);
+		P.masks[o] = b->mask;
+		if(!b->seedable){ or_plain.push_back(o); continue; }
+		or_seed.push_back(o);
+		if(!fit((size_t)(n_out - group_begin) + b->ns, o - group_or0 + 1)){
+			if(!fit(b->ns, 1) || P.group_end.size() + 1 >= MAX_GROUPS){ fits = false; return 0; }
+			P.group_end.push_back(n_out); P.group_offmask.push_back(group_mask); P.group_or.push_back(group_or0); P.group_nor.push_back(group_last - group_or0 + 1);
+			P.group_chunks.push_back(pf_run); P.group_rec_end.push_back((uint32_t)P.recs.size());
+			group_begin = n_out; group_mask = 0; group_or0 = o; pf_run = 0;
+		}
+		group_last = o;
+		int slot;
+		if((rc = block_chunks(b, X, flush, flushed, slot)) != 0) return rc;
+		const Rec r = { b->seeds(), b->run(slot), b->spans(), b->ns, o - group_or0, n_out - group_begin, pf_run };
+		P.recs.push_back(r);
+		n_out += b->ns; pf_run += b->total[slot];
+		if(!(o & 1u)){ irr_off_mask |= b->off_mask; group_mask |= b->off_mask; }
+	}
+	P.group_end.push_back(n_out); P.group_offmask.push_back(group_mask); P.group_or.push_back(group_or0);
+	P.group_nor.push_back(or_seed.empty() ? 0u : group_last - group_or0 + 1);
+	P.group_chunks.push_back(pf_run); P.group_rec_end.push_back((uint32_t)P.recs.size());
+	P.n_seeds = n_out;
+	return 0;
+}
+
+inline uint32_t count_le(const uint32_t *a, uint32_t n, uint32_t v)
+{
+	if(n == 0) return 0;
+	const uint32_t *b = a;
+	for(uint32_t len = n;len > 1;){ const uint32_t half = len >> 1; b = (b[half] <= v) ? b + half : b; len -= half; }
+	return (uint32_t)(b - a) + (b[0] <= v ? 1u : 0u);
+}
+
+struct LaunchShape { uint32_t n_chunks, per_wg, slice_cap, n_irr_wg; };
+
+inline bool plan_slices(const PassPlan &P, size_t g, uint32_t grid, bool with_irr, uint32_t *start, LaunchShape &L)
+{
+	const uint32_t ns = P.group_seeds(g), seeds_per_turn = 16u*(WG_THREADS/64);
+	const Rec *const R = P.recs.data() + (g ? P.group_rec_end[g - 1] : 0u);
+	const uint32_t nr = P.group_rec_end[g] - (g ? P.group_rec_end[g - 1] : 0u);
+	L.n_irr_wg = with_irr ? std::min<uint32_t>((ns + seeds_per_turn - 1u)/seeds_per_turn, grid/4u) : 0u;
+	const uint32_t G = grid - L.n_irr_wg;
+	L.n_chunks = P.group_chunks[g]; L.per_wg = std::max<uint32_t>(1u, (L.n_chunks + G - 1u)/G); L.slice_cap = 2;
+	if(ns == 0) return true;
+	uint32_t r = 0, at = 0;
+	for(uint32_t w = 0;w <= G;++w){
+		const uint64_t target = (uint64_t)w*L.per_wg;
+		while(r + 1u < nr && R[r + 1u].chunk_base <= target) ++r;
+		const uint32_t rel = (uint32_t)std::min<uint64_t>(target - R[r].chunk_base, 0xFFFFFFFFull);
+		const uint32_t n_le = R[r].seed_base + count_le(R[r].run, R[r].ns, rel);
+		at = std::max(n_le, 1u) - 1u;
+		start[w] = at;
+	}
+	for(uint32_t w = G + 1;w <= MAX_WG;++w) start[w] = at;
+	for(uint32_t w = 0;w < G;++w) L.slice_cap = std::max(L.slice_cap, std::min(start[w + 1] + 2u, ns + 1u) - start[w]);
+	return 17*(size_t)P.group_nor[g] + 9*(size_t)L.slice_cap + 64 <= LDS_BUDGET;
+}
+
+inline void expand_group(const PassPlan &P, size_t g, uint32_t *seeds, uint8_t *spans, uint32_t *prefix)
+{
+	const Rec *const R = P.recs.data() + (g ? P.group_rec_end[g - 1] : 0u);
+	const uint32_t nr = P.group_rec_end[g] - (g ? P.group_rec_end[g - 1] : 0u);
+	if(seeds){
+		for(uint32_t r = 0;r < nr;++r){
+			const uint32_t *const src = R[r].seeds; uint32_t *const dst = seeds + R[r].seed_base; const uint32_t id = R[r].local;
+			for(uint32_t k = 0;k < R[r].ns;k += U32_UNIT){ for(uint32_t j = 0;j < U32_UNIT;++j) dst[k + j] = src[k + j] | id; }
+		}
+	}
+	if(spans){
+		for(uint32_t r = 0;r < nr;++r){
+			const uint8_t *const src = R[r].spans; uint8_t *const dst = spans + R[r].seed_base;
+			for(uint32_t k = 0;k < R[r].ns;k += SPAN_UNIT) memcpy(dst + k, src + k, SPAN_UNIT);
+		}
+	}
+	if(prefix){
+		for(uint32_t r = 0;r < nr;++r){
+			const uint32_t *const src = R[r].run; uint32_t *const dst = prefix + R[r].seed_base; const uint32_t base = R[r].chunk_base;
+			for(uint32_t k = 0;k < R[r].ns;k += U32_UNIT){ for(uint32_t j = 0;j < U32_UNIT;++j) dst[k + j] = base + src[k + j]; }
+		}
+		prefix[P.group_seeds(g)] = P.group_chunks[g];
+	}
+}
+
+inline void expand_pass(const PassPlan &P, uint32_t *seeds, uint8_t *spans, uint32_t *prefix)
+{
+	size_t s0 = 0, p0 = 0;
+	for(size_t g = 0;g < P.n_groups();++g){
+		expand_group(P, g, seeds ? seeds + s0 : nullptr, spans ? spans + s0 : nullptr, prefix ? prefix + p0 : nullptr);
+		s0 = P.group_end[g]; p0 = (size_t)P.group_end[g] + g + 1;
+	}
+}
+
+}
+
+#endif
diff --git a/pcramp_amd/csrc/pcr_select.inc b/pcramp_amd/csrc/pcr_select.inc
--- a/pcramp_amd/csrc/pcr_select.inc
+++ b/pcramp_amd/csrc/pcr_select.inc
@@ -3,31 +3,22 @@
 struct PlanLists {
 	std::vector<uint32_t> s2_seeds; std::vector<uint4> s2_masks; std::vector<uint8_t> s2_floors;
 	std::vector<uint32_t> s2_group_end, s2_group_offmask, s2_group_or, s2_group_nor;
+	pcrplan::PassPlan s3;
 	std::vector<pcr_ctx::S3Launch> s3_launch;
+	bool s3_expanded = false;
 	std::vector<uint32_t> s3_prefix;
 	std::vector<uint8_t> s3_spans;
 	std::vector<uint32_t> s1_seeds;
 	void clear()
 	{
 		s2_seeds.clear(); s2_masks.clear(); s2_floors.clear(); s2_group_end.clear(); s2_group_offmask.clear(); s2_group_or.clear(); s2_group_nor.clear();
-		s3_launch.clear(); s3_prefix.clear(); s3_spans.clear(); s1_seeds.clear();
+		s3.clear(); s3_launch.clear(); s3_expanded = false; s3_prefix.clear(); s3_spans.clear(); s1_seeds.clear();
 	}
 };
 
-inline uint32_t spread16(uint32_t v)
-{
-	v &= 0xFFFFu;
-	v = (v | (v << 8)) & 0x00FF00FFu; v = (v | (v << 4)) & 0x0F0F0F0Fu;
-	v = (v | (v << 2)) & 0x33333333u; return (v | (v << 1)) & 0x55555555u;
-}
-
 constexpr uint32_t S2_MAX_GROUPS = 4096;
-bool plan_seed2(pcr_ctx *ctx, PlanLists &L, const std::vector<pcrhost::Candidate> &cand, std::vector<uint32_t> &or_seed, std::vector<uint32_t> &or_plain, uint32_t &irr_off_mask,
-	const SeqSet *S3 = nullptr)
-{
-	std::vector<uint32_t> &pf = L.s3_prefix;
-	pf.clear();
-	uint32_t pf_run = 0;
+bool plan_seed2(pcr_ctx *ctx, PlanLists &L, const std::vector<pcrhost::Candidate> &cand, std::vector<uint32_t> &or_seed, std::vector<uint32_t> &or_plain, uint32_t &irr_off_mask)
+{
 	const uint32_t n_or = 2*(uint32_t)cand.size();
 	std::vector<uint32_t> &out = L.s2_seeds;
 	out.clear(); L.s2_group_end.clear(); L.s2_group_offmask.clear(); L.s2_group_or.clear(); L.s2_group_nor.clear();
@@ -36,50 +27,24 @@
 	if(ctx->s2_cache.size() > 16384) ctx->s2_cache.clear();
 	size_t group_begin = 0; uint32_t group_mask = 0, group_or0 = 0, group_last = 0;
 	auto fits = [&](size_t n, uint32_t g_or){
-		if(S3) return g_or <= S3_MAX_OR && n <= S3_MAX_SEEDS;
 		return g_or <= S2_MAX_OR && n <= S2_MAX_SEEDS && sizeof(S2Shared) + 17*(size_t)g_or + 8*n + 1024 <= 160*1024;
 	};
-	auto mask_of = [](const Planes &m){
-		return make_uint4(spread16(m.a) | (spread16(m.a >> 16) << 1), spread16(m.c) | (spread16(m.c >> 16) << 1),
-		                  spread16(m.g) | (spread16(m.g >> 16) << 1), spread16(m.t) | (spread16(m.t >> 16) << 1));
-	};
-	std::vector<uint8_t> &spans = L.s3_spans;
-	spans.clear();
-	if(ctx->s3_cache.size() > 16384) ctx->s3_cache.clear();
+	auto mask_of = [](const Planes &m){ const pcrplan::Mask16 k = pcrplan::mask_of(m); return make_uint4(k.x, k.y, k.z, k.w); };
 	for(uint32_t o = 0;o < n_or;++o){
 		const pcrhost::Candidate &c = cand[o >> 1];
 		const Planes &m = (o & 1u) ? c.rc : c.fwd;
 		const pcr_ctx::S2Key key = {m.a, m.c, m.g, m.t, c.floor_};
-		pcr_ctx::S3Entry *e3 = nullptr; const pcr_ctx::S2Entry *e2 = nullptr;
-		if(S3){
-			auto it = ctx->s3_cache.find(key);
-			if(it == ctx->s3_cache.end()){
-				pcr_ctx::S3Entry e; e.off_mask = 0;
-				ctx->s3_tmp.clear(); ctx->s2_tmp.clear();
-				e.seedable = pcrhost::orientation_index_seeds(m, c.floor_, ctx->s3_next, ctx->s3_tmp, ctx->s2_tmp);
-				e.mask = mask_of(m);
-				e.seeds.reserve(ctx->s3_tmp.size()); e.spans.reserve(ctx->s3_tmp.size());
-				for(const pcrhost::FoldSeed &sd : ctx->s3_tmp){
-					e.seeds.push_back((sd.code << 14) | ((uint32_t)sd.off << 9)); e.spans.push_back((uint8_t)(sd.lo | (sd.hi << 2))); e.off_mask |= 1u << sd.off;
-				}
-				it = ctx->s3_cache.emplace(key, std::move(e)).first;
-			}
-			e3 = &it->second; e2 = e3;
-		}
-		else{
-			auto it = ctx->s2_cache.find(key);
-			if(it == ctx->s2_cache.end()){
-				pcr_ctx::S2Entry e; e.off_mask = 0;
-				ctx->s2_tmp.clear();
-				e.seedable = pcrhost::orientation_seeds(m, c.floor_, 0, ctx->s2_tmp, nullptr, S2_Q);
-				e.mask = mask_of(m);
-				e.seeds.reserve(ctx->s2_tmp.size());
-				for(const pcrhost::Seed &sd : ctx->s2_tmp){ e.seeds.push_back((sd.code << 14) | ((uint32_t)sd.off << 9)); e.off_mask |= 1u << sd.off; }
-				it = ctx->s2_cache.emplace(key, std::move(e)).first;
-			}
-			e2 = &it->second;
-		}
-		const pcr_ctx::S2Entry &e = *e2;
+		auto it = ctx->s2_cache.find(key);
+		if(it == ctx->s2_cache.end()){
+			pcr_ctx::S2Entry e; e.off_mask = 0;
+			ctx->s2_tmp.clear();
+			e.seedable = pcrhost::orientation_seeds(m, c.floor_, 0, ctx->s2_tmp, nullptr, S2_Q);
+			e.mask = mask_of(m);
+			e.seeds.reserve(ctx->s2_tmp.size());
+			for(const pcrhost::Seed &sd : ctx->s2_tmp){ e.seeds.push_back((sd.code << 14) | ((uint32_t)sd.off << 9)); e.off_mask |= 1u << sd.off; }
+			it = ctx->s2_cache.emplace(key, std::move(e)).first;
+		}
+		const pcr_ctx::S2Entry &e = it->second;
 		L.s2_masks[o] = e.mask;
 		if(!e.seedable){ or_plain.push_back(o); continue; }
 		or_seed.push_back(o);
@@ -87,67 +52,47 @@
 			if(!fits(e.seeds.size(), 1) || L.s2_group_end.size() + 1 >= S2_MAX_GROUPS) return false;
 			L.s2_group_end.push_back((uint32_t)out.size()); L.s2_group_offmask.push_back(group_mask); L.s2_group_or.push_back(group_or0); L.s2_group_nor.push_back(group_last - group_or0 + 1);
 			group_begin = out.size(); group_mask = 0; group_or0 = o;
-			if(S3){ pf.push_back(pf_run); pf_run = 0; }
 		}
 		group_last = o;
 		const size_t at = out.size();
 		out.resize(at + e.seeds.size());
 		for(size_t k = 0;k < e.seeds.size();++k) out[at + k] = e.seeds[k] | (o - group_or0);
-		if(S3){
-			spans.insert(spans.end(), e3->spans.begin(), e3->spans.end());
-			pcr_ctx::S3Chunks *ch = nullptr;
-			for(pcr_ctx::S3Chunks &x : e3->chunks){ if(x.gen == S3->pix_generation){ ch = &x; break; } }
-			if(!ch){
-				ch = &e3->chunks[e3->next_slot]; e3->next_slot = (e3->next_slot + 1u) % pcr_ctx::S3_CHUNK_SETS;
-				ch->run.resize(e.seeds.size());
-				const uint32_t *const start = S3->pix_start_h.data();
-				uint32_t run = 0;
-				for(size_t k = 0;k < e.seeds.size();++k){
-					const uint32_t key4 = (e.seeds[k] >> 14) << 2, sp = e3->spans[k];
-					ch->run[k] = run; run += (start[key4 + (sp >> 2) + 1u] - start[key4 + (sp & 3u)] + 63u) >> 6;
-				}
-				ch->total = run; ch->gen = S3->pix_generation;
-			}
-			const size_t pa = pf.size();
-			pf.resize(pa + ch->run.size());
-			for(size_t k = 0;k < ch->run.size();++k) pf[pa + k] = pf_run + ch->run[k];
-			pf_run += ch->total;
-		}
 		if(!(o & 1u)){ irr_off_mask |= e.off_mask; group_mask |= e.off_mask; }
 	}
 	L.s2_group_end.push_back((uint32_t)out.size()); L.s2_group_offmask.push_back(group_mask); L.s2_group_or.push_back(group_or0);
 	L.s2_group_nor.push_back(or_seed.empty() ? 0u : group_last - group_or0 + 1);
-	if(S3) pf.push_back(pf_run);
 	return true;
 }
 
-constexpr size_t S3_LDS_BUDGET = 120*1024;
-constexpr uint32_t S3_WG_THREADS = 1024;
+int plan_seed3(pcr_ctx *ctx, const SeqSet &S, PlanLists &L, const std::vector<pcrhost::Candidate> &cand, std::vector<uint32_t> &or_seed, std::vector<uint32_t> &or_plain,
+	uint32_t &irr_off_mask, bool &fits)
+{
+	const pcrplan::SetIndex X = { S.pix_start_h.data(), S.pix_generation };
+	L.s3_expanded = false;
+	return pcrplan::plan_lists(ctx->s3_blocks, L.s3, cand, X, or_seed, or_plain, irr_off_mask, [ctx]{ return flush_launcher(ctx); }, fits);
+}
+void expand_seed3_in_job(PlanLists &L)
+{
+	const pcrplan::PassPlan &Q = L.s3;
+	L.s2_seeds.resize(Q.n_seeds + pcrplan::LIST_SLACK/sizeof(uint32_t)); L.s3_prefix.resize(Q.prefix_size() + pcrplan::LIST_SLACK/sizeof(uint32_t)); L.s3_spans.resize(Q.n_seeds + pcrplan::LIST_SLACK);
+	pcrplan::expand_pass(Q, L.s2_seeds.data(), L.s3_spans.data(), L.s3_prefix.data());
+	L.s3_expanded = true;
+}
+
+static_assert(pcrplan::MAX_OR == S3_MAX_OR && pcrplan::MAX_SEEDS == S3_MAX_SEEDS && pcrplan::MAX_WG == S3_MAX_WG && pcrplan::MAX_GROUPS == S2_MAX_GROUPS, "pcr_plan.hpp plans for other limits than k_seed3's");
+static_assert(sizeof(pcrplan::Mask16) == sizeof(uint4), "a mask entry is 16 bytes");
+constexpr uint32_t S3_WG_THREADS = pcrplan::WG_THREADS;
 uint32_t seed3_grid(const pcr_ctx *ctx) { return std::min<uint32_t>(2*ctx->n_cu, S3_MAX_WG); }
 bool plan_seed3_slices(pcr_ctx *ctx, PlanLists &PL, bool with_irr)
 {
-	const uint32_t G_all = seed3_grid(ctx), seeds_per_turn = 16u*(S3_WG_THREADS/64);
-	PL.s3_launch.resize(PL.s2_group_end.size());
-	size_t g_begin = 0, g_prefix = 0;
-	for(size_t g = 0;g < PL.s2_group_end.size();++g){
-		const uint32_t ns = PL.s2_group_end[g] - (uint32_t)g_begin;
-		g_begin = PL.s2_group_end[g];
-		const uint32_t *P = PL.s3_prefix.data() + g_prefix;
-		g_prefix += (size_t)ns + 1;
+	const uint32_t G_all = seed3_grid(ctx);
+	PL.s3_launch.resize(PL.s3.n_groups());
+	for(size_t g = 0;g < PL.s3.n_groups();++g){
 		pcr_ctx::S3Launch &L = PL.s3_launch[g];
-		L.n_irr_wg = with_irr ? std::min<uint32_t>((ns + seeds_per_turn - 1u)/seeds_per_turn, G_all/4u) : 0u;
-		const uint32_t G = G_all - L.n_irr_wg;
-		L.n_chunks = P[ns]; L.per_wg = std::max<uint32_t>(1u, (L.n_chunks + G - 1u)/G); L.slice_cap = 2;
-		if(ns == 0) continue;
-		uint32_t at = 0;
-		for(uint32_t w = 0;w <= G;++w){
-			const uint64_t target = (uint64_t)w*L.per_wg;
-			while(at + 1u < ns && P[at + 1u] <= target) ++at;
-			L.W.start[w] = at;
-		}
-		for(uint32_t w = G + 1;w <= S3_MAX_WG;++w) L.W.start[w] = at;
-		for(uint32_t w = 0;w < G;++w) L.slice_cap = std::max(L.slice_cap, std::min(L.W.start[w + 1] + 2u, ns + 1u) - L.W.start[w]);
-		if(17*(size_t)PL.s2_group_nor[g] + 9*(size_t)L.slice_cap + 64 > S3_LDS_BUDGET) return false;
+		pcrplan::LaunchShape sh;
+		const bool ok = pcrplan::plan_slices(PL.s3, g, G_all, with_irr, L.W.start, sh);
+		L.n_chunks = sh.n_chunks; L.per_wg = sh.per_wg; L.slice_cap = sh.slice_cap; L.n_irr_wg = sh.n_irr_wg;
+		if(!ok) return false;
 	}
 	return true;
 }
@@ -380,7 +325,20 @@
 	return rc;
 }
 
-int choose_scan_form(pcr_ctx *ctx, SeqSet &S, const std::vector<pcrhost::Candidate> &cand, int optimize_5, int optimize_3, uint32_t min_oligo_length, ScanPlan &P, PlanLists &L)
+struct PlanClock {
+	pcr_ctx *ctx; std::chrono::steady_clock::time_point t0;
+	explicit PlanClock(pcr_ctx *c) : ctx(c) { if(ctx->timing) t0 = std::chrono::steady_clock::now(); }
+	void mark(int part)
+	{
+		if(!ctx->timing) return;
+		const auto t1 = std::chrono::steady_clock::now();
+		ctx->t_plan[part] += std::chrono::duration<double, std::micro>(t1 - t0).count();
+		t0 = t1;
+	}
+};
+
+int choose_scan_form(pcr_ctx *ctx, SeqSet &S, const std::vector<pcrhost::Candidate> &cand, int optimize_5, int optimize_3, uint32_t min_oligo_length, ScanPlan &P, PlanLists &L,
+	PlanClock &clock)
 {
 	const uint32_t n_or = 2*(uint32_t)cand.size();
 	std::vector<uint32_t> &or_seed = P.or_seed, &or_plain = P.or_plain;
@@ -393,7 +351,7 @@
 		bool worth = true;
 		if(!S.pix_valid){
 			std::vector<uint32_t> os, op; uint32_t om = 0;
-			worth = plan_seed2(ctx, L, cand, os, op, om, nullptr) && op.empty() && !os.empty();
+			worth = plan_seed2(ctx, L, cand, os, op, om) && op.empty() && !os.empty();
 		}
 		if(worth){
 			if((rc = ensure_pos_index(ctx, S)) != PCR_OK) return rc;
@@ -402,19 +360,22 @@
 			want_seed3 = S.pix_usable && irr_ok; P.s3_with_irr = P.n_live > 0;
 		}
 	}
-	bool use_seed2 = false;
+	bool use_seed2 = false, use_seed3 = false;
 	if(seed2_ok){
-		use_seed2 = plan_seed2(ctx, L, cand, or_seed, or_plain, P.irr_off_mask, want_seed3 ? &S : nullptr);
-		if(want_seed3 && !(use_seed2 && or_plain.empty() && !or_seed.empty() && plan_seed3_slices(ctx, L, P.s3_with_irr))){
-			or_seed.clear(); or_plain.clear();
-			use_seed2 = plan_seed2(ctx, L, cand, or_seed, or_plain, P.irr_off_mask, nullptr);
-		}
+		if(want_seed3){
+			bool fits = false;
+			if((rc = plan_seed3(ctx, S, L, cand, or_seed, or_plain, P.irr_off_mask, fits)) != PCR_OK) return rc;
+			clock.mark(1);
+			use_seed3 = fits && or_plain.empty() && !or_seed.empty() && plan_seed3_slices(ctx, L, P.s3_with_irr);
+			clock.mark(2);
+			if(use_seed3 && ctx->s3_lists_caller){ expand_seed3_in_job(L); clock.mark(1); }
+			if(!use_seed3){ or_seed.clear(); or_plain.clear(); P.irr_off_mask = 0; L.s3.clear(); L.s3_launch.clear(); }
+		}
+		use_seed2 = use_seed3 || plan_seed2(ctx, L, cand, or_seed, or_plain, P.irr_off_mask);
 		if(use_seed2 && !or_plain.empty() && (n_or <= S1_MAX_OR || or_seed.empty())) use_seed2 = false;
 		if(!use_seed2){ or_seed.clear(); or_plain.clear(); P.irr_off_mask = 0; }
 	}
-	const bool use_seed3 = use_seed2 && want_seed3 && or_plain.empty() && !or_seed.empty()
-		&& L.s3_prefix.size() == L.s2_seeds.size() + L.s2_group_end.size() && L.s3_spans.size() == L.s2_seeds.size();
-	if(use_seed2){ P.form = use_seed3 ? ScanForm::Seed3 : ScanForm::Seed2; P.n_seeds = L.s2_seeds.size(); }
+	if(use_seed2){ P.form = use_seed3 ? ScanForm::Seed3 : ScanForm::Seed2; P.n_seeds = use_seed3 ? L.s3.n_seeds : L.s2_seeds.size(); }
 	else if(no_shifts && !ctx->host_seed_tables && n_or <= S1_MAX_OR){
 		plan_seed1(ctx, L, cand, or_seed, or_plain, P.irr_off_mask);
 		P.form = ScanForm::Seed1Dev; P.n_seeds = L.s1_seeds.size();
@@ -432,6 +393,7 @@
 	if(or_seed.empty() && P.form != ScanForm::Popcount) P.form = ScanForm::BitSliced;
 	P.need_plain = (ctx->scan_version != 1) && !or_plain.empty();
 	P.need_seedset = !or_seed.empty() && S.n_degen_tiles > 0;
+	if(!use_seed3) clock.mark(1);
 	return PCR_OK;
 }
 
@@ -509,8 +471,8 @@
 	bytes += (T.seedset.T.tab.size() + T.seedset.T.bias.size() + P.or_seed.size() + 256)*sizeof(uint32_t);
 	bytes += (H.image.size() + H.heads.size() + H.multi.size() + 64)*sizeof(uint32_t);
 	if(seed2){
-		bytes += L.s2_masks.size()*sizeof(uint4) + L.s2_floors.size() + L.s2_seeds.size()*sizeof(uint32_t) + 512;
-		if(seed3) bytes += L.s3_prefix.size()*sizeof(uint32_t) + L.s3_spans.size() + 128;
+		if(seed3) bytes += L.s3.masks.size()*sizeof(uint4) + L.s2_floors.size() + L.s3.n_seeds*(sizeof(uint32_t) + 1) + L.s3.prefix_size()*sizeof(uint32_t) + 640 + 3*pcrplan::LIST_SLACK;
+		else bytes += L.s2_masks.size()*sizeof(uint4) + L.s2_floors.size() + L.s2_seeds.size()*sizeof(uint32_t) + 512;
 	}
 	if(build_tables) bytes += L.s1_seeds.size()*sizeof(uint32_t) + 256;
 	T.bits_bytes = J.bits_bytes; T.fuse = J.fuse;
@@ -541,12 +503,25 @@
 		if((rc = ctx->s1_multi.ensure(S1_MAX_SEEDS)) != PCR_OK) return rc;
 		T.ST.image = ctx->s1_image.p; T.ST.heads = ctx->s1_heads.p; T.ST.multi = ctx->s1_multi.p; T.ST.flat = 1;
 	}
-	if(seed2){
+	if(seed3){
+		const pcrplan::PassPlan &Q = L.s3;
+		uint32_t *h32 = nullptr; uint8_t *h8 = nullptr;
+		if(L.s3_expanded) T.ST2.seeds = st.put(L.s2_seeds.data(), Q.n_seeds);
+		else{ T.ST2.seeds = st.reserve(Q.n_seeds, h32); pcrplan::expand_pass(Q, h32, nullptr, nullptr); }
+		T.ST2.masks = st.put((const uint4 *)Q.masks.data(), Q.masks.size());
+		T.ST2.floors = st.put(L.s2_floors.data(), L.s2_floors.size());
+		T.ST2.n_seeds = Q.n_seeds; T.ST2.n_or = n_or;
+		if(L.s3_expanded){ T.d_s3_prefix = st.put(L.s3_prefix.data(), Q.prefix_size()); T.d_s3_spans = st.put(L.s3_spans.data(), Q.n_seeds); }
+		else{
+			T.d_s3_prefix = st.reserve(Q.prefix_size(), h32); pcrplan::expand_pass(Q, nullptr, nullptr, h32);
+			T.d_s3_spans = st.reserve(Q.n_seeds, h8); pcrplan::expand_pass(Q, nullptr, h8, nullptr);
+		}
+	}
+	else if(seed2){
 		T.ST2.seeds = st.put(L.s2_seeds.data(), L.s2_seeds.size());
 		T.ST2.masks = st.put(L.s2_masks.data(), L.s2_masks.size());
 		T.ST2.floors = st.put(L.s2_floors.data(), L.s2_floors.size());
 		T.ST2.n_seeds = (uint32_t)L.s2_seeds.size(); T.ST2.n_or = n_or;
-		if(seed3){ T.d_s3_prefix = st.put(L.s3_prefix.data(), L.s3_prefix.size()); T.d_s3_spans = st.put(L.s3_spans.data(), L.s3_spans.size()); }
 	}
 	const size_t ctrl_bytes = (8 + 2*(size_t)S.n)*sizeof(uint32_t);
 	if(T.fuse){
@@ -621,6 +596,8 @@
 int launch_seed_groups(pcr_ctx *ctx, SeqSet &S, const ScanPlan &P, const PlanLists &L, const StagedTables &T, const FusedAmp *fa, const HitSink &sink)
 {
 	const bool seed3 = P.form == ScanForm::Seed3;
+	const std::vector<uint32_t> &group_end = seed3 ? L.s3.group_end : L.s2_group_end, &group_offmask = seed3 ? L.s3.group_offmask : L.s2_group_offmask,
+		&group_or = seed3 ? L.s3.group_or : L.s2_group_or, &group_nor = seed3 ? L.s3.group_nor : L.s2_group_nor;
 	const uint32_t tiles_per_wg = S2_WAVES*2;
 	const dim3 sgrid(std::max<uint32_t>(1u, std::min<uint32_t>((S.n_tiles + tiles_per_wg - 1)/tiles_per_wg, ctx->n_cu))), sblock(S2_THREADS);
 	int rc;
@@ -633,22 +610,22 @@
 	bool irr_by_index = P.s3_with_irr;
 	if(!seed3){
 		irr_by_index = P.or_plain.empty() && P.n_live > 0 && !ctx->no_irr_index;
-		for(size_t g = 0, b = 0;g < L.s2_group_end.size();++g){ if((size_t)L.s2_group_end[g] - b > (size_t)sgrid.x*S2_THREADS) irr_by_index = false; b = L.s2_group_end[g]; }
+		for(size_t g = 0, b = 0;g < group_end.size();++g){ if((size_t)group_end[g] - b > (size_t)sgrid.x*S2_THREADS) irr_by_index = false; b = group_end[g]; }
 		if(irr_by_index && (rc = irr_index_usable(ctx, S, irr_by_index)) != PCR_OK) return rc;
 	}
 	uint32_t g_begin = 0, g_prefix = 0;
 	bool first_launch = true;
-	for(size_t g = 0;g < L.s2_group_end.size();++g){
+	for(size_t g = 0;g < group_end.size();++g){
 		Seed2Tables Tg = T.ST2;
-		const uint32_t or0 = L.s2_group_or[g], g_or = L.s2_group_nor[g];
+		const uint32_t or0 = group_or[g], g_or = group_nor[g];
 		const uint8_t *const d_spans = seed3 ? T.d_s3_spans + g_begin : nullptr;
-		Tg.seeds = T.ST2.seeds + g_begin; Tg.n_seeds = L.s2_group_end[g] - g_begin;
+		Tg.seeds = T.ST2.seeds + g_begin; Tg.n_seeds = group_end[g] - g_begin;
 		Tg.masks = T.ST2.masks + (size_t)or0; Tg.floors = T.ST2.floors + or0; Tg.n_or = g_or; Tg.or_base = or0;
-		g_begin = L.s2_group_end[g];
+		g_begin = group_end[g];
 		if(Tg.n_seeds == 0){ g_prefix += 1u; continue; }
 		const size_t dyn = (size_t)g_or*sizeof(uint4) + (((size_t)g_or + 15) & ~size_t(15)) + 8*((size_t)Tg.n_seeds + 64) + 16;
 		IrrArgs2 IA; IA.scan = S.irr_scan.p; IA.irr = S.irr.p; IA.n_live = P.n_live;
-		IA.off_mask = L.s2_group_offmask[g];
+		IA.off_mask = group_offmask[g];
 		IA.exhaustive = first_launch ? 1u : 0u;
 		IA.ix_first = IA.ix_last = IA.ix_words = nullptr; IA.min_cws = std::min<uint32_t>(P.min_len, 255u);
 		if(!P.or_plain.empty()){
@@ -659,7 +636,7 @@
 			IA.ix_first = S.irx_first.p; IA.ix_last = S.irx_last.p; IA.ix_words = S.irx_words.p; IA.n_live = 0;
 		}
 		if(ctx->debug_log) fprintf(stderr, "[pcramp] k_seed2: %u workgroups, %u seeds of orientations %u..%u (group %zu of %zu), %zu + %zu B of LDS\n", sgrid.x, Tg.n_seeds,
-			or0, or0 + g_or - 1, g + 1, L.s2_group_end.size(), sizeof(S2Shared), dyn);
+			or0, or0 + g_or - 1, g + 1, group_end.size(), sizeof(S2Shared), dyn);
 		S2Clear Z = { nullptr, 0u, nullptr, 0u, nullptr };
 		if(T.lean && first_launch){
 			Z.z0 = (uint4 *)fa->d_fr; Z.z1 = (uint4 *)fa->d_rf; Z.n0 = Z.n1 = (uint32_t)(T.bits_bytes/16); Z.ctrl = sink.counters;
@@ -788,14 +765,17 @@
 	SeqSet &S = ctx->sets[J.which];
 	HostTimer timer(ctx, 0);
 	if(ctx->timing) ++ctx->n_timed;
+	PlanClock clock(ctx);
 	pcrhost::build_candidates((const uint64_t *)pairs, n_pairs, J.opt5 != 0, J.opt3 != 0, J.thr, J.cand);
+	clock.mark(0);
 	const uint32_t ncand = (uint32_t)J.cand.size();
 	if(S.n == 0 || ncand == 0) return PCR_OK;
 	int rc;
-	if((rc = choose_scan_form(ctx, S, J.cand, J.opt5, J.opt3, J.min_len, J.P, J.L)) != PCR_OK) return rc;
+	if((rc = choose_scan_form(ctx, S, J.cand, J.opt5, J.opt3, J.min_len, J.P, J.L, clock)) != PCR_OK) return rc;
 	if(ctx->debug_log) fprintf(stderr, "[pcramp] scan plan: form=%s, %u candidates, %zu seeded orientations (%zu seeds), %zu plain, %u/%u IUPAC tiles, %u-slot buckets\n",
 		form_name(J.P.form), ncand, J.P.or_seed.size(), J.P.n_seeds, J.P.or_plain.size(), S.n_degen_tiles, S.n_tiles, S.bucket_cap);
 	prepare_tables(S, J, J.has_fa ? &J.fa : nullptr);
+	clock.mark(3);
 	return PCR_OK;
 }
 
@@ -1062,6 +1042,7 @@
 		release_job(ctx, J);
 		return rc;
 	}
+	PlanClock clock(ctx);
 	pcr_ctx::Pending p;
 	p.which = (int)which; p.pairs.assign(pairs, pairs + n_pairs); p.opt5 = optimize_5; p.opt3 = optimize_3;
 	p.thr = select_threshold; p.min_len = min_oligo_length; p.args = *args; p.d_fr = d_bits_fr; p.d_rf = d_bits_rf;
@@ -1072,6 +1053,7 @@
 		ctx->pending.push_back(std::move(p));
 		++ctx->n_pipelined;
 		L->q.push(&ctx->lq_client, J, J->seq);
+		clock.mark(4);
 		return PCR_OK;
 	}
 	assert(ctx->lq_client.queued.load() == 0);
```
